# kshedden/muscato

Measured on AMD Instinct MI355X. Metric: reads/sec (100 bp, multi-map) at 1/2/4/8 MI355X; confirm-kernel HBM GB/s vs peak, higher is better.
Workload: dtype u32

## Files before the change

include/muscato_hip.h:

```cpp
#ifndef MUSCATO_HIP_H
#define MUSCATO_HIP_H

#include <stdint.h>

#ifdef __cplusplus
extern "C" {
#endif

#define MUSC_ABI_VERSION 3
#define MUSC_MAX_WINDOWS 16

typedef struct musc_ctx musc_ctx;

typedef struct {
  uint32_t read_idx;
  uint32_t gene_idx;
  uint32_t pos;
  uint32_t nmiss;
} musc_hit;

typedef struct {
  int32_t n_windows;
  int32_t windows[MUSC_MAX_WINDOWS];
  int32_t window_width;
  double pmatch;
  int32_t min_dinuc;
  int32_t max_read_length;
  int32_t max_matches;
  int32_t match_mode;
  int32_t mmtol;
  int32_t apply_mmtol;
  int32_t max_mismatch_p1;
  int32_t skip_block_check;
  int32_t n_shards;
  int32_t reserved[2];
} musc_params;

typedef struct {
  uint64_t n_reads;
  uint64_t n_read_windows;
  uint64_t n_candidates;
  uint64_t n_pairs;
  uint64_t n_accepted;
  uint64_t n_hits;
  uint64_t n_overflow_blocks;
  uint64_t confirm_bytes;
  uint32_t confirm_launches;
  uint32_t n_batches;
  float ms_screen;
  float ms_scan;
  uint32_t match_variant;
  float ms_confirm;
  float ms_select;
  float ms_total;
  float ms_index_build;
  float ms_read_prep;
  uint64_t n_descriptors;
  uint32_t index_kind;
  uint32_t match_launches;
  uint64_t n_overflow_entries;
  uint64_t match_bytes;
  uint64_t match_bytes_strict;
  uint64_t index_bytes;
} musc_stats;

int musc_abi_version(void);

int musc_init(int device_ordinal, musc_ctx** out);
void musc_destroy(musc_ctx* ctx);
const char* musc_last_error(musc_ctx* ctx);
int musc_reload_env(musc_ctx* ctx);

int musc_db_load_ascii(musc_ctx* ctx, const char* seqs, const uint64_t* offsets, uint32_t nseq,
                       int on_device);
int musc_db_load_packed(musc_ctx* ctx, const uint8_t* bases2bit, const uint8_t* nmask,
                        const uint64_t* seq_offsets, uint32_t nseq);
int musc_db_build_index(musc_ctx* ctx, int32_t window_width);
int musc_db_build_index_for(musc_ctx* ctx, const musc_params* params, int32_t max_read_len);

int musc_db_set_partition_bases(musc_ctx* ctx, uint64_t max_bases);
int musc_db_partitions(musc_ctx* ctx, uint32_t* first_target, uint32_t cap, uint32_t* n);

int musc_reads_load_ascii(musc_ctx* ctx, const char* seqs, const uint64_t* offsets,
                          uint64_t nreads, int on_device);
int musc_reads_load_packed(musc_ctx* ctx, const uint8_t* bases2bit, const uint8_t* nmask,
                           const uint64_t* read_offsets, uint64_t nreads);
int musc_reads_load_packed32(musc_ctx* ctx, const uint8_t* bases2bit, const uint8_t* nmask,
                             const uint32_t* lengths, uint32_t fixed_len, uint64_t nreads, int async);

int musc_reads_sort_unique(musc_ctx* ctx, const char* seqs, const uint64_t* offsets, uint64_t nreads,
                           int on_device, uint32_t** order, uint32_t** ustart, uint64_t* nunique);

typedef struct musc_fastq_prep {
  uint64_t n_records, n_short, n_reads, n_unique;
  uint32_t max_len, reserved;
  uint64_t *name_off, *seq_off;
  uint32_t *name_len, *seq_len;
  uint32_t *order, *ustart;
} musc_fastq_prep;
int  musc_reads_prep_fastq(musc_ctx* ctx, const char* text, uint64_t nbytes, int on_device,
                           int32_t min_read_len, int32_t max_read_len, musc_fastq_prep* out);
void musc_fastq_prep_free(musc_fastq_prep* p);

int musc_match_device(musc_ctx* ctx, const musc_params* params, uint64_t* nhits);
int musc_hits_copy(musc_ctx* ctx, musc_hit* dst, uint64_t capacity, int dst_on_device);
int musc_hits_copy_packed(musc_ctx* ctx, uint64_t* dst, uint64_t capacity, int dst_on_device,
                          uint64_t read_base, const int32_t* bits);
int musc_hits_unpack(musc_ctx* ctx, const uint64_t* src, uint64_t n, int on_device, const int32_t* bits,
                     musc_hit* dst);
int musc_hits_copy_compact(musc_ctx* ctx, uint32_t* words, uint64_t words_capacity, uint8_t* counts,
                           uint64_t counts_capacity, int dst_on_device, const int32_t* bits);
int musc_match(musc_ctx* ctx, const musc_params* params, musc_hit** hits, uint64_t* nhits);
void musc_free_hits(musc_hit* hits);

int musc_get_stats(musc_ctx* ctx, musc_stats* out);

int musc_results_set_gene_text(musc_ctx* ctx, const char* text, const uint64_t* offsets, const uint8_t* absent, uint32_t nseq);
int musc_results_set_read_text(musc_ctx* ctx, const char* text, const uint64_t* offsets, uint64_t nreads);
int musc_results_order(musc_ctx* ctx, const musc_hit* hits, uint64_t n, int on_device, uint64_t* nlines, uint64_t* nbytes);
int musc_results_hits(musc_ctx* ctx, musc_hit* dst, uint64_t capacity, int dst_on_device);
int musc_results_text(musc_ctx* ctx, uint64_t line0, uint64_t nlines, char* dst, uint64_t capacity, int dst_on_device,
                      uint64_t* nbytes);
int musc_results_last_ms(musc_ctx* ctx, float* ms_order, float* ms_text);
int musc_results_number_key(uint32_t pos, uint32_t nmiss, uint64_t* key);

#define MUSC_INSTANCE_WORDS 4
#define MUSC_INST_MATCH_T 1u
#define MUSC_INST_MATCH_G 2u
#define MUSC_INST_SCREEN 3u
#define MUSC_INST_SCREEN_T 4u
#define MUSC_INST_CONFIRM 5u
int musc_last_instance(const musc_ctx* ctx, uint32_t* out);
int musc_instances(uint32_t* out, uint32_t capacity, uint32_t* n);

int musc_stream_plan(uint64_t nreads, uint32_t fixed_len, uint32_t batch_reads, uint64_t* ends, uint8_t* is_batch_end,
                     uint64_t capacity, uint64_t* n, uint64_t* planned_batches);

int musc_overflow_probes(musc_ctx* ctx, uint32_t** read_idx, uint32_t** window, uint64_t* n);
void musc_free_u32(uint32_t* p);

int musc_gather(musc_ctx* const* ctxs, int n, const uint64_t* read_base, musc_hit** hits,
                uint64_t* nhits);
int musc_gather_rccl(musc_ctx* const* ctxs, int n, const uint64_t* read_base, musc_hit** hits,
                     uint64_t* nhits);
int musc_rccl_probe(char* msg, uint64_t cap);

#ifdef __cplusplus
}
#endif
#endif
```

muscato_amd/_lib.py:

```python
from __future__ import annotations

import ctypes
import os

HERE = os.path.dirname(os.path.abspath(__file__))
LIB_PATH = os.environ.get("MUSC_LIB_PATH") or os.path.join(HERE, "libmuscato_hip.so")

MUSC_MAX_WINDOWS = 16


class MuscHit(ctypes.Structure):
    _fields_ = [("read_idx", ctypes.c_uint32), ("gene_idx", ctypes.c_uint32),
                ("pos", ctypes.c_uint32), ("nmiss", ctypes.c_uint32)]


class MuscParams(ctypes.Structure):
    _fields_ = [
        ("n_windows", ctypes.c_int32),
        ("windows", ctypes.c_int32 * MUSC_MAX_WINDOWS),
        ("window_width", ctypes.c_int32),
        ("pmatch", ctypes.c_double),
        ("min_dinuc", ctypes.c_int32),
        ("max_read_length", ctypes.c_int32),
        ("max_matches", ctypes.c_int32),
        ("match_mode", ctypes.c_int32),
        ("mmtol", ctypes.c_int32),
        ("apply_mmtol", ctypes.c_int32),
        ("max_mismatch_p1", ctypes.c_int32),
        ("skip_block_check", ctypes.c_int32),
        ("n_shards", ctypes.c_int32),
        ("reserved", ctypes.c_int32 * 2),
    ]


class MuscStats(ctypes.Structure):
    _fields_ = [
        ("n_reads", ctypes.c_uint64), ("n_read_windows", ctypes.c_uint64),
        ("n_candidates", ctypes.c_uint64), ("n_pairs", ctypes.c_uint64), ("n_accepted", ctypes.c_uint64),
        ("n_hits", ctypes.c_uint64), ("n_overflow_blocks", ctypes.c_uint64),
        ("confirm_bytes", ctypes.c_uint64),
        ("confirm_launches", ctypes.c_uint32), ("n_batches", ctypes.c_uint32),
        ("ms_screen", ctypes.c_float), ("ms_scan", ctypes.c_float), ("match_variant", ctypes.c_uint32),
        ("ms_confirm", ctypes.c_float), ("ms_select", ctypes.c_float), ("ms_total", ctypes.c_float),
        ("ms_index_build", ctypes.c_float), ("ms_read_prep", ctypes.c_float),
        ("n_descriptors", ctypes.c_uint64),
        ("index_kind", ctypes.c_uint32), ("match_launches", ctypes.c_uint32),
        ("n_overflow_entries", ctypes.c_uint64), ("match_bytes", ctypes.c_uint64),
        ("match_bytes_strict", ctypes.c_uint64), ("index_bytes", ctypes.c_uint64),
    ]


class MuscFastqPrep(ctypes.Structure):
    _fields_ = [
        ("n_records", ctypes.c_uint64), ("n_short", ctypes.c_uint64), ("n_reads", ctypes.c_uint64), ("n_unique", ctypes.c_uint64),
        ("max_len", ctypes.c_uint32), ("reserved", ctypes.c_uint32),
        ("name_off", ctypes.POINTER(ctypes.c_uint64)), ("seq_off", ctypes.POINTER(ctypes.c_uint64)),
        ("name_len", ctypes.POINTER(ctypes.c_uint32)), ("seq_len", ctypes.POINTER(ctypes.c_uint32)),
        ("order", ctypes.POINTER(ctypes.c_uint32)), ("ustart", ctypes.POINTER(ctypes.c_uint32)),
    ]


SYMBOLS = [
    "musc_abi_version", "musc_init", "musc_destroy", "musc_last_error", "musc_reload_env",
    "musc_db_load_ascii", "musc_db_load_packed", "musc_db_build_index", "musc_db_build_index_for",
    "musc_db_set_partition_bases", "musc_db_partitions",
    "musc_reads_load_ascii", "musc_reads_load_packed", "musc_reads_load_packed32", "musc_reads_sort_unique",
    "musc_reads_prep_fastq", "musc_fastq_prep_free",
    "musc_match_device", "musc_hits_copy", "musc_hits_copy_packed", "musc_hits_copy_compact", "musc_hits_unpack", "musc_match", "musc_free_hits",
    "musc_get_stats", "musc_last_instance", "musc_instances", "musc_stream_plan", "musc_gather", "musc_gather_rccl", "musc_rccl_probe", "musc_overflow_probes", "musc_free_u32",
    "musc_results_set_gene_text", "musc_results_set_read_text", "musc_results_order", "musc_results_hits", "musc_results_text",
    "musc_results_last_ms", "musc_results_number_key",
]

_lib = None


def load() -> ctypes.CDLL:
    global _lib
    if _lib is not None:
        return _lib
    if not os.path.exists(LIB_PATH):
        raise ImportError(
            "muscato_amd: %s is missing -- build it with `python -m muscato_amd.build` "
            "(hipcc, gfx950).  There is no CPU fallback." % LIB_PATH)
    import sys
    torch = sys.modules.get("torch")
    if torch is not None:
        try:
            if torch.cuda.is_available():
                torch.cuda.init()
        except Exception:
            pass
    lib = ctypes.CDLL(LIB_PATH)
    for s in SYMBOLS:
        if not hasattr(lib, s):
            raise ImportError("muscato_amd: %s does not export %s" % (LIB_PATH, s))
    vp, u64, i32 = ctypes.c_void_p, ctypes.c_uint64, ctypes.c_int32
    lib.musc_abi_version.restype = ctypes.c_int
    lib.musc_init.argtypes = [ctypes.c_int, ctypes.POINTER(vp)]
    lib.musc_destroy.argtypes = [vp]
    lib.musc_destroy.restype = None
    lib.musc_last_error.argtypes = [vp]
    lib.musc_last_error.restype = ctypes.c_char_p
    lib.musc_reload_env.argtypes = [vp]
    lib.musc_db_load_ascii.argtypes = [vp, vp, vp, ctypes.c_uint32, ctypes.c_int]
    lib.musc_db_load_packed.argtypes = [vp, vp, vp, vp, ctypes.c_uint32]
    lib.musc_db_build_index.argtypes = [vp, i32]
    lib.musc_db_build_index_for.argtypes = [vp, ctypes.POINTER(MuscParams), i32]
    lib.musc_db_set_partition_bases.argtypes = [vp, u64]
    lib.musc_db_partitions.argtypes = [vp, vp, ctypes.c_uint32, ctypes.POINTER(ctypes.c_uint32)]
    lib.musc_reads_load_ascii.argtypes = [vp, vp, vp, u64, ctypes.c_int]
    lib.musc_reads_load_packed.argtypes = [vp, vp, vp, vp, u64]
    lib.musc_reads_load_packed32.argtypes = [vp, vp, vp, vp, ctypes.c_uint32, u64, ctypes.c_int]
    lib.musc_reads_sort_unique.argtypes = [vp, vp, vp, u64, ctypes.c_int, ctypes.POINTER(vp), ctypes.POINTER(vp),
                                           ctypes.POINTER(u64)]
    lib.musc_reads_prep_fastq.argtypes = [vp, vp, u64, ctypes.c_int, i32, i32, ctypes.POINTER(MuscFastqPrep)]
    lib.musc_reads_prep_fastq.restype = ctypes.c_int
    lib.musc_fastq_prep_free.argtypes = [ctypes.POINTER(MuscFastqPrep)]
    lib.musc_fastq_prep_free.restype = None
    lib.musc_match_device.argtypes = [vp, ctypes.POINTER(MuscParams), ctypes.POINTER(u64)]
    lib.musc_hits_copy.argtypes = [vp, vp, u64, ctypes.c_int]
    lib.musc_hits_copy_packed.argtypes = [vp, vp, u64, ctypes.c_int, u64, ctypes.POINTER(i32)]
    lib.musc_hits_copy_compact.argtypes = [vp, vp, u64, vp, u64, ctypes.c_int, ctypes.POINTER(i32)]
    lib.musc_hits_unpack.argtypes = [vp, vp, u64, ctypes.c_int, ctypes.POINTER(i32), vp]
    lib.musc_match.argtypes = [vp, ctypes.POINTER(MuscParams), ctypes.POINTER(vp), ctypes.POINTER(u64)]
    lib.musc_free_hits.argtypes = [vp]
    lib.musc_free_hits.restype = None
    lib.musc_get_stats.argtypes = [vp, ctypes.POINTER(MuscStats)]
    lib.musc_last_instance.argtypes = [vp, ctypes.POINTER(ctypes.c_uint32)]
    lib.musc_instances.argtypes = [ctypes.POINTER(ctypes.c_uint32), ctypes.c_uint32, ctypes.POINTER(ctypes.c_uint32)]
    lib.musc_stream_plan.argtypes = [u64, ctypes.c_uint32, ctypes.c_uint32, vp, vp, u64, ctypes.POINTER(u64), ctypes.POINTER(u64)]
    lib.musc_overflow_probes.argtypes = [vp, ctypes.POINTER(vp), ctypes.POINTER(vp), ctypes.POINTER(u64)]
    lib.musc_overflow_probes.restype = ctypes.c_int
    lib.musc_free_u32.argtypes = [vp]
    lib.musc_free_u32.restype = None
    lib.musc_gather.argtypes = [ctypes.POINTER(vp), ctypes.c_int, ctypes.POINTER(u64),
                                ctypes.POINTER(vp), ctypes.POINTER(u64)]
    lib.musc_gather_rccl.argtypes = lib.musc_gather.argtypes
    lib.musc_rccl_probe.argtypes = [ctypes.c_char_p, ctypes.c_uint64]
    lib.musc_results_set_gene_text.argtypes = [vp, vp, vp, vp, ctypes.c_uint32]
    lib.musc_results_set_read_text.argtypes = [vp, vp, vp, u64]
    lib.musc_results_order.argtypes = [vp, vp, u64, ctypes.c_int, ctypes.POINTER(u64), ctypes.POINTER(u64)]
    lib.musc_results_hits.argtypes = [vp, vp, u64, ctypes.c_int]
    lib.musc_results_text.argtypes = [vp, u64, u64, vp, u64, ctypes.c_int, ctypes.POINTER(u64)]
    lib.musc_results_last_ms.argtypes = [vp, ctypes.POINTER(ctypes.c_float), ctypes.POINTER(ctypes.c_float)]
    lib.musc_results_number_key.argtypes = [ctypes.c_uint32, ctypes.c_uint32, ctypes.POINTER(u64)]
    for name in ("musc_results_set_gene_text", "musc_results_set_read_text", "musc_results_order", "musc_results_hits",
                 "musc_results_text", "musc_results_last_ms", "musc_results_number_key"):
        getattr(lib, name).restype = ctypes.c_int
    for name in ("musc_init", "musc_reload_env", "musc_db_load_ascii", "musc_db_load_packed", "musc_db_build_index", "musc_db_build_index_for", "musc_db_build_index_for",
                 "musc_db_set_partition_bases", "musc_db_partitions",
                 "musc_reads_load_ascii", "musc_reads_load_packed", "musc_reads_load_packed32", "musc_reads_sort_unique", "musc_match_device",
                 "musc_hits_copy", "musc_hits_copy_packed", "musc_hits_copy_compact", "musc_hits_unpack", "musc_match", "musc_get_stats", "musc_last_instance", "musc_instances",
                 "musc_stream_plan", "musc_gather", "musc_gather_rccl", "musc_rccl_probe"):
        getattr(lib, name).restype = ctypes.c_int
    _lib = lib
    return lib
```

muscato_amd/csrc/muscato_hip.hip:

```cpp

#include <hip/hip_runtime.h>
#include <rccl/rccl.h>
#include <dlfcn.h>

#include <algorithm>
#include <cstdarg>
#include <cstdio>
#include <cstdlib>
#include <cstring>
#include <map>
#include <mutex>
#include <string>
#include <type_traits>
#include <vector>

#include "../../include/muscato_hip.h"

#include "kernels_common.hpp"
#include "kernels_index.hpp"
#include "kernels_screen.hpp"
#include "kernels_confirm.hpp"
#include "kernels_match.hpp"
#include "kernels_match_lane_inst.hpp"
#include "kernels_screen_lane.hpp"
#include "kernels_partition.hpp"
#include "kernels_results.hpp"
MUSC_LANE_INSTANCES_4(extern)
MUSC_LANE_INSTANCES_8(extern)
MUSC_LANE_INSTANCES_12(extern)
MUSC_LANE_INSTANCES_8W(extern)
MUSC_LANE_INSTANCES_12W(extern)
MUSC_LANE_INSTANCES_16W(extern)
MUSC_LANE_INSTANCES_SPEC(extern)
MUSC_DMA_INSTANCES(extern)


namespace {

thread_local std::string g_init_error;

template <class T>
struct DevBuf {
  T* p = nullptr;
  uint64_t cap = 0;
  void release() {
    if (p) (void)hipFree(p);
    p = nullptr;
    cap = 0;
  }
};

struct Roctx {
  int (*push)(const char*) = nullptr;
  int (*pop)() = nullptr;
  Roctx() {
    for (const char* name : {"librocprofiler-sdk-roctx.so.1", "librocprofiler-sdk-roctx.so", "libroctx64.so.4", "libroctx64.so"}) {
      if (void* h = dlopen(name, RTLD_NOW | RTLD_LOCAL)) {
        push = reinterpret_cast<int (*)(const char*)>(dlsym(h, "roctxRangePushA"));
        pop = reinterpret_cast<int (*)()>(dlsym(h, "roctxRangePop"));
        if (push && pop) return;
        push = nullptr;
        pop = nullptr;
      }
    }
  }
};
const Roctx& roctx() {
  static const Roctx r;
  return r;
}
struct Range {
  bool on;
  explicit Range(const char* name) : on(roctx().push != nullptr) {
    if (on) (void)roctx().push(name);
  }
  ~Range() {
    if (on) (void)roctx().pop();
  }
};

struct CaptureGuard {
  hipStream_t st = nullptr;
  bool active = false;
  hipError_t begin(hipStream_t s) {
    const hipError_t e = hipStreamBeginCapture(s, hipStreamCaptureModeThreadLocal);
    if (e == hipSuccess) {
      st = s;
      active = true;
    }
    return e;
  }
  hipError_t end(hipGraph_t* g) {
    active = false;
    return hipStreamEndCapture(st, g);
  }
  ~CaptureGuard() {
    if (!active) return;
    hipGraph_t g = nullptr;
    (void)hipStreamEndCapture(st, &g);
    if (g) (void)hipGraphDestroy(g);
    (void)hipGetLastError();
  }
};

struct TmpBufs {
  void* p[16] = {};
  int n = 0;
  template <class T>
  hipError_t alloc(T** out, size_t bytes) {
    void* q = nullptr;
    *out = nullptr;
    if (n >= 16) return hipErrorOutOfMemory;
    const hipError_t e = hipMalloc(&q, bytes ? bytes : 16);
    if (e == hipSuccess) p[n++] = q;
    *out = (T*)q;
    return e;
  }
  void release() {
    for (int i = 0; i < n; i++) (void)hipFree(p[i]);
    n = 0;
  }
  ~TmpBufs() { release(); }
};

}

struct StreamPlan {
  std::vector<uint64_t> piece_end, batch_end;
};
static void stream_plan(uint64_t nreads, uint64_t batch_reads, StreamPlan* sp) {
  auto up64 = [](uint64_t x) { return (x + 63) & ~63ull; };
  sp->piece_end.clear();
  sp->batch_end.clear();
  const uint64_t full = std::max<uint64_t>(up64(batch_reads), 64);
  const uint64_t last_max = std::max<uint64_t>(up64(batch_reads / 16), 64);
  const uint64_t piece = up64(std::max<uint64_t>(batch_reads / 4, 64));
  for (uint64_t r0 = 0; r0 < nreads;) {
    const uint64_t left = nreads - r0;
    const uint64_t n = left >= 2 * full ? full : left <= last_max ? left : up64((left + 1) / 2);
    for (uint64_t p = r0 + piece; p < r0 + n; p += piece) sp->piece_end.push_back(p);
    r0 += n;
    sp->piece_end.push_back(r0);
    sp->batch_end.push_back(r0);
  }
}
static uint64_t stream_plan_batch(const StreamPlan& sp, uint64_t r0) {
  const auto it = std::upper_bound(sp.batch_end.begin(), sp.batch_end.end(), r0);
  return it == sp.batch_end.end() ? 0 : *it - r0;
}

struct EnvKnobs {
  enum { IDX_AUTO = 0, IDX_CLASSIC, IDX_LINES, IDX_CLASSIC64 };
  int index = IDX_AUTO;
  bool match_dma = false;
  bool screen_wg = false;
  int context = 0;
  bool no_x_context = false;
  bool force_wide = false;
  int index_bits = 0;
  bool ctx_direct = false;
  int debug_grid = 0;
  bool debug_sync = false;
  int graph = -1;
  bool pipeline = false;
  bool no_spec = false;
  long batch_reads = 0;
  long index_budget_mb = 0;
  void read() {
    *this = EnvKnobs();
    auto is = [](const char* v, const char* w) { return v && !strcmp(v, w); };
    const char* e = getenv("MUSC_INDEX");
    index = is(e, "classic") ? IDX_CLASSIC : is(e, "lines") ? IDX_LINES : is(e, "classic64") ? IDX_CLASSIC64 : IDX_AUTO;
    e = getenv("MUSC_MATCH");
    match_dma = is(e, "dma");
    screen_wg = is(getenv("MUSC_SCREEN"), "wg");
    e = getenv("MUSC_CONTEXT");
    context = is(e, "narrow") ? 1 : is(e, "wide") ? 2 : 0;
    no_x_context = getenv("MUSC_NO_X_CONTEXT") != nullptr;
    force_wide = getenv("MUSC_DEBUG_FORCE_WIDE") != nullptr;
    if ((e = getenv("MUSC_DEBUG_INDEX_BITS"))) index_bits = atoi(e);
    ctx_direct = (e = getenv("MUSC_DEBUG_CTX_DIRECT")) && atoi(e) > 0;
    if ((e = getenv("MUSC_DEBUG_GRID"))) debug_grid = atoi(e);
    debug_sync = getenv("MUSC_DEBUG_SYNC") != nullptr;
    if ((e = getenv("MUSC_GRAPH"))) graph = atoi(e);
    if ((e = getenv("MUSC_PIPELINE"))) pipeline = atoi(e) > 0;
    no_spec = getenv("MUSC_NO_SPEC") != nullptr;
    if ((e = getenv("MUSC_BATCH_READS"))) batch_reads = atol(e);
    if ((e = getenv("MUSC_DEBUG_INDEX_BUDGET_MB"))) index_budget_mb = atol(e);
  }
};

struct musc_ctx {
  int device = 0;
  hipStream_t stream = nullptr;
  std::string err;
  EnvKnobs env;

  uint32_t* db2 = nullptr;
  uint32_t* dbm2 = nullptr;
  bool db_has_x = false;
  bool reads_have_x = false;
  DevBuf<uint32_t> rdx;
  uint64_t rdx_epoch = ~0ull;
  int rdx_wide = -1;
  uint64_t xok_epoch = ~0ull;
  double xok_pmatch = -1.0;
  int32_t xok_mmp1 = -1;
  bool xok = false;
  uint32_t* dbx = nullptr;
  uint64_t max_tlen = 0;
  uint64_t xokdb_epoch = ~0ull;
  int32_t xokdb_key[CTX_MAX_W + 3] = {0};
  bool xokdb = false;
  uint64_t* seq_off = nullptr;
  uint32_t nseq = 0;
  uint64_t nbases = 0;
  uint64_t db_words = 0;
  std::vector<uint64_t> h_seq_off;

  uint64_t part_bases = 0;
  std::vector<uint32_t> part_first;
  int part_kind = 0;
  uint64_t part_size = 0;
  uint32_t cur_part = 0;
  DevBuf<musc_hit> pacc;
  DevBuf<uint32_t> pbest;
  DevBuf<uint64_t> pcnt, padj;
  DevBuf<uint32_t> pflags, pflags_tmp;
  DevBuf<uint32_t> block_acc;

  int idx_ww = 0, idx_bits = 0, idx_direct = 0;
  uint32_t idx_g0 = 0, idx_g1 = 0;
  int wide = 0;
  Bucket* idx_T = nullptr;
  uint4* idx_E = nullptr;
  bool idx_lines = false;
  unsigned scrt_resident = 0;
  int scrt_rw = 0;
  uint64_t idx_T_bytes = 0, idx_E_cap = 0;
  uint64_t idx_n = 0;
  uint64_t idx_novf = 0;
  int idx_kind = 0;
  int idx_wide = 0;
  int idx_CL = 0;
  CtxBucket* ctx_T = nullptr;
  CtxEntry* ctx_E = nullptr;
  uint64_t ctx_T_cap = 0, ctx_E_cap = 0;
  PathParams* d_pp = nullptr;
  PathParams h_pp;
  bool h_pp_valid = false;
  MatchParams* d_mp = nullptr;
  MatchParams h_mp;
  bool h_mp_valid = false;
  int spec_geom = 0;
  DevBuf<uint4> spill;

  uint32_t* rd = nullptr;
  uint64_t rd_cap = 0;
  uint32_t* rdm = nullptr;
  uint64_t nreads = 0;
  int rw = 0;
  uint32_t max_len = 0;

  struct Upload {
    uint32_t* stage = nullptr;
    uint64_t stage_words = 0;
    hipStream_t s_up = nullptr;
    std::vector<hipEvent_t> ev;
    StreamPlan plan;
    uint64_t next_piece = 0;
    uint64_t packed_upto = 0;
    uint32_t L = 0;
    bool active = false;
  } up;

  struct BatchSet {
    DevBuf<uint32_t> wb, rvalid, tbase, tcount;
    DevBuf<uint4> cdesc;
  } bs[2];
  int cur = 0;
  hipStream_t stream2 = nullptr;
  hipStream_t s_confirm = nullptr;
  hipEvent_t ev_ready[2] = {nullptr, nullptr}, ev_free[2] = {nullptr, nullptr}, ev_join = nullptr;
  DevBuf<uint32_t> scan_tmp, tcount2, tpre;
  DevBuf<uint4> stage;
  DevBuf<uint32_t> p_nx;
  DevBuf<uint16_t> nmiss_tab;
  DevBuf<uint32_t> block_table;
  bool force_exact_blocks = false;
  uint64_t exact_epoch = 0;
  musc_params exact_params;
  PathParams last_pp;
  uint32_t last_max_matches = 0;
  uint32_t last_inst[MUSC_INSTANCE_WORDS] = {0, 0, 0, 0};
  bool last_exact_blocks = false;
  unsigned long long* counters = nullptr;
  uint64_t* h_pinned = nullptr;

  DevBuf<musc_hit> hits;
  uint64_t nhits = 0;
  DevBuf<uint64_t> packed;
  std::vector<hipEvent_t> dl_ev;
  DevBuf<musc_hit> gathered;
  uint32_t* d_flag = nullptr;

  char* res_gtext = nullptr;
  uint64_t* res_goff = nullptr;
  uint32_t* res_rank = nullptr;
  char* res_ttext = nullptr;
  uint64_t* res_toff = nullptr;
  DevBuf<musc_hit> res_hits;
  DevBuf<uint64_t> res_off;
  DevBuf<unsigned char> res_stage;
  uint64_t res_n = 0, res_bytes = 0;
  bool res_valid = false;
  bool hits_current = false;
  float res_ms_order = 0, res_ms_text = 0;

  uint32_t batch_reads = 16u << 20;
  uint64_t data_epoch = 1;
  uint64_t sized_epoch = 0;
  musc_params sized_params;
  bool sized_exact_blocks = false;
  uint32_t sized_bsz = 0;
  musc_stats stats;
  hipGraphExec_t graph_exec = nullptr;
  bool graph_failed = false;
  uint64_t graph_epoch = 0;
  musc_params graph_params;
  int graph_block_mode = -1;
  uint32_t graph_batches = 0;
  std::vector<hipEvent_t> ev_pool;
  size_t ev_used = 0;
  double nm_pmatch = -1.0;
  int32_t nm_mmp1 = -1;
  uint32_t nm_maxlen = 0xFFFFFFFFu;
};

namespace {

int fail(musc_ctx* c, int code, const char* fmt, ...) {
  char buf[512];
  va_list ap;
  va_start(ap, fmt);
  vsnprintf(buf, sizeof buf, fmt, ap);
  va_end(ap);
  if (c) c->err = buf; else g_init_error = buf;
  return code;
}

#define HIPCHK(c, expr)                                                                 \
  do {                                                                                  \
    hipError_t e_ = (expr);                                                             \
    if (e_ != hipSuccess) {                                                             \
      (void)hipGetLastError();                                                          \
      return fail((c), 10, "%s failed: %s (%s:%d)", #expr, hipGetErrorString(e_), __FILE__, __LINE__); \
    }                                                                                   \
  } while (0)

template <class T>
int ensure(musc_ctx* c, DevBuf<T>& b, uint64_t n, bool keep = false) {
  if (n <= b.cap && b.p) return 0;
  uint64_t ncap = std::max<uint64_t>(n, b.cap + b.cap / 2);
  ncap = std::max<uint64_t>(ncap, 1024);
  T* np = nullptr;
  HIPCHK(c, hipMalloc((void**)&np, ncap * sizeof(T) + 64));
  if (keep && b.p && b.cap) {
    hipError_t e = hipMemcpyAsync(np, b.p, b.cap * sizeof(T), hipMemcpyDeviceToDevice, c->stream);
    if (e == hipSuccess) e = hipStreamSynchronize(c->stream);
    if (e != hipSuccess) {
      (void)hipFree(np);
      return fail(c, 10, "hit buffer grow failed: %s", hipGetErrorString(e));
    }
  }
  b.release();
  b.p = np;
  b.cap = ncap;
  return 0;
}

inline unsigned nblk(uint64_t n, unsigned b) { return (unsigned)((n + b - 1) / b); }

uint64_t scan_tmp_elems(uint64_t n) {
  uint64_t t = 0;
  while (n > SCAN_TILE) {
    n = (n + SCAN_TILE - 1) / SCAN_TILE;
    t += (n + 8 + 3) & ~3ull;
  }
  return t + 8;
}

int scan_u32(musc_ctx* c, const uint32_t* in, uint32_t* out, uint64_t n, bool inclusive, uint32_t* tmp,
             hipStream_t st = nullptr) {
  if (!st) st = c->stream;
  const uint64_t nb = (n + SCAN_TILE - 1) / SCAN_TILE;
  if (nb > 0x7FFFFFFFull) return fail(c, 11, "scan too large");
  if (nb <= 1) {
    if (inclusive) hipLaunchKernelGGL(k_scan_block<true>, dim3(1), dim3(SCAN_BLOCK), 0, st, in, out, (uint32_t*)nullptr, n);
    else hipLaunchKernelGGL(k_scan_block<false>, dim3(1), dim3(SCAN_BLOCK), 0, st, in, out, (uint32_t*)nullptr, n);
    HIPCHK(c, hipGetLastError());
    return 0;
  }
  uint32_t* sums = tmp;
  if (inclusive) hipLaunchKernelGGL(k_scan_block<true>, dim3((unsigned)nb), dim3(SCAN_BLOCK), 0, st, in, out, sums, n);
  else hipLaunchKernelGGL(k_scan_block<false>, dim3((unsigned)nb), dim3(SCAN_BLOCK), 0, st, in, out, sums, n);
  HIPCHK(c, hipGetLastError());
  int rc = scan_u32(c, sums, sums, nb, false, tmp + ((nb + 8 + 3) & ~3ull), st);
  if (rc) return rc;
  hipLaunchKernelGGL(k_scan_add, dim3((unsigned)nb), dim3(SCAN_BLOCK), 0, st, out, sums, n);
  HIPCHK(c, hipGetLastError());
  return 0;
}

int scan_u64(musc_ctx* c, const uint64_t* in, uint64_t* out, uint64_t n, uint64_t* tmp) {
  const uint64_t nb = (n + SCAN_TILE - 1) / SCAN_TILE;
  if (nb > 0x7FFFFFFFull) return fail(c, 11, "scan too large");
  if (nb <= 1) {
    hipLaunchKernelGGL(k_scan64_block, dim3(1), dim3(SCAN_BLOCK), 0, c->stream, in, out, (uint64_t*)nullptr, n);
    HIPCHK(c, hipGetLastError());
    return 0;
  }
  hipLaunchKernelGGL(k_scan64_block, dim3((unsigned)nb), dim3(SCAN_BLOCK), 0, c->stream, in, out, tmp, n);
  HIPCHK(c, hipGetLastError());
  int rc = scan_u64(c, tmp, tmp, nb, tmp + ((nb + 8 + 3) & ~3ull));
  if (rc) return rc;
  hipLaunchKernelGGL(k_scan64_add, dim3((unsigned)nb), dim3(SCAN_BLOCK), 0, c->stream, out, tmp, n);
  HIPCHK(c, hipGetLastError());
  return 0;
}

void free_index(musc_ctx* c) {
  c->idx_ww = 0;
  c->idx_n = 0;
  c->data_epoch++;
}

void drop_ctx_index(musc_ctx* c) {
  if (c->ctx_T) (void)hipFree(c->ctx_T);
  if (c->ctx_E) (void)hipFree(c->ctx_E);
  c->ctx_T = nullptr;
  c->ctx_E = nullptr;
  c->ctx_T_cap = c->ctx_E_cap = 0;
}

void drop_gene_text(musc_ctx* c) {
  if (c->res_gtext) (void)hipFree(c->res_gtext);
  if (c->res_goff) (void)hipFree(c->res_goff);
  if (c->res_rank) (void)hipFree(c->res_rank);
  c->res_gtext = nullptr;
  c->res_goff = nullptr;
  c->res_rank = nullptr;
  c->res_valid = false;
  c->hits_current = false;
}
void drop_read_text(musc_ctx* c) {
  if (c->res_ttext) (void)hipFree(c->res_ttext);
  if (c->res_toff) (void)hipFree(c->res_toff);
  c->res_ttext = nullptr;
  c->res_toff = nullptr;
  c->res_valid = false;
}
void forget_read_text(musc_ctx* c) {
  drop_read_text(c);
  c->hits_current = false;
}

void free_db(musc_ctx* c) {
  free_index(c);
  drop_gene_text(c);
  if (c->db2) (void)hipFree(c->db2);
  if (c->dbm2) (void)hipFree(c->dbm2);
  if (c->dbx) (void)hipFree(c->dbx);
  if (c->seq_off) (void)hipFree(c->seq_off);
  c->db2 = c->dbm2 = c->dbx = nullptr;
  c->db_has_x = false;
  c->seq_off = nullptr;
  c->nseq = 0;
  c->nbases = 0;
  c->h_seq_off.clear();
  c->part_first.clear();
  c->data_epoch++;
}

void drop_reads(musc_ctx* c, bool keep_rd) {
  if (c->up.active) {
    (void)hipStreamSynchronize(c->up.s_up);
    c->up.active = false;
  }
  if (c->rd && !(keep_rd && c->rd_cap)) {
    (void)hipFree(c->rd);
    c->rd = nullptr;
    c->rd_cap = 0;
  }
  if (c->rdm) (void)hipFree(c->rdm);
  c->rdm = nullptr;
  forget_read_text(c);
  c->reads_have_x = false;
  c->nreads = 0;
  c->rw = 0;
  c->data_epoch++;
}
void free_reads(musc_ctx* c) { drop_reads(c, false); }

struct EvPair {
  hipEvent_t a, b;
};

hipEvent_t pool_event(musc_ctx* c) {
  if (c->ev_used == c->ev_pool.size()) {
    hipEvent_t e = nullptr;
    if (hipEventCreate(&e) != hipSuccess) return nullptr;
    c->ev_pool.push_back(e);
  }
  return c->ev_pool[c->ev_used++];
}

struct Timer {
  musc_ctx* c;
  bool off = false;
  std::vector<EvPair> ev[5];
  explicit Timer(musc_ctx* ctx) : c(ctx) { c->ev_used = 0; }
  int begin(int fam, hipStream_t s = nullptr) {
    if (off) return 0;
    EvPair p;
    p.a = pool_event(c);
    p.b = pool_event(c);
    if (!p.a || !p.b) return 1;
    (void)hipEventRecord(p.a, s ? s : c->stream);
    ev[fam].push_back(p);
    return 0;
  }
  void end(int fam, hipStream_t s = nullptr) {
    if (!off && !ev[fam].empty()) (void)hipEventRecord(ev[fam].back().b, s ? s : c->stream);
  }
  float total(int fam) {
    float t = 0;
    for (auto& p : ev[fam]) {
      float ms = 0;
      if (hipEventElapsedTime(&ms, p.a, p.b) == hipSuccess) t += ms;
    }
    return t;
  }
};

int check_params(musc_ctx* c, const musc_params* P) {
  if (!P) return fail(c, 2, "params is NULL");
  if (P->n_windows < 1 || P->n_windows > MUSC_MAX_WINDOWS)
    return fail(c, 2, "n_windows=%d outside 1..%d", P->n_windows, MUSC_MAX_WINDOWS);
  if (P->window_width < 1 || P->window_width > 4096) return fail(c, 2, "bad window_width=%d", P->window_width);
  for (int k = 0; k < P->n_windows; k++)
    if (P->windows[k] < 0 || P->windows[k] > 60000) return fail(c, 2, "bad window start %d", P->windows[k]);
  if (!(P->pmatch >= 0.0 && P->pmatch <= 1.0)) return fail(c, 2, "PMatch=%g outside [0,1]", P->pmatch);
  if (P->match_mode != 0 && P->match_mode != 1) return fail(c, 2, "match_mode must be 0 (best) or 1 (first)");
  if (P->mmtol < 0) return fail(c, 2, "MMTol < 0");
  if (P->max_mismatch_p1 < 0) return fail(c, 2, "max_mismatch_p1 < 0");
  return 0;
}

}

extern "C" {

int musc_abi_version(void) { return MUSC_ABI_VERSION; }

const char* musc_last_error(musc_ctx* ctx) { return ctx ? ctx->err.c_str() : g_init_error.c_str(); }

int musc_init(int device_ordinal, musc_ctx** out) {
  if (!out) return fail(nullptr, 2, "musc_init: out is NULL");
  *out = nullptr;
  int ndev = 0;
  hipError_t e = hipGetDeviceCount(&ndev);
  if (e != hipSuccess || ndev == 0)
    return fail(nullptr, 3, "musc_init: no HIP device (%s); this library has no CPU fallback",
                e == hipSuccess ? "device count 0" : hipGetErrorString(e));
  if (device_ordinal < 0 || device_ordinal >= ndev)
    return fail(nullptr, 2, "musc_init: device %d outside 0..%d", device_ordinal, ndev - 1);
  hipDeviceProp_t prop;
  if ((e = hipGetDeviceProperties(&prop, device_ordinal)) != hipSuccess)
    return fail(nullptr, 3, "musc_init: hipGetDeviceProperties: %s", hipGetErrorString(e));
  if (strncmp(prop.gcnArchName, "gfx950", 6) != 0)
    return fail(nullptr, 3, "musc_init: device %d is %s; this library is built for gfx950 only",
                device_ordinal, prop.gcnArchName);
  if ((e = hipSetDevice(device_ordinal)) != hipSuccess)
    return fail(nullptr, 3, "musc_init: hipSetDevice: %s", hipGetErrorString(e));
  musc_ctx* c = new musc_ctx();
  c->device = device_ordinal;
  memset(&c->stats, 0, sizeof c->stats);
  if ((e = hipStreamCreateWithFlags(&c->stream, hipStreamNonBlocking)) != hipSuccess ||
      (e = hipStreamCreateWithFlags(&c->stream2, hipStreamNonBlocking)) != hipSuccess ||
      (e = hipEventCreateWithFlags(&c->ev_ready[0], hipEventDisableTiming)) != hipSuccess ||
      (e = hipEventCreateWithFlags(&c->ev_ready[1], hipEventDisableTiming)) != hipSuccess ||
      (e = hipEventCreateWithFlags(&c->ev_free[0], hipEventDisableTiming)) != hipSuccess ||
      (e = hipEventCreateWithFlags(&c->ev_free[1], hipEventDisableTiming)) != hipSuccess ||
      (e = hipEventCreateWithFlags(&c->ev_join, hipEventDisableTiming)) != hipSuccess ||
      (e = hipMalloc((void**)&c->counters, CNT_WORDS * sizeof(unsigned long long))) != hipSuccess ||
      (e = hipMalloc((void**)&c->d_flag, 4)) != hipSuccess ||
      (e = hipMalloc((void**)&c->d_mp, sizeof(MatchParams))) != hipSuccess ||
      (e = hipMalloc((void**)&c->d_pp, sizeof(PathParams))) != hipSuccess ||
      (e = hipHostMalloc((void**)&c->h_pinned, CNT_WORDS * sizeof(uint64_t))) != hipSuccess) {
    fail(nullptr, 3, "musc_init: %s", hipGetErrorString(e));
    musc_destroy(c);
    return 3;
  }
  c->env.read();
  if (c->env.batch_reads >= 1 && c->env.batch_reads <= (16l << 20)) c->batch_reads = (uint32_t)c->env.batch_reads;
  *out = c;
  return 0;
}

int musc_reload_env(musc_ctx* c) {
  if (!c) return 1;
  c->env.read();
  c->sized_epoch = 0;
  return 0;
}

void musc_destroy(musc_ctx* c) {
  if (!c) return;
  (void)hipSetDevice(c->device);
  if (c->stream) (void)hipStreamSynchronize(c->stream);
  if (c->stream2) (void)hipStreamSynchronize(c->stream2);
  free_db(c);
  free_reads(c);
  if (c->idx_T) (void)hipFree(c->idx_T);
  if (c->idx_E) (void)hipFree(c->idx_E);
  if (c->ctx_T) (void)hipFree(c->ctx_T);
  if (c->ctx_E) (void)hipFree(c->ctx_E);
  if (c->d_mp) (void)hipFree(c->d_mp);
  if (c->d_pp) (void)hipFree(c->d_pp);
  c->spill.release();
  for (int i = 0; i < 2; i++) {
    c->bs[i].wb.release(); c->bs[i].tbase.release(); c->bs[i].rvalid.release(); c->bs[i].tcount.release();
    c->bs[i].cdesc.release();
  }
  c->scan_tmp.release(); c->tcount2.release(); c->tpre.release(); c->stage.release(); c->rdx.release();
  c->p_nx.release();
  c->nmiss_tab.release();
  c->block_table.release();
  c->pacc.release(); c->pbest.release(); c->pcnt.release(); c->padj.release(); c->pflags.release(); c->pflags_tmp.release();
  c->block_acc.release();
  c->hits.release();
  c->packed.release();
  c->gathered.release();
  c->res_hits.release(); c->res_off.release(); c->res_stage.release();
  if (c->d_flag) (void)hipFree(c->d_flag);
  if (c->counters) (void)hipFree(c->counters);
  if (c->h_pinned) (void)hipHostFree(c->h_pinned);
  for (hipEvent_t ev : {c->ev_ready[0], c->ev_ready[1], c->ev_free[0], c->ev_free[1], c->ev_join})
    if (ev) (void)hipEventDestroy(ev);
  for (hipEvent_t ev : c->ev_pool) (void)hipEventDestroy(ev);
  if (c->graph_exec) (void)hipGraphExecDestroy(c->graph_exec);
  for (hipEvent_t ev : c->up.ev) (void)hipEventDestroy(ev);
  for (hipEvent_t ev : c->dl_ev) (void)hipEventDestroy(ev);
  if (c->up.stage) (void)hipFree(c->up.stage);
  if (c->up.s_up) (void)hipStreamDestroy(c->up.s_up);
  if (c->stream2) (void)hipStreamDestroy(c->stream2);
  if (c->stream) (void)hipStreamDestroy(c->stream);
  delete c;
}


static int db_xblocks(musc_ctx* c) {
  const uint64_t nblk64 = (c->db_words + 64 + 3) / 4;
  const uint64_t nw = nblk64 / 32 + 4;
  if (c->dbx) (void)hipFree(c->dbx);
  c->dbx = nullptr;
  HIPCHK(c, hipMalloc((void**)&c->dbx, nw * 4));
  HIPCHK(c, hipMemsetAsync(c->dbx, 0, nw * 4, c->stream));
  hipLaunchKernelGGL(k_db_xblocks, dim3(nblk(nblk64, 256)), dim3(256), 0, c->stream, c->dbm2, c->db_words, c->dbx);
  HIPCHK(c, hipGetLastError());
  HIPCHK(c, hipStreamSynchronize(c->stream));
  return 0;
}

static int db_finish(musc_ctx* c) {
  uint32_t hasx = 0;
  HIPCHK(c, hipMemcpyAsync(&hasx, c->d_flag, 4, hipMemcpyDeviceToHost, c->stream));
  unsigned long long tl = 0;
  HIPCHK(c, hipMemsetAsync(c->counters + CNT_SCRATCH, 0, 8, c->stream));
  hipLaunchKernelGGL(k_max_len, dim3(std::min(nblk(c->nseq, 256), MAX_GRID)), dim3(256), 0, c->stream, c->seq_off, (uint64_t)c->nseq, c->counters + CNT_SCRATCH);
  HIPCHK(c, hipGetLastError());
  HIPCHK(c, hipMemcpyAsync(&tl, c->counters + CNT_SCRATCH, 8, hipMemcpyDeviceToHost, c->stream));
  HIPCHK(c, hipStreamSynchronize(c->stream));
  c->max_tlen = tl;
  c->db_has_x = hasx != 0;
  if (!hasx) {
    (void)hipFree(c->dbm2);
    c->dbm2 = nullptr;
    return 0;
  }
  return db_xblocks(c);
}

static int db_alloc(musc_ctx* c, const uint64_t* offsets, uint32_t nseq, int on_device) {
  HIPCHK(c, hipSetDevice(c->device));
  free_db(c);
  if (nseq == 0) return fail(c, 2, "database has no sequences");
  uint64_t first = 0, last = 0;
  if (on_device) {
    HIPCHK(c, hipMemcpy(&first, offsets, 8, hipMemcpyDeviceToHost));
    HIPCHK(c, hipMemcpy(&last, offsets + nseq, 8, hipMemcpyDeviceToHost));
  } else {
    first = offsets[0];
    last = offsets[nseq];
  }
  if (first != 0) return fail(c, 2, "offsets[0] must be 0");
  if (last >= (1ull << 36)) return fail(c, 2, "database larger than 2^36 bases");
  c->nseq = nseq;
  c->nbases = last;
  c->db_words = (last + 15) / 16;
  c->h_seq_off.resize((size_t)nseq + 1);
  if (on_device) HIPCHK(c, hipMemcpy(c->h_seq_off.data(), offsets, ((uint64_t)nseq + 1) * 8, hipMemcpyDeviceToHost));
  else memcpy(c->h_seq_off.data(), offsets, ((uint64_t)nseq + 1) * 8);
  const uint64_t alloc_words = c->db_words + 64;
  HIPCHK(c, hipMalloc((void**)&c->db2, alloc_words * 4));
  HIPCHK(c, hipMalloc((void**)&c->dbm2, alloc_words * 4));
  HIPCHK(c, hipMemsetAsync(c->db2, 0, alloc_words * 4, c->stream));
  HIPCHK(c, hipMemsetAsync(c->dbm2, 0, alloc_words * 4, c->stream));
  HIPCHK(c, hipMalloc((void**)&c->seq_off, ((uint64_t)nseq + 1) * 8));
  HIPCHK(c, hipMemcpyAsync(c->seq_off, offsets, ((uint64_t)nseq + 1) * 8,
                           on_device ? hipMemcpyDeviceToDevice : hipMemcpyHostToDevice, c->stream));
  HIPCHK(c, hipMemsetAsync(c->d_flag, 0, 4, c->stream));
  return 0;
}

int musc_db_load_ascii(musc_ctx* c, const char* seqs, const uint64_t* offsets, uint32_t nseq, int on_device) {
  if (!c) return 1;
  if (!seqs || !offsets) return fail(c, 2, "musc_db_load_ascii: NULL input");
  int rc = db_alloc(c, offsets, nseq, on_device);
  if (rc) return rc;
  const unsigned char* src = (const unsigned char*)seqs;
  TmpBufs B;
  unsigned char* tmp = nullptr;
  if (!on_device && c->nbases) {
    HIPCHK(c, B.alloc(&tmp, c->nbases));
    HIPCHK(c, hipMemcpyAsync(tmp, seqs, c->nbases, hipMemcpyHostToDevice, c->stream));
    src = tmp;
  }
  if (c->db_words) {
    hipLaunchKernelGGL(k_pack_db_ascii, dim3(nblk(c->db_words, 256)), dim3(256), 0, c->stream, src, c->nbases,
                       c->db2, c->dbm2, c->db_words, c->d_flag);
    HIPCHK(c, hipGetLastError());
  }
  return db_finish(c);
}

int musc_db_load_packed(musc_ctx* c, const uint8_t* bases2bit, const uint8_t* nmask, const uint64_t* seq_offsets,
                        uint32_t nseq) {
  if (!c) return 1;
  if (!bases2bit || !seq_offsets) return fail(c, 2, "musc_db_load_packed: NULL input");
  int rc = db_alloc(c, seq_offsets, nseq, 0);
  if (rc) return rc;
  TmpBufs B;
  uint32_t* t2 = nullptr;
  uint16_t* tm = nullptr;
  const uint64_t w = c->db_words;
  if (w) {
    HIPCHK(c, B.alloc(&t2, w * 4));
    HIPCHK(c, hipMemsetAsync(t2, 0, w * 4, c->stream));
    HIPCHK(c, hipMemcpyAsync(t2, bases2bit, (c->nbases + 3) / 4, hipMemcpyHostToDevice, c->stream));
    if (nmask) {
      HIPCHK(c, B.alloc(&tm, w * 2));
      HIPCHK(c, hipMemsetAsync(tm, 0, w * 2, c->stream));
      HIPCHK(c, hipMemcpyAsync(tm, nmask, (c->nbases + 7) / 8, hipMemcpyHostToDevice, c->stream));
    }
    hipLaunchKernelGGL(k_pack_db_packed, dim3(nblk(w, 256)), dim3(256), 0, c->stream, t2, tm, c->db2, c->dbm2, w,
                       c->d_flag);
    HIPCHK(c, hipGetLastError());
  }
  return db_finish(c);
}

extern "C++" {
struct IdxRange {
  uint32_t g0, g1;
  uint64_t b0, b1, size;
};
static IdxRange whole_db(const musc_ctx* c) { return IdxRange{0, c->nseq, 0, c->nbases, c->nbases}; }

static uint64_t index_room(musc_ctx* c, uint64_t reserve) {
  size_t mfree = 0, mtotal = 0;
  if (hipMemGetInfo(&mfree, &mtotal) != hipSuccess) {
    (void)hipGetLastError();
    return 0;
  }
  const uint64_t have = (uint64_t)mfree + c->idx_T_bytes + c->idx_E_cap * sizeof(uint4) +
                        (c->ctx_T ? c->ctx_T_cap * sizeof(CtxBucket) : 0) + (c->ctx_E ? c->ctx_E_cap * sizeof(CtxEntry) : 0);
  uint64_t room = have > reserve ? have - reserve : 0;
  if (c->env.index_budget_mb > 0) room = std::min<uint64_t>(room, (uint64_t)c->env.index_budget_mb << 20);
  return room;
}

static uint64_t lines_need(uint64_t nb, uint64_t bases) {
  return (nb + 1) * (sizeof(LineBucket) + 8) + (bases > 7 * nb ? (bases - 7 * nb) * 16 : 0) + nb * 64;
}
static uint64_t classic64_need(uint64_t nb, uint64_t bases) { return (nb + 1) * (sizeof(Bucket) + 16) + bases * sizeof(uint4); }
static const uint64_t LINES_RESERVE = 12ull << 30, CLASSIC_RESERVE = 4ull << 30, CTX_RESERVE = 4ull << 30;

static bool want_line_buckets(musc_ctx* c, int32_t ww, int bits, int direct, uint64_t bases) {
  if (c->env.index == EnvKnobs::IDX_LINES) return true;
  if (c->env.index == EnvKnobs::IDX_CLASSIC64) return false;
  if (!direct) return false;
  (void)ww;
  const uint64_t nb = 1ull << bits;
  if (bases < 4 * nb) return false;
  return lines_need(nb, bases) <= index_room(c, LINES_RESERVE);
}

static void classic_table(const musc_ctx* c, int32_t ww, uint64_t bases, int* bits, int* direct) {
  *direct = 0;
  const uint64_t floor_bases = std::max<uint64_t>(bases, 1ull << 19);
  if (2 * ww <= 30 && (1ull << (2 * ww)) <= 32 * floor_bases) {
    *bits = 2 * ww;
    *direct = 1;
  } else {
    *bits = 10;
    while (*bits < 31 && (1ull << *bits) < bases) (*bits)++;
  }
  if (c->env.index_bits >= 8 && c->env.index_bits <= 31) { *bits = c->env.index_bits; *direct = 0; }
}

static void ctx_table(const musc_ctx* c, int32_t ww, uint64_t bases, int* bits, int* direct) {
  *direct = 0;
  const uint64_t floor_bases = std::max<uint64_t>(bases, 1ull << 9);
  if (2 * ww <= 30 && ((1ull << (2 * ww)) <= 2 * floor_bases || c->env.ctx_direct)) {
    *bits = 2 * ww;
    *direct = 1;
  } else {
    *bits = 10;
    while (*bits < 30 && (1ull << *bits) < bases) (*bits)++;
  }
  if (c->env.index_bits >= 8 && c->env.index_bits <= 30) { *bits = c->env.index_bits; *direct = 0; }
}
static uint64_t ctx_need(int bits, int wide, uint64_t bases) {
  const uint64_t esz = wide ? sizeof(CtxEntryW) : sizeof(CtxEntry);
  return ((1ull << bits) + 1) * (sizeof(CtxBucket) + 12) + bases / (wide ? 2 : 3) * esz;
}

template <class BT>
static int build_index_buckets(musc_ctx* c, int32_t ww, int bits, int direct, const IdxRange& R) {
  const uint64_t nb = 1ull << bits;
  c->ev_used = 0;
  hipEvent_t e0 = pool_event(c), e1 = pool_event(c), e2 = pool_event(c), e3 = pool_event(c);
  if (!e0 || !e1 || !e2 || !e3) return fail(c, 10, "hipEventCreate failed");
  if (c->idx_T_bytes < (nb + 1) * sizeof(BT)) {
    if (c->idx_T) (void)hipFree(c->idx_T);
    c->idx_T = nullptr;
    c->idx_T_bytes = 0;
    HIPCHK(c, hipMalloc((void**)&c->idx_T, (nb + 1) * sizeof(BT)));
    c->idx_T_bytes = (nb + 1) * sizeof(BT);
  }
  BT* const T = reinterpret_cast<BT*>(c->idx_T);
  TmpBufs B;
  uint64_t *tmp = nullptr, *stmp = nullptr;
  HIPCHK(c, B.alloc(&tmp, (nb + 1 + 16) * 8));
  HIPCHK(c, B.alloc(&stmp, scan_tmp_elems(nb + 1) * 8));
  HIPCHK(c, hipEventRecord(e0, c->stream));
  HIPCHK(c, hipMemsetAsync(T, 0, (nb + 1) * sizeof(BT), c->stream));
  const unsigned blocks = (unsigned)std::min<uint64_t>((R.b1 - R.b0 + 255) / 256, 1u << 22);
  if (R.b1 > R.b0) {
    hipLaunchKernelGGL((k_index<false, BT>), dim3(blocks), dim3(256), 0, c->stream, c->db2, c->dbm2, c->seq_off, c->nseq,
                       R.b0, R.b1, ww, bits, direct, c->wide, T, (uint4*)nullptr);
    HIPCHK(c, hipGetLastError());
  }
  hipLaunchKernelGGL((k_index_ovf_count<BT>), dim3(nblk(nb + 1, 256)), dim3(256), 0, c->stream, T, nb, tmp);
  HIPCHK(c, hipGetLastError());
  int rc = scan_u64(c, tmp, tmp, nb + 1, stmp);
  if (rc) return rc;
  uint64_t novf = 0;
  HIPCHK(c, hipMemcpyAsync(&novf, tmp + nb, 8, hipMemcpyDeviceToHost, c->stream));
  hipLaunchKernelGGL((k_index_ovf_set<BT>), dim3(nblk(nb, 256)), dim3(256), 0, c->stream, T, nb, tmp);
  HIPCHK(c, hipGetLastError());
  HIPCHK(c, hipEventRecord(e2, c->stream));
  HIPCHK(c, hipStreamSynchronize(c->stream));
  B.release();
  if (std::is_same<BT, LineBucket>::value) {
    if (novf >= 0xFFFFFFF0ull) return fail(c, 5, "internal: %llu overflow lines do not fit 32-bit numbers", (unsigned long long)novf);
    novf *= 8;
  }
  c->idx_novf = novf;
  if (c->idx_E_cap < novf + 16) {
    if (c->idx_E) (void)hipFree(c->idx_E);
    c->idx_E = nullptr;
    c->idx_E_cap = 0;
    HIPCHK(c, hipMalloc((void**)&c->idx_E, ((uint64_t)novf + 16) * sizeof(uint4)));
    c->idx_E_cap = novf + 16;
  }
  HIPCHK(c, hipEventRecord(e3, c->stream));
  if (R.b1 > R.b0) {
    hipLaunchKernelGGL((k_index<true, BT>), dim3(blocks), dim3(256), 0, c->stream, c->db2, c->dbm2, c->seq_off, c->nseq,
                       R.b0, R.b1, ww, bits, direct, c->wide, T, c->idx_E);
    HIPCHK(c, hipGetLastError());
  }
  HIPCHK(c, hipEventRecord(e1, c->stream));
  HIPCHK(c, hipStreamSynchronize(c->stream));
  float ms = 0, ms2 = 0;
  (void)hipEventElapsedTime(&ms, e0, e2);
  (void)hipEventElapsedTime(&ms2, e3, e1);
  c->stats.ms_index_build = ms + ms2;
  return 0;
}
}

static int build_index_classic(musc_ctx* c, int32_t ww, const IdxRange& R, int lines_kind) {
  c->wide = c->nbases >= 0xFFFFFFF0ull || c->env.force_wide;
  if (c->wide && c->nseq >= (1u << 24))
    return fail(c, 5, "a database of 2^32 bases or more may hold at most 2^24 targets (has %u)", c->nseq);
  int bits, direct;
  classic_table(c, ww, R.size, &bits, &direct);
  if (c->idx_ww == ww && c->idx_kind == 0 && c->idx_T && c->idx_bits == bits && c->idx_direct == direct &&
      c->idx_g0 == R.g0 && c->idx_g1 == R.g1 && (lines_kind < 0 || c->idx_lines == (lines_kind == 1)) &&
      !(c->env.index == EnvKnobs::IDX_LINES && !c->idx_lines) && !(c->env.index == EnvKnobs::IDX_CLASSIC64 && c->idx_lines))
    return 0;
  const bool lines = lines_kind >= 0 ? lines_kind == 1 : want_line_buckets(c, ww, bits, direct, R.size) && bits <= 30;
  free_index(c);
  drop_ctx_index(c);
  c->idx_kind = 0;
  c->idx_lines = lines;
  const int rc = lines ? build_index_buckets<LineBucket>(c, ww, bits, direct, R) : build_index_buckets<Bucket>(c, ww, bits, direct, R);
  if (rc) return rc;
  c->idx_ww = ww;
  c->idx_bits = bits;
  c->idx_direct = direct;
  c->idx_g0 = R.g0;
  c->idx_g1 = R.g1;
  return 0;
}

int musc_db_build_index(musc_ctx* c, int32_t ww) {
  if (!c) return 1;
  if (!c->db2) return fail(c, 4, "no database loaded");
  if (ww < 1 || ww > 4096) return fail(c, 2, "bad window width %d", ww);
  HIPCHK(c, hipSetDevice(c->device));
  return build_index_classic(c, ww, whole_db(c), -1);
}

static int build_index_ctx(musc_ctx* c, int32_t ww, int32_t CL, int wide, const IdxRange& R) {
  int bits, direct;
  ctx_table(c, ww, R.size, &bits, &direct);
  if (c->idx_kind == 1 && c->idx_ww == ww && c->idx_CL == CL && c->idx_wide == wide && c->idx_bits == bits &&
      c->idx_direct == direct && c->idx_g0 == R.g0 && c->idx_g1 == R.g1 && c->ctx_T)
    return 0;
  free_index(c);
  c->wide = 0;
  const uint64_t nb = 1ull << bits;
  if (ctx_need(bits, wide, R.size) > index_room(c, CTX_RESERVE)) return 100;
  if (c->idx_T) (void)hipFree(c->idx_T);
  if (c->idx_E) (void)hipFree(c->idx_E);
  c->idx_T = nullptr;
  c->idx_E = nullptr;
  c->idx_T_bytes = c->idx_E_cap = 0;
  c->ev_used = 0;
  hipEvent_t e0 = pool_event(c), e1 = pool_event(c), e2 = pool_event(c), e3 = pool_event(c);
  if (!e0 || !e1 || !e2 || !e3) return fail(c, 10, "hipEventCreate failed");
  if (c->ctx_T_cap < nb + 1) {
    if (c->ctx_T) (void)hipFree(c->ctx_T);
    c->ctx_T = nullptr;
    c->ctx_T_cap = 0;
    if (hipMalloc((void**)&c->ctx_T, (nb + 1) * sizeof(CtxBucket)) != hipSuccess) {
      (void)hipGetLastError();
      c->ctx_T = nullptr;
      return 100;
    }
    c->ctx_T_cap = nb + 1;
  }
  TmpBufs B;
  uint64_t *tmp = nullptr, *stmp = nullptr;
  uint32_t* cursor = nullptr;
  if (B.alloc(&tmp, (nb + 1 + 16) * 8) != hipSuccess || B.alloc(&stmp, scan_tmp_elems(nb + 1) * 8) != hipSuccess ||
      B.alloc(&cursor, (nb + 1) * 4) != hipSuccess) {
    (void)hipGetLastError();
    return 100;
  }
  HIPCHK(c, hipEventRecord(e0, c->stream));
  HIPCHK(c, hipMemsetAsync(c->ctx_T, 0, (nb + 1) * sizeof(CtxBucket), c->stream));
  HIPCHK(c, hipMemsetAsync(cursor, 0, (nb + 1) * 4, c->stream));
  const unsigned blocks = (unsigned)std::min<uint64_t>((R.b1 - R.b0 + 255) / 256, 1u << 22);
  const uint32_t* const xm2 = c->db_has_x ? c->dbm2 : nullptr;
  const uint32_t* const xbl = c->db_has_x ? c->dbx : nullptr;
  if (R.b1 > R.b0) {
    hipLaunchKernelGGL((k_index_ctx<false, false>), dim3(blocks), dim3(256), 0, c->stream, c->db2, xm2, xbl, c->seq_off, c->nseq, c->nbases,
                       R.b0, R.b1, ww, bits, direct, CL, c->ctx_T, (void*)nullptr, cursor);
    HIPCHK(c, hipGetLastError());
  }
  hipLaunchKernelGGL(k_ctx_ovf_count, dim3(nblk(nb + 1, 256)), dim3(256), 0, c->stream, c->ctx_T, nb,
                     (uint32_t)(wide ? CTXW_INLINE : CTX_INLINE), tmp);
  HIPCHK(c, hipGetLastError());
  int rc = scan_u64(c, tmp, tmp, nb + 1, stmp);
  if (rc) return rc;
  uint64_t novf = 0;
  HIPCHK(c, hipMemcpyAsync(&novf, tmp + nb, 8, hipMemcpyDeviceToHost, c->stream));
  hipLaunchKernelGGL(k_ctx_ovf_set, dim3(nblk(nb, 256)), dim3(256), 0, c->stream, c->ctx_T, nb, tmp);
  HIPCHK(c, hipGetLastError());
  HIPCHK(c, hipEventRecord(e2, c->stream));
  HIPCHK(c, hipStreamSynchronize(c->stream));
  if (novf >= 0xFFFFFFF0ull) return fail(c, 5, "internal: %llu overflow entries do not fit 32-bit offsets", (unsigned long long)novf);
  c->idx_novf = novf;
  const uint64_t ecap = (ctx_entries_bytes(novf + 16, wide) + sizeof(CtxEntry) - 1) / sizeof(CtxEntry);
  if (c->ctx_E_cap < ecap) {
    if (c->ctx_E) (void)hipFree(c->ctx_E);
    c->ctx_E = nullptr;
    c->ctx_E_cap = 0;
    if (hipMalloc((void**)&c->ctx_E, ecap * sizeof(CtxEntry)) != hipSuccess) {
      (void)hipGetLastError();
      c->ctx_E = nullptr;
      return 100;
    }
    c->ctx_E_cap = ecap;
  }
  HIPCHK(c, hipEventRecord(e3, c->stream));
  if (R.b1 > R.b0) {
    if (wide)
      hipLaunchKernelGGL((k_index_ctx<true, true>), dim3(blocks), dim3(256), 0, c->stream, c->db2, xm2, xbl, c->seq_off, c->nseq, c->nbases,
                         R.b0, R.b1, ww, bits, direct, CL, c->ctx_T, (void*)c->ctx_E, cursor);
    else
      hipLaunchKernelGGL((k_index_ctx<true, false>), dim3(blocks), dim3(256), 0, c->stream, c->db2, xm2, xbl, c->seq_off, c->nseq, c->nbases,
                         R.b0, R.b1, ww, bits, direct, CL, c->ctx_T, (void*)c->ctx_E, cursor);
    HIPCHK(c, hipGetLastError());
  }
  HIPCHK(c, hipEventRecord(e1, c->stream));
  HIPCHK(c, hipStreamSynchronize(c->stream));
  float ms = 0, ms2 = 0;
  (void)hipEventElapsedTime(&ms, e0, e2);
  (void)hipEventElapsedTime(&ms2, e3, e1);
  c->stats.ms_index_build = ms + ms2;
  c->idx_kind = 1;
  c->idx_wide = wide;
  c->idx_ww = ww;
  c->idx_CL = CL;
  c->idx_bits = bits;
  c->idx_direct = direct;
  c->idx_g0 = R.g0;
  c->idx_g1 = R.g1;
  return 0;
}

enum MatchKind { MK_LANE = 2, MK_DMA = 3 };
static int match_kind(const musc_ctx* c, int W) {
  if (c->env.match_dma && W == 2 && c->rw == 8 && c->idx_kind == 1 && !c->idx_wide && !c->db_has_x && !c->reads_have_x) return MK_DMA;
  return MK_LANE;
}

static bool reads_xpos(musc_ctx* c, int wide) {
  if (c->rdx_epoch == c->data_epoch && c->rdx_wide == wide) return true;
  if (ensure(c, c->rdx, c->nreads)) return false;
  if (wide)
    hipLaunchKernelGGL(k_read_xpos<true>, dim3(nblk(c->nreads, 256)), dim3(256), 0, c->stream, c->rd, c->rdm, c->nreads, c->rw, c->rdx.p);
  else
    hipLaunchKernelGGL(k_read_xpos<false>, dim3(nblk(c->nreads, 256)), dim3(256), 0, c->stream, c->rd, c->rdm, c->nreads, c->rw, c->rdx.p);
  if (hipGetLastError() != hipSuccess) return false;
  c->rdx_epoch = c->data_epoch;
  c->rdx_wide = wide;
  c->xok_epoch = ~0ull;
  c->xokdb_epoch = ~0ull;
  return true;
}

static bool reads_x_fit(musc_ctx* c, const musc_params* P, uint32_t max_len, int wide) {
  if (!c->rdm || !c->rd || !c->nreads) return false;
  if (c->env.no_x_context) return false;
  if (!reads_xpos(c, wide)) return false;
  max_len = std::max(max_len, c->max_len);
  if (c->xok_epoch == c->data_epoch && c->xok_pmatch == P->pmatch && c->xok_mmp1 == P->max_mismatch_p1) return c->xok;
  std::vector<uint16_t> tab((size_t)max_len + 2);
  for (uint32_t L = 0; L < tab.size(); L++) {
    volatile double a = 1.0 - P->pmatch;
    volatile double b = a * (double)L;
    long long v = (long long)b;
    if (P->max_mismatch_p1 > 0) v = P->max_mismatch_p1 - 1;
    if (v < 0) v = 0;
    if (v > 0xFFFE) v = 0xFFFE;
    tab[L] = (uint16_t)v;
  }
  TmpBufs B;
  uint16_t* d_tab = nullptr;
  uint32_t bad = 1;
  if (B.alloc(&d_tab, tab.size() * 2) != hipSuccess) return false;
  if (hipMemcpyAsync(d_tab, tab.data(), tab.size() * 2, hipMemcpyHostToDevice, c->stream) != hipSuccess) return false;
  if (hipMemsetAsync(c->d_flag, 0, 4, c->stream) != hipSuccess) return false;
  hipLaunchKernelGGL(k_xpos_check, dim3(nblk(c->nreads, 256)), dim3(256), 0, c->stream, c->rd, c->rdx.p, c->nreads, c->rw, d_tab,
                     max_len, wide ? XPos<true>::MAX : XPos<false>::MAX, c->d_flag);
  if (hipMemcpyAsync(&bad, c->d_flag, 4, hipMemcpyDeviceToHost, c->stream) != hipSuccess) return false;
  if (hipStreamSynchronize(c->stream) != hipSuccess) return false;
  c->xok = bad == 0;
  c->xok_epoch = c->data_epoch;
  c->xok_pmatch = P->pmatch;
  c->xok_mmp1 = P->max_mismatch_p1;
  return c->xok;
}

static bool reads_x_fit_db(musc_ctx* c, const musc_params* P, int wide) {
  if (!c->rdm || !c->rd || !c->nreads) return false;
  if (!reads_xpos(c, wide)) return false;
  int32_t key[CTX_MAX_W + 3] = {P->n_windows, P->window_width, wide};
  XWins wn;
  memset(&wn, 0, sizeof wn);
  wn.n = P->n_windows;
  wn.ww = P->window_width;
  for (int k = 0; k < P->n_windows && k < CTX_MAX_W; k++) key[3 + k] = wn.q1[k] = P->windows[k];
  if (c->xokdb_epoch == c->data_epoch && memcmp(key, c->xokdb_key, sizeof key) == 0) return c->xokdb;
  uint32_t bad = 1;
  if (hipMemsetAsync(c->d_flag, 0, 4, c->stream) != hipSuccess) return false;
  if (wide) hipLaunchKernelGGL(k_xpos_check_db<true>, dim3(nblk(c->nreads, 256)), dim3(256), 0, c->stream, c->rdx.p, c->nreads, wn, c->d_flag);
  else hipLaunchKernelGGL(k_xpos_check_db<false>, dim3(nblk(c->nreads, 256)), dim3(256), 0, c->stream, c->rdx.p, c->nreads, wn, c->d_flag);
  if (hipMemcpyAsync(&bad, c->d_flag, 4, hipMemcpyDeviceToHost, c->stream) != hipSuccess) return false;
  if (hipStreamSynchronize(c->stream) != hipSuccess) return false;
  c->xokdb = bad == 0;
  c->xokdb_epoch = c->data_epoch;
  memcpy(c->xokdb_key, key, sizeof key);
  return c->xokdb;
}

static bool ctx_eligible(musc_ctx* c, const musc_params* P, uint32_t max_len, int* CL, int* wide) {
  if (c->env.index != EnvKnobs::IDX_AUTO) return false;
  if (c->db_has_x && (c->max_tlen >= 0x80000000ull || c->nseq > (1u << 24) || c->env.no_x_context)) return false;
  if (c->nbases >= 0xFFFFFFF0ull || c->env.force_wide) return false;
  if (P->n_windows > CTX_MAX_W) return false;
  int q1min = P->windows[0], q1max = P->windows[0];
  for (int k = 1; k < P->n_windows; k++) {
    q1min = std::min(q1min, P->windows[k]);
    q1max = std::max(q1max, P->windows[k]);
  }
  const int64_t span = (int64_t)q1max - q1min + (int64_t)max_len;
  const int wenv = c->env.context;
  *CL = q1max;
  *wide = 0;
  if (span > CTX_BASES || q1max > CTX_BASES || wenv == 2) {
    if (wenv == 1) return false;
    if (span > CTXW_BASES || q1max > CTXW_BASES) return false;
    *wide = 1;
  }
  if (c->reads_have_x && !(c->db_has_x ? reads_x_fit_db(c, P, *wide) : reads_x_fit(c, P, max_len, *wide))) return false;
  return true;
}

enum { PK_CTX = 1, PK_LINES = 2, PK_CLASSIC64 = 3 };
static const uint32_t MAX_PARTITIONS = 4096;

static int index_kind_for(musc_ctx* c, int32_t ww, bool ctx_ok, int wide, uint64_t bases, bool fit, uint64_t extra) {
  int bits, direct;
  if (ctx_ok) {
    ctx_table(c, ww, bases, &bits, &direct);
    if (ctx_need(bits, wide, bases) <= index_room(c, CTX_RESERVE + extra)) return PK_CTX;
  }
  classic_table(c, ww, bases, &bits, &direct);
  const uint64_t nb = 1ull << bits;
  const bool lines = bits <= 30 && (c->env.index == EnvKnobs::IDX_LINES ||
                                    (c->env.index != EnvKnobs::IDX_CLASSIC64 && direct && bases >= 4 * nb &&
                                     lines_need(nb, bases) <= index_room(c, LINES_RESERVE + extra)));
  if (lines) return !fit || lines_need(nb, bases) <= index_room(c, LINES_RESERVE + extra) ? PK_LINES : 0;
  return !fit || classic64_need(nb, bases) <= index_room(c, CLASSIC_RESERVE + extra) ? PK_CLASSIC64 : 0;
}

static uint64_t merge_reserve(const musc_ctx* c) {
  const uint64_t tuples = std::max<uint64_t>(c->hits.cap, c->nreads);
  return 20 * (c->nreads + 1) + (4ull << BLOCK_TABLE_BITS) + 20 * tuples;
}

static bool cut_targets(const musc_ctx* c, uint64_t limit, std::vector<uint32_t>* first, uint64_t* largest) {
  const std::vector<uint64_t>& off = c->h_seq_off;
  limit = std::min(limit, c->nbases);
  first->assign(1, 0u);
  *largest = 0;
  uint32_t g = 0;
  while (g < c->nseq) {
    uint32_t g1 = (uint32_t)(std::upper_bound(off.begin() + g + 1, off.begin() + c->nseq + 1, off[g] + limit) - off.begin()) - 1;
    if (g1 <= g) g1 = g + 1;
    *largest = std::max<uint64_t>(*largest, off[g1] - off[g]);
    first->push_back(g1);
    if (first->size() > MAX_PARTITIONS + 1) return false;
    g = g1;
  }
  return true;
}

static int plan_partitions(musc_ctx* c, const musc_params* P, uint32_t max_len) {
  const int32_t ww = P->window_width;
  const std::vector<uint32_t> one = {0u, c->nseq};
  if (!c->part_bases && c->idx_ww == ww && c->idx_g0 == 0 && c->idx_g1 == c->nseq && c->nseq) {
    c->part_first = one;
    return 0;
  }
  int CL = 0, wide = 0;
  const bool ctx_ok = ctx_eligible(c, P, max_len, &CL, &wide);
  std::vector<uint32_t> first;
  uint64_t largest = 0;
  int kind = 0;
  if (c->part_bases) {
    if (!cut_targets(c, c->part_bases, &first, &largest))
      return fail(c, 5, "DbPartitionBases %llu cuts the database into more than %u partitions",
                  (unsigned long long)c->part_bases, MAX_PARTITIONS);
    const uint64_t extra = first.size() > 2 ? merge_reserve(c) : 0;
    kind = index_kind_for(c, ww, ctx_ok, wide, largest, true, extra);
    if (!kind) kind = index_kind_for(c, ww, false, wide, largest, false, 0);
  } else if (index_kind_for(c, ww, ctx_ok, wide, c->nbases, true, 0)) {
    first = one;
  } else {
    uint32_t lo = 2, hi = MAX_PARTITIONS;
    bool found = false;
    while (lo <= hi) {
      const uint32_t n = lo + (hi - lo) / 2;
      std::vector<uint32_t> f;
      uint64_t lg = 0;
      const bool ok = cut_targets(c, (c->nbases + n - 1) / n, &f, &lg);
      const int k = ok ? index_kind_for(c, ww, ctx_ok, wide, lg, true, merge_reserve(c)) : 0;
      if (k) {
        first.swap(f);
        largest = lg;
        kind = k;
        found = true;
        hi = n - 1;
      } else {
        lo = n + 1;
      }
    }
    if (!found)
      return fail(c, 5, "the index of this database does not fit the device even in %u partitions", MAX_PARTITIONS);
  }
  c->part_first = first;
  c->part_kind = first.size() > 2 ? kind : 0;
  c->part_size = first.size() > 2 ? largest : c->nbases;
  return 0;
}

static int ensure_index(musc_ctx* c, const musc_params* P, uint32_t max_len) {
  int CL = 0, wide = 0;
  if (c->part_first.size() > 2) {
    const uint32_t p = c->cur_part;
    const uint32_t g0 = c->part_first[p], g1 = c->part_first[p + 1];
    const IdxRange R{g0, g1, c->h_seq_off[g0], c->h_seq_off[g1], c->part_size};
    if (c->part_kind == PK_CTX) {
      if (!ctx_eligible(c, P, max_len, &CL, &wide)) return fail(c, 12, "internal: a partition lost context-bucket eligibility");
      const int rc = build_index_ctx(c, P->window_width, CL, wide, R);
      if (rc == 100)
        return fail(c, 5, "the context index of partition %u (%llu bases) does not fit the device", p,
                    (unsigned long long)(R.b1 - R.b0));
      return rc;
    }
    return build_index_classic(c, P->window_width, R, c->part_kind == PK_LINES ? 1 : 0);
  }
  if (ctx_eligible(c, P, max_len, &CL, &wide)) {
    const int rc = build_index_ctx(c, P->window_width, CL, wide, whole_db(c));
    if (rc != 100) return rc;
  }
  return musc_db_build_index(c, P->window_width);
}

int musc_db_build_index_for(musc_ctx* c, const musc_params* P, int32_t max_read_len) {
  if (!c) return 1;
  int rc = check_params(c, P);
  if (rc) return rc;
  if (!c->db2) return fail(c, 4, "no database loaded");
  HIPCHK(c, hipSetDevice(c->device));
  const uint32_t ml = max_read_len > 0 ? (uint32_t)max_read_len
                                       : (P->max_read_length > 0 ? (uint32_t)P->max_read_length : c->max_len);
  if ((rc = plan_partitions(c, P, ml))) return rc;
  c->cur_part = 0;
  return ensure_index(c, P, ml);
}

int musc_db_set_partition_bases(musc_ctx* c, uint64_t max_bases) {
  if (!c) return 1;
  c->part_bases = max_bases;
  return 0;
}

int musc_db_partitions(musc_ctx* c, uint32_t* first_target, uint32_t cap, uint32_t* n) {
  if (!c) return 1;
  if (!n) return fail(c, 2, "musc_db_partitions: n is NULL");
  *n = c->part_first.empty() ? 0u : (uint32_t)c->part_first.size() - 1;
  if (!first_target || !*n) return 0;
  if (cap < *n + 1) return fail(c, 2, "musc_db_partitions: room for %u boundaries < %u", cap, *n + 1);
  memcpy(first_target, c->part_first.data(), (*n + 1) * sizeof(uint32_t));
  return 0;
}


static int upload_prepare(musc_ctx* c, uint64_t r0, uint64_t n, hipStream_t st) {
  musc_ctx::Upload& u = c->up;
  if (!u.active) return 0;
  const uint64_t want = std::min<uint64_t>(r0 + n, c->nreads);
  while (u.packed_upto < want && u.next_piece < u.plan.piece_end.size()) {
    const uint64_t i = u.next_piece;
    const uint64_t first = u.packed_upto, cnt = u.plan.piece_end[i] - first;
    HIPCHK(c, hipStreamWaitEvent(st, u.ev[i], 0));
    hipLaunchKernelGGL(k_pack_reads_fixed, dim3(nblk(cnt * (uint64_t)c->rw, 256)), dim3(256), 0, st, u.stage, first, cnt, u.L, c->rw, c->rd);
    HIPCHK(c, hipGetLastError());
    u.packed_upto = first + cnt;
    u.next_piece = i + 1;
  }
  if (u.packed_upto >= c->nreads) u.active = false;
  return 0;
}

static int reads_load(musc_ctx* c, const unsigned char* ascii, const uint8_t* bases2bit, const uint8_t* nmask,
                      const uint64_t* offsets, uint64_t nreads, int on_device, bool packed) {
  HIPCHK(c, hipSetDevice(c->device));
  free_reads(c);
  if (nreads >= 0xFFFFFFF0ull) return fail(c, 2, "too many reads for 32-bit read_idx");
  c->nreads = nreads;
  if (nreads == 0) {
    c->rw = 4;
    return 0;
  }
  TmpBufs B;
  uint64_t* d_off = nullptr;
  const uint64_t* offp = offsets;
  if (!on_device) {
    HIPCHK(c, B.alloc(&d_off, (nreads + 1) * 8));
    HIPCHK(c, hipMemcpyAsync(d_off, offsets, (nreads + 1) * 8, hipMemcpyHostToDevice, c->stream));
    offp = d_off;
  }
  HIPCHK(c, hipMemsetAsync(c->counters + CNT_SCRATCH, 0, 8, c->stream));
  hipLaunchKernelGGL(k_max_len, dim3(std::min(nblk(nreads, 256), MAX_GRID)), dim3(256), 0, c->stream, offp, nreads, c->counters + CNT_SCRATCH);
  HIPCHK(c, hipGetLastError());
  HIPCHK(c, hipMemcpyAsync(c->h_pinned, c->counters + CNT_SCRATCH, 8, hipMemcpyDeviceToHost, c->stream));
  uint64_t first = 0, total = 0;
  HIPCHK(c, hipMemcpyAsync(&first, offp, 8, hipMemcpyDeviceToHost, c->stream));
  HIPCHK(c, hipMemcpyAsync(&total, offp + nreads, 8, hipMemcpyDeviceToHost, c->stream));
  HIPCHK(c, hipStreamSynchronize(c->stream));
  const uint64_t maxlen = c->h_pinned[0];
  if (first != 0) return fail(c, 2, "read offsets[0] must be 0");
  if (maxlen > 65535) return fail(c, 2, "read of %llu bases exceeds the 65535-base record limit", (unsigned long long)maxlen);
  c->max_len = (uint32_t)maxlen;
  int rw = (int)((2 * maxlen + 31) / 32) + 1;
  rw = (rw + 3) & ~3;
  if (rw < 4) rw = 4;
  c->rw = rw;
  const uint64_t words = nreads * (uint64_t)rw;
  if (words >= (1ull << 32)) return fail(c, 2, "too many read words for one dispatch (reads x record words >= 2^32)");
  HIPCHK(c, hipMalloc((void**)&c->rd, words * 4 + 256));
  HIPCHK(c, hipMemsetAsync(c->rd + words, 0, 256, c->stream));
  const bool may_have_x = !packed || nmask != nullptr;
  if (may_have_x) {
    HIPCHK(c, hipMalloc((void**)&c->rdm, words * 4 + 256));
    HIPCHK(c, hipMemsetAsync(c->rdm + words, 0, 256, c->stream));
  }
  uint32_t* d_hasx = c->d_flag;
  HIPCHK(c, hipMemsetAsync(d_hasx, 0, 4, c->stream));
  unsigned char *t1 = nullptr, *t2 = nullptr;
  if (!packed) {
    const unsigned char* src = ascii;
    if (!on_device && total) {
      HIPCHK(c, B.alloc(&t1, total));
      HIPCHK(c, hipMemcpyAsync(t1, ascii, total, hipMemcpyHostToDevice, c->stream));
      src = t1;
    }
    hipLaunchKernelGGL(k_pack_reads<false>, dim3(nblk(words, 256)), dim3(256), 0, c->stream, src,
                       (const uint32_t*)nullptr, (const uint32_t*)nullptr, offp, nreads, rw, c->rd, c->rdm, d_hasx);
  } else {
    const uint64_t b2 = ((total + 3) / 4 + 7) & ~3ull, bm = ((total + 7) / 8 + 7) & ~3ull;
    HIPCHK(c, B.alloc(&t1, b2 + 16));
    HIPCHK(c, hipMemsetAsync(t1, 0, b2 + 16, c->stream));
    HIPCHK(c, hipMemcpyAsync(t1, bases2bit, (total + 3) / 4, hipMemcpyHostToDevice, c->stream));
    if (nmask) {
      HIPCHK(c, B.alloc(&t2, bm + 16));
      HIPCHK(c, hipMemsetAsync(t2, 0, bm + 16, c->stream));
      HIPCHK(c, hipMemcpyAsync(t2, nmask, (total + 7) / 8, hipMemcpyHostToDevice, c->stream));
    }
    hipLaunchKernelGGL(k_pack_reads<true>, dim3(nblk(words, 256)), dim3(256), 0, c->stream,
                       (const unsigned char*)nullptr, (const uint32_t*)t1, (const uint32_t*)t2, offp, nreads, rw,
                       c->rd, c->rdm, d_hasx);
  }
  HIPCHK(c, hipGetLastError());
  uint32_t hasx = 0;
  HIPCHK(c, hipMemcpyAsync(&hasx, d_hasx, 4, hipMemcpyDeviceToHost, c->stream));
  HIPCHK(c, hipStreamSynchronize(c->stream));
  c->reads_have_x = hasx != 0;
  if (!hasx && c->rdm) {
    (void)hipFree(c->rdm);
    c->rdm = nullptr;
  }
  return 0;
}

static int reads_load_fixed(musc_ctx* c, const uint8_t* bases2bit, uint32_t L, uint64_t nreads, int async) {
  HIPCHK(c, hipSetDevice(c->device));
  drop_reads(c, true);
  int rw = (int)((2ull * L + 31) / 32) + 1;
  rw = (rw + 3) & ~3;
  if (rw < 4) rw = 4;
  const uint64_t words = nreads * (uint64_t)rw;
  const char* refuse = nreads >= 0xFFFFFFF0ull ? "too many reads for 32-bit read_idx"
                       : L > 65535             ? "read length exceeds the 65535-base record limit"
                       : words >= (1ull << 32) ? "too many read words for one dispatch (reads x record words >= 2^32)"
                                               : nullptr;
  if (refuse) {
    free_reads(c);
    return fail(c, 2, "%s", refuse);
  }
  c->nreads = nreads;
  if (nreads == 0) {
    c->rw = 4;
    return 0;
  }
  c->max_len = L;
  c->rw = rw;
  c->reads_have_x = false;
  musc_ctx::Upload& u = c->up;
  const uint64_t total_bytes = (nreads * (uint64_t)L + 3) / 4;
  const uint64_t need_words = (total_bytes + 3) / 4 + 4;
  if (u.stage_words < need_words) {
    if (u.stage) (void)hipFree(u.stage);
    u.stage = nullptr;
    u.stage_words = 0;
    HIPCHK(c, hipMalloc((void**)&u.stage, need_words * 4));
    u.stage_words = need_words;
  }
  if (!u.s_up) HIPCHK(c, hipStreamCreateWithFlags(&u.s_up, hipStreamNonBlocking));
  stream_plan(nreads, c->batch_reads, &u.plan);
  const std::vector<uint64_t>& ends = u.plan.piece_end;
  u.L = L;
  u.packed_upto = 0;
  u.next_piece = 0;
  while (u.ev.size() < ends.size()) {
    hipEvent_t e = nullptr;
    HIPCHK(c, hipEventCreateWithFlags(&e, hipEventDisableTiming));
    u.ev.push_back(e);
  }
  HIPCHK(c, hipMemsetAsync(u.stage + (need_words - 4), 0, 16, u.s_up));
  for (size_t i = 0; i < ends.size(); i++) {
    const uint64_t b0 = (i ? ends[i - 1] : 0) * (uint64_t)L / 4;
    const uint64_t b1 = std::min<uint64_t>((ends[i] * (uint64_t)L + 3) / 4, total_bytes);
    HIPCHK(c, hipMemcpyAsync(reinterpret_cast<uint8_t*>(u.stage) + b0, bases2bit + b0, b1 - b0, hipMemcpyHostToDevice, u.s_up));
    HIPCHK(c, hipEventRecord(u.ev[i], u.s_up));
  }
  u.active = true;
  if (c->rd_cap < words * 4 + 256) {
    if (c->rd) (void)hipFree(c->rd);
    c->rd = nullptr;
    c->rd_cap = 0;
    HIPCHK(c, hipMalloc((void**)&c->rd, words * 4 + 256));
    c->rd_cap = words * 4 + 256;
  }
  HIPCHK(c, hipMemsetAsync(c->rd + words, 0, 256, c->stream));
  if (!async) {
    int rc = upload_prepare(c, 0, nreads, c->stream);
    if (rc) return rc;
    HIPCHK(c, hipStreamSynchronize(c->stream));
  }
  return 0;
}

int musc_reads_load_packed32(musc_ctx* c, const uint8_t* bases2bit, const uint8_t* nmask, const uint32_t* lengths,
                             uint32_t fixed_len, uint64_t nreads, int async) {
  if (!c) return 1;
  if (!bases2bit && nreads) return fail(c, 2, "musc_reads_load_packed32: NULL input");
  if (!lengths && !nmask) return reads_load_fixed(c, bases2bit, fixed_len, nreads, async);
  HIPCHK(c, hipSetDevice(c->device));
  TmpBufs B;
  uint64_t *d_off = nullptr, *stmp = nullptr;
  uint32_t* d_len = nullptr;
  HIPCHK(c, B.alloc(&d_off, (nreads + 2) * 8));
  if (lengths) {
    HIPCHK(c, B.alloc(&d_len, (nreads + 1) * 4));
    HIPCHK(c, B.alloc(&stmp, scan_tmp_elems(nreads + 1) * 8));
    HIPCHK(c, hipMemcpyAsync(d_len, lengths, nreads * 4, hipMemcpyHostToDevice, c->stream));
    hipLaunchKernelGGL(k_widen_u32, dim3(nblk(nreads + 1, 256)), dim3(256), 0, c->stream, d_len, nreads, d_off);
    HIPCHK(c, hipGetLastError());
    int rc = scan_u64(c, d_off, d_off, nreads + 1, stmp);
    if (rc) return rc;
  } else {
    hipLaunchKernelGGL(k_iota_mul, dim3(nblk(nreads + 1, 256)), dim3(256), 0, c->stream, d_off, nreads, (uint64_t)fixed_len);
    HIPCHK(c, hipGetLastError());
  }
  return reads_load(c, nullptr, bases2bit, nmask, d_off, nreads, 1, true);
}

int musc_reads_load_ascii(musc_ctx* c, const char* seqs, const uint64_t* offsets, uint64_t nreads, int on_device) {
  if (!c) return 1;
  if ((!seqs || !offsets) && nreads) return fail(c, 2, "musc_reads_load_ascii: NULL input");
  return reads_load(c, (const unsigned char*)seqs, nullptr, nullptr, offsets, nreads, on_device, false);
}

int musc_reads_load_packed(musc_ctx* c, const uint8_t* bases2bit, const uint8_t* nmask, const uint64_t* read_offsets,
                           uint64_t nreads) {
  if (!c) return 1;
  if ((!bases2bit || !read_offsets) && nreads) return fail(c, 2, "musc_reads_load_packed: NULL input");
  return reads_load(c, nullptr, bases2bit, nmask, read_offsets, nreads, 0, true);
}


static int match_partitioned(musc_ctx* c, const musc_params* P, uint64_t* nhits);

}

#include "muscato_pass.hpp"

extern "C" {

static int match_partitions_run(musc_ctx* c, const musc_params* P, uint64_t* nhits) {
  const uint32_t np = (uint32_t)c->part_first.size() - 1;
  const uint64_t nr = c->nreads;
  const bool check_blocks = !P->skip_block_check;
  const uint32_t BT = 1u << BLOCK_TABLE_BITS;
  int rc = 0;
  if ((rc = ensure(c, c->pbest, nr + 1))) return rc;
  HIPCHK(c, hipMemsetAsync(c->pbest.p, 0xFF, (nr + 1) * 4, c->stream));
  if (check_blocks) {
    if ((rc = ensure(c, c->block_acc, BT))) return rc;
    HIPCHK(c, hipMemsetAsync(c->block_acc.p, 0, (uint64_t)BT * 4, c->stream));
  }
  musc_stats sum;
  memset(&sum, 0, sizeof sum);
  std::vector<uint64_t> seg(np + 1, 0);
  for (uint32_t p = 0; p < np && !rc; p++) {
    c->cur_part = p;
    uint64_t nh = 0;
    if ((rc = ensure_index(c, P, c->max_len))) break;
    const float build_ms = c->stats.ms_index_build;
    if ((rc = match_index_pass(c, P, &nh))) break;
    const musc_stats& s = c->stats;
    sum.n_read_windows += s.n_read_windows;
    sum.n_candidates += s.n_candidates;
    sum.n_pairs += s.n_pairs;
    sum.n_accepted += s.n_accepted;
    sum.confirm_bytes += s.confirm_bytes;
    sum.confirm_launches += s.confirm_launches;
    sum.n_batches += s.n_batches;
    sum.ms_screen += s.ms_screen;
    sum.ms_scan += s.ms_scan;
    sum.ms_confirm += s.ms_confirm;
    sum.ms_select += s.ms_select;
    sum.ms_total += s.ms_total;
    sum.ms_index_build += build_ms;
    sum.n_descriptors += s.n_descriptors;
    sum.match_launches += s.match_launches;
    sum.n_overflow_entries += s.n_overflow_entries;
    sum.match_bytes += s.match_bytes;
    sum.match_bytes_strict += s.match_bytes_strict;
    sum.index_kind = s.index_kind;
    sum.match_variant = s.match_variant;
    sum.index_bytes = s.index_bytes;
    if (nh) {
      if ((rc = ensure(c, c->pacc, seg[p] + nh, true))) break;
      HIPCHK(c, hipMemcpyAsync(c->pacc.p + seg[p], c->hits.p, nh * sizeof(musc_hit), hipMemcpyDeviceToDevice, c->stream));
      hipLaunchKernelGGL(k_part_best, dim3(std::min(nblk(nh, 256), 4u * MAX_GRID)), dim3(256), 0, c->stream,
                         reinterpret_cast<const uint4*>(c->pacc.p + seg[p]), nh, c->pbest.p);
      HIPCHK(c, hipGetLastError());
    }
    if (check_blocks) {
      hipLaunchKernelGGL(k_add_u32, dim3(nblk(BT, 256)), dim3(256), 0, c->stream, c->block_acc.p, c->block_table.p, (uint64_t)BT);
      HIPCHK(c, hipGetLastError());
    }
    seg[p + 1] = seg[p] + nh;
  }
  if (rc) return rc;

  Range rg("partition merge");
  hipEvent_t ev0 = pool_event(c), ev1 = pool_event(c);
  if (!ev0 || !ev1) return fail(c, 10, "hipEventCreate failed");
  HIPCHK(c, hipEventRecord(ev0, c->stream));
  const uint64_t total_in = seg[np];
  const uint32_t mmtol = P->mmtol > 0xFFFF ? 0xFFFFu : (uint32_t)P->mmtol;
  uint64_t max_seg = 0;
  for (uint32_t p = 0; p < np; p++) max_seg = std::max(max_seg, seg[p + 1] - seg[p]);
  if (max_seg >= 0xFFFFFFFFull) return fail(c, 6, "one partition returned %llu tuples (>= 2^32)", (unsigned long long)max_seg);
  if ((rc = ensure(c, c->pcnt, nr + 1)) || (rc = ensure(c, c->padj, nr + 1)) ||
      (rc = ensure(c, c->pflags, max_seg + 1)) || (rc = ensure(c, c->pflags_tmp, scan_tmp_elems(max_seg + 1))))
    return rc;
  if (scan_tmp_elems(nr + 1) * 2 > c->pflags_tmp.cap && (rc = ensure(c, c->pflags_tmp, scan_tmp_elems(nr + 1) * 2)))
    return rc;
  HIPCHK(c, hipMemsetAsync(c->pcnt.p, 0, (nr + 1) * 8, c->stream));
  if (total_in) {
    hipLaunchKernelGGL(k_part_count, dim3(std::min(nblk(total_in, 256), 4u * MAX_GRID)), dim3(256), 0, c->stream,
                       reinterpret_cast<const uint4*>(c->pacc.p), total_in, c->pbest.p, mmtol, P->apply_mmtol,
                       reinterpret_cast<unsigned long long*>(c->pcnt.p));
    HIPCHK(c, hipGetLastError());
  }
  if ((rc = scan_u64(c, c->pcnt.p, c->pcnt.p, nr + 1, reinterpret_cast<uint64_t*>(c->pflags_tmp.p)))) return rc;
  HIPCHK(c, hipMemcpyAsync(c->h_pinned, c->pcnt.p + nr, 8, hipMemcpyDeviceToHost, c->stream));
  HIPCHK(c, hipStreamSynchronize(c->stream));
  const uint64_t total = c->h_pinned[0];
  if ((rc = ensure(c, c->hits, total ? total : 1))) return rc;
  HIPCHK(c, hipMemsetAsync(c->d_flag, 0, 4, c->stream));
  for (uint32_t p = 0; p < np; p++) {
    const uint64_t n = seg[p + 1] - seg[p];
    if (!n) continue;
    const uint4* const h = reinterpret_cast<const uint4*>(c->pacc.p + seg[p]);
    const dim3 grid(std::min(nblk(n + 1, 256), 4u * MAX_GRID));
    hipLaunchKernelGGL(k_part_flags, grid, dim3(256), 0, c->stream, h, n, c->pbest.p, mmtol, P->apply_mmtol, c->pflags.p);
    HIPCHK(c, hipGetLastError());
    if ((rc = scan_u32(c, c->pflags.p, c->pflags.p, n + 1, false, c->pflags_tmp.p, c->stream))) return rc;
    hipLaunchKernelGGL(k_part_head, grid, dim3(256), 0, c->stream, h, n, c->pflags.p, c->pcnt.p, c->padj.p);
    HIPCHK(c, hipGetLastError());
    hipLaunchKernelGGL(k_part_scatter, grid, dim3(256), 0, c->stream, h, n, c->pflags.p, c->padj.p, c->pcnt.p,
                       reinterpret_cast<uint4*>(c->hits.p), total, c->d_flag);
    HIPCHK(c, hipGetLastError());
  }
  if (check_blocks) {
    HIPCHK(c, hipMemcpyAsync(c->block_table.p, c->block_acc.p, (uint64_t)BT * 4, hipMemcpyDeviceToDevice, c->stream));
    HIPCHK(c, hipMemsetAsync(c->counters + CNT_OVF_BLOCKS, 0, 8, c->stream));
    hipLaunchKernelGGL(k_block_overflow, dim3(1024), dim3(256), 0, c->stream, c->block_table.p, c->last_max_matches, c->counters);
    HIPCHK(c, hipGetLastError());
  }
  HIPCHK(c, hipEventRecord(ev1, c->stream));
  c->h_pinned[1] = 0;
  HIPCHK(c, hipMemcpyAsync(c->h_pinned, c->counters + CNT_OVF_BLOCKS, 8, hipMemcpyDeviceToHost, c->stream));
  HIPCHK(c, hipMemcpyAsync(c->h_pinned + 1, c->d_flag, 4, hipMemcpyDeviceToHost, c->stream));
  HIPCHK(c, hipStreamSynchronize(c->stream));
  if (c->h_pinned[1]) return fail(c, 12, "internal: the partition merge overran its %llu tuples", (unsigned long long)total);
  float merge_ms = 0;
  (void)hipEventElapsedTime(&merge_ms, ev0, ev1);
  sum.ms_select += merge_ms;
  sum.ms_total += merge_ms;
  sum.n_reads = nr;
  sum.n_hits = c->nhits = total;
  sum.n_overflow_blocks = check_blocks ? c->h_pinned[0] : ~0ull;
  c->stats = sum;
  c->last_exact_blocks = check_blocks;
  if (nhits) *nhits = total;
  return 0;
}

static int match_partitioned(musc_ctx* c, const musc_params* P, uint64_t* nhits) {
  const bool keep_force = c->force_exact_blocks;
  c->force_exact_blocks = true;
  const int rc = match_partitions_run(c, P, nhits);
  c->force_exact_blocks = keep_force;
  (void)hipStreamSynchronize(c->stream);
  c->pacc.release();
  c->pbest.release();
  c->pcnt.release();
  c->padj.release();
  c->pflags.release();
  c->pflags_tmp.release();
  c->block_acc.release();
  return rc;
}

int musc_hits_copy(musc_ctx* c, musc_hit* dst, uint64_t capacity, int dst_on_device) {
  if (!c) return 1;
  if (capacity < c->nhits) return fail(c, 2, "musc_hits_copy: capacity %llu < %llu hits",
                                       (unsigned long long)capacity, (unsigned long long)c->nhits);
  if (c->nhits == 0) return 0;
  if (!dst) return fail(c, 2, "musc_hits_copy: dst is NULL");
  HIPCHK(c, hipSetDevice(c->device));
  HIPCHK(c, hipMemcpyAsync(dst, c->hits.p, c->nhits * sizeof(musc_hit),
                           dst_on_device ? hipMemcpyDeviceToDevice : hipMemcpyDeviceToHost, c->stream));
  HIPCHK(c, hipStreamSynchronize(c->stream));
  return 0;
}


static ResData res_data(const musc_ctx* c) {
  ResData D;
  D.rd = c->rd;
  D.rdm = c->reads_have_x ? c->rdm : nullptr;
  D.db2 = c->db2;
  D.dbm2 = c->db_has_x ? c->dbm2 : nullptr;
  D.seq_off = c->seq_off;
  D.gtext = c->res_gtext;
  D.goff = c->res_goff;
  D.ttext = c->res_ttext;
  D.toff = c->res_toff;
  D.nreads = c->nreads;
  D.nseq = c->nseq;
  D.rw = c->rw;
  return D;
}

static int upload_text(musc_ctx* c, const char* what, const char* text, const uint64_t* offsets, uint64_t n, char** d_text, uint64_t** d_off) {
  for (uint64_t i = 0; i < n; i++)
    if (offsets[i + 1] < offsets[i]) return fail(c, 2, "%s: offsets decrease at item %llu", what, (unsigned long long)i);
  const uint64_t bytes = offsets[n];
  HIPCHK(c, hipMalloc((void**)d_text, bytes + 16));
  HIPCHK(c, hipMalloc((void**)d_off, (n + 1) * 8));
  if (bytes) HIPCHK(c, hipMemcpyAsync(*d_text, text, bytes, hipMemcpyHostToDevice, c->stream));
  HIPCHK(c, hipMemcpyAsync(*d_off, offsets, (n + 1) * 8, hipMemcpyHostToDevice, c->stream));
  HIPCHK(c, hipStreamSynchronize(c->stream));
  return 0;
}

int musc_results_set_gene_text(musc_ctx* c, const char* text, const uint64_t* offsets, const uint8_t* absent, uint32_t nseq) {
  if (!c) return 1;
  if (!offsets || (!text && offsets[nseq] != 0)) return fail(c, 2, "musc_results_set_gene_text: NULL input");
  if (!c->db2 || nseq != c->nseq)
    return fail(c, 2, "musc_results_set_gene_text: text of %u genes for a database of %u targets", nseq, c->nseq);
  HIPCHK(c, hipSetDevice(c->device));
  const bool list_ok = c->hits_current;
  drop_gene_text(c);
  c->hits_current = list_ok;
  int rc = upload_text(c, "musc_results_set_gene_text", text, offsets, nseq, &c->res_gtext, &c->res_goff);
  if (rc) {
    drop_gene_text(c);
    return rc;
  }
  std::vector<uint32_t> order;
  order.reserve(nseq);
  for (uint32_t g = 0; g < nseq; g++)
    if (!absent || !absent[g]) order.push_back(g);
  auto cmp = [&](uint32_t a, uint32_t b) {
    const uint64_t la = offsets[a + 1] - offsets[a], lb = offsets[b + 1] - offsets[b];
    const int d = memcmp(text + offsets[a], text + offsets[b], (size_t)std::min(la, lb));
    return d ? d : la < lb ? -1 : la > lb ? 1 : 0;
  };
  std::sort(order.begin(), order.end(), [&](uint32_t a, uint32_t b) { return cmp(a, b) < 0; });
  std::vector<uint32_t> rank(nseq, RES_ABSENT);
  uint32_t rk = 0;
  for (size_t i = 0; i < order.size(); i++) {
    if (i && cmp(order[i - 1], order[i]) != 0) rk++;
    rank[order[i]] = rk;
  }
  hipError_t e = hipMalloc((void**)&c->res_rank, (uint64_t)nseq * 4 + 16);
  if (e == hipSuccess) e = hipMemcpy(c->res_rank, rank.data(), (uint64_t)nseq * 4, hipMemcpyHostToDevice);
  if (e != hipSuccess) {
    drop_gene_text(c);
    return fail(c, 10, "musc_results_set_gene_text: %s", hipGetErrorString(e));
  }
  return 0;
}

int musc_results_set_read_text(musc_ctx* c, const char* text, const uint64_t* offsets, uint64_t nreads) {
  if (!c) return 1;
  if (!offsets || (!text && offsets[nreads] != 0)) return fail(c, 2, "musc_results_set_read_text: NULL input");
  if (nreads != c->nreads)
    return fail(c, 2, "musc_results_set_read_text: text of %llu reads, %llu are loaded", (unsigned long long)nreads, (unsigned long long)c->nreads);
  HIPCHK(c, hipSetDevice(c->device));
  drop_read_text(c);
  const int rc = upload_text(c, "musc_results_set_read_text", text, offsets, nreads, &c->res_ttext, &c->res_toff);
  if (rc) drop_read_text(c);
  return rc;
}

int musc_results_number_key(uint32_t pos, uint32_t nmiss, uint64_t* key) {
  if (!key || nmiss > 99999u) return 2;
  *key = res_number_key(pos, nmiss);
  return 0;
}

static int results_order_impl(musc_ctx* c, const musc_hit* hits, uint64_t n, int on_device) {
  const dim3 B256(256);
  auto grid = [](uint64_t k) { return dim3(std::max(1u, std::min(nblk(k, 256), MAX_GRID))); };
  const uint4* d_in = reinterpret_cast<const uint4*>(hits);
  TmpBufs B;
  if (!hits) {
    if (!c->hits_current)
      return fail(c, 2, "musc_results_order: the resident tuple list is not that of a pass over the reads and the database in hand");
    d_in = reinterpret_cast<const uint4*>(c->hits.p);
    n = c->nhits;
  } else if (on_device && ((uintptr_t)hits & 15u)) {
    return fail(c, 2, "musc_results_order: a device list must be 16-byte aligned");
  } else if (!on_device && n) {
    for (uint64_t i = 0; i < n; i++) {
      const musc_hit& h = hits[i];
      if (h.read_idx >= c->nreads || h.gene_idx >= c->nseq || h.nmiss > RES_MAX_NMISS ||
          h.pos > c->h_seq_off[(size_t)h.gene_idx + 1] - c->h_seq_off[h.gene_idx])
        return fail(c, 2, "musc_results_order: tuple %llu (read %u, gene %u, pos %u, nmiss %u) is outside the loaded reads and targets",
                    (unsigned long long)i, h.read_idx, h.gene_idx, h.pos, h.nmiss);
    }
    uint4* up = nullptr;
    HIPCHK(c, B.alloc(&up, n * 16));
    HIPCHK(c, hipMemcpyAsync(up, hits, n * 16, hipMemcpyHostToDevice, c->stream));
    d_in = up;
  }
  if (n >= 0xFFFFFFF0ull) return fail(c, 2, "musc_results_order: too many tuples for 32-bit line numbers");
  int rc;
  if ((rc = ensure(c, c->res_off, n + 1))) return rc;
  if (n == 0) {
    HIPCHK(c, hipMemsetAsync(c->res_off.p, 0, 8, c->stream));
    HIPCHK(c, hipStreamSynchronize(c->stream));
    return 0;
  }

  uint32_t *keep = nullptr, *excl = nullptr, *stmp = nullptr;
  uint4* a = nullptr;
  HIPCHK(c, B.alloc(&keep, n * 4));
  HIPCHK(c, B.alloc(&excl, n * 4));
  HIPCHK(c, B.alloc(&stmp, scan_tmp_elems(n) * 4));
  HIPCHK(c, hipMemsetAsync(c->d_flag, 0, 4, c->stream));
  hipLaunchKernelGGL(k_results_flag, grid(n), B256, 0, c->stream, d_in, n, c->nreads, c->nseq, c->seq_off, c->res_rank, keep, c->d_flag);
  HIPCHK(c, hipGetLastError());
  if ((rc = scan_u32(c, keep, excl, n, false, stmp))) return rc;
  uint32_t* const h32 = reinterpret_cast<uint32_t*>(c->h_pinned);
  HIPCHK(c, hipMemcpyAsync(h32, c->d_flag, 4, hipMemcpyDeviceToHost, c->stream));
  HIPCHK(c, hipMemcpyAsync(h32 + 1, excl + (n - 1), 4, hipMemcpyDeviceToHost, c->stream));
  HIPCHK(c, hipMemcpyAsync(h32 + 2, keep + (n - 1), 4, hipMemcpyDeviceToHost, c->stream));
  HIPCHK(c, hipStreamSynchronize(c->stream));
  if (h32[0] & 1u)
    return fail(c, 2, "musc_results_order: a tuple names a read, a target or a position outside the loaded reads and targets");
  const bool read_major = !(h32[0] & 2u);
  const uint64_t m = (uint64_t)h32[1] + h32[2];
  if ((rc = ensure(c, c->res_hits, std::max<uint64_t>(m, 1)))) return rc;
  uint4* const out = reinterpret_cast<uint4*>(c->res_hits.p);
  if (m == 0) {
    HIPCHK(c, hipMemsetAsync(c->res_off.p, 0, 8, c->stream));
    HIPCHK(c, hipStreamSynchronize(c->stream));
    return 0;
  }
  HIPCHK(c, B.alloc(&a, m * 16));
  hipLaunchKernelGGL(k_results_compact, grid(n), B256, 0, c->stream, d_in, keep, excl, n, a);
  HIPCHK(c, hipGetLastError());

  uint64_t *k0 = nullptr, *k1 = nullptr;
  uint32_t *p0 = nullptr, *p1 = nullptr;
  void* tmp = nullptr;
  size_t tmp_bytes = 0;
  auto sort_bufs = [&](TmpBufs& T, uint64_t k) -> int {
    HIPCHK(c, T.alloc(&k0, k * 8));
    HIPCHK(c, T.alloc(&k1, k * 8));
    HIPCHK(c, T.alloc(&p0, k * 4));
    HIPCHK(c, T.alloc(&p1, k * 4));
    tmp_bytes = 0;
    for (unsigned end : {32u, 33u, 60u, 63u}) {
      size_t tb = 0;
      HIPCHK(c, rocprim::radix_sort_pairs(nullptr, tb, k0, k1, p0, p1, (size_t)k, 0u, end, c->stream));
      tmp_bytes = std::max(tmp_bytes, tb);
    }
    HIPCHK(c, T.alloc(&tmp, tmp_bytes));
    return 0;
  };
  auto sort_pass = [&](const uint32_t* idx, uint64_t k, uint32_t what, unsigned end_bit) -> int {
    hipLaunchKernelGGL(k_results_keys, grid(k), B256, 0, c->stream, a, idx, p0, k, what, c->res_rank, c->rd, c->rw, c->db2,
                       c->db_has_x ? c->dbm2 : (const uint32_t*)nullptr, c->seq_off, k0);
    HIPCHK(c, hipGetLastError());
    HIPCHK(c, rocprim::radix_sort_pairs(tmp, tmp_bytes, k0, k1, p0, p1, (size_t)k, 0u, end_bit, c->stream));
    std::swap(p0, p1);
    return 0;
  };

  if (!read_major) {
    TmpBufs T;
    uint4* a2 = nullptr;
    if ((rc = sort_bufs(T, m))) return rc;
    HIPCHK(c, B.alloc(&a2, m * 16));
    hipLaunchKernelGGL(k_results_iota, grid(m), B256, 0, c->stream, p0, m);
    HIPCHK(c, hipGetLastError());
    if ((rc = sort_pass(nullptr, m, RES_KEY_READ, 32u))) return rc;
    hipLaunchKernelGGL(k_results_gather, grid(m), B256, 0, c->stream, a, p0, m, a2);
    HIPCHK(c, hipGetLastError());
    HIPCHK(c, hipStreamSynchronize(c->stream));
    a = a2;
  }

  uint32_t *multi = nullptr, *incl = nullptr, *idx = nullptr;
  HIPCHK(c, B.alloc(&multi, m * 4));
  HIPCHK(c, B.alloc(&incl, m * 4));
  HIPCHK(c, hipMemsetAsync(c->counters + CNT_SCRATCH, 0, 8, c->stream));
  hipLaunchKernelGGL(k_results_segments, grid(m), B256, 0, c->stream, a, m, c->rd, c->rw, multi, c->counters + CNT_SCRATCH);
  HIPCHK(c, hipGetLastError());
  if ((rc = scan_u32(c, multi, incl, m, true, stmp))) return rc;
  HIPCHK(c, hipMemcpyAsync(h32, incl + (m - 1), 4, hipMemcpyDeviceToHost, c->stream));
  HIPCHK(c, hipMemcpyAsync(c->h_pinned + 1, c->counters + CNT_SCRATCH, 8, hipMemcpyDeviceToHost, c->stream));
  HIPCHK(c, hipStreamSynchronize(c->stream));
  const uint64_t k = h32[0], maxlen = c->h_pinned[1];
  if (k == 0) {
    HIPCHK(c, hipMemcpyAsync(out, a, m * 16, hipMemcpyDeviceToDevice, c->stream));
  } else {
    TmpBufs T;
    if ((rc = sort_bufs(T, k))) return rc;
    HIPCHK(c, T.alloc(&idx, k * 4));
    hipLaunchKernelGGL(k_results_idx, grid(m), B256, 0, c->stream, multi, incl, m, idx);
    hipLaunchKernelGGL(k_results_iota, grid(k), B256, 0, c->stream, p0, k);
    HIPCHK(c, hipGetLastError());
    const uint32_t nw = (uint32_t)((maxlen + RES_BASES_PER_WORD - 1) / RES_BASES_PER_WORD);
    if ((rc = sort_pass(idx, k, RES_KEY_RANK, 32u))) return rc;
    if ((rc = sort_pass(idx, k, RES_KEY_NUMBER, 60u))) return rc;
    for (uint32_t w = nw; w-- > 0;)
      if ((rc = sort_pass(idx, k, RES_KEY_SPAN + w, 63u))) return rc;
    if ((rc = sort_pass(idx, k, RES_KEY_READ, 32u))) return rc;
    hipLaunchKernelGGL(k_results_place, grid(m), B256, 0, c->stream, a, multi, incl, idx, p0, m, out);
    HIPCHK(c, hipGetLastError());
    HIPCHK(c, hipStreamSynchronize(c->stream));
  }

  uint64_t* stmp64 = nullptr;
  HIPCHK(c, B.alloc(&stmp64, scan_tmp_elems(m + 1) * 8));
  hipLaunchKernelGGL(k_results_len, grid(m + 1), B256, 0, c->stream, out, m, res_data(c), c->res_off.p);
  HIPCHK(c, hipGetLastError());
  if ((rc = scan_u64(c, c->res_off.p, c->res_off.p, m + 1, stmp64))) return rc;
  HIPCHK(c, hipMemcpyAsync(c->h_pinned, c->res_off.p + m, 8, hipMemcpyDeviceToHost, c->stream));
  HIPCHK(c, hipStreamSynchronize(c->stream));
  c->res_n = m;
  c->res_bytes = c->h_pinned[0];
  return 0;
}

int musc_results_order(musc_ctx* c, const musc_hit* hits, uint64_t n, int on_device, uint64_t* nlines, uint64_t* nbytes) {
  if (!c) return 1;
  if (nlines) *nlines = 0;
  if (nbytes) *nbytes = 0;
  c->res_valid = false;
  c->res_n = c->res_bytes = 0;
  if (!c->db2 || !c->res_gtext || !c->res_rank) return fail(c, 2, "musc_results_order: no gene text (musc_results_set_gene_text)");
  if (c->up.active) return fail(c, 2, "musc_results_order: a streamed read load has not been matched yet");
  HIPCHK(c, hipSetDevice(c->device));
  c->ev_used = 0;
  hipEvent_t e0 = pool_event(c), e1 = pool_event(c);
  if (!e0 || !e1) return fail(c, 10, "hipEventCreate failed");
  HIPCHK(c, hipEventRecord(e0, c->stream));
  const int rc = results_order_impl(c, hits, n, on_device);
  if (rc) {
    (void)hipStreamSynchronize(c->stream);
    return rc;
  }
  HIPCHK(c, hipEventRecord(e1, c->stream));
  HIPCHK(c, hipStreamSynchronize(c->stream));
  c->res_ms_order = 0;
  (void)hipEventElapsedTime(&c->res_ms_order, e0, e1);
  c->res_ms_text = 0;
  c->res_valid = true;
  if (nlines) *nlines = c->res_n;
  if (nbytes) *nbytes = c->res_bytes;
  return 0;
}

int musc_results_hits(musc_ctx* c, musc_hit* dst, uint64_t capacity, int dst_on_device) {
  if (!c) return 1;
  if (!c->res_valid) return fail(c, 2, "musc_results_hits: no ordered list (musc_results_order)");
  if (capacity < c->res_n) return fail(c, 2, "musc_results_hits: capacity %llu < %llu tuples", (unsigned long long)capacity, (unsigned long long)c->res_n);
  if (c->res_n == 0) return 0;
  if (!dst) return fail(c, 2, "musc_results_hits: dst is NULL");
  HIPCHK(c, hipSetDevice(c->device));
  HIPCHK(c, hipMemcpyAsync(dst, c->res_hits.p, c->res_n * sizeof(musc_hit), dst_on_device ? hipMemcpyDeviceToDevice : hipMemcpyDeviceToHost, c->stream));
  HIPCHK(c, hipStreamSynchronize(c->stream));
  return 0;
}

static const uint64_t RES_STAGE_BYTES = 64ull << 20;
static const uint64_t RES_STAGE_LINES = 1ull << 20;

static void launch_render(musc_ctx* c, uint64_t l0, uint64_t l1, unsigned char* out) {
  const uint64_t nl = l1 - l0;
  const unsigned blocks = (unsigned)std::min<uint64_t>((nl + 3) / 4, 4 * MAX_GRID);
  hipLaunchKernelGGL(k_results_render, dim3(blocks), dim3(256), 0, c->stream, reinterpret_cast<const uint4*>(c->res_hits.p), c->res_off.p, l0, l1,
                     res_data(c), out, c->d_flag);
}

static int results_text_impl(musc_ctx* c, uint64_t l0, uint64_t l1, char* dst, uint64_t capacity, int dst_on_device, uint64_t* nbytes) {
  HIPCHK(c, hipMemcpyAsync(c->h_pinned, c->res_off.p + l0, 8, hipMemcpyDeviceToHost, c->stream));
  HIPCHK(c, hipMemcpyAsync(c->h_pinned + 1, c->res_off.p + l1, 8, hipMemcpyDeviceToHost, c->stream));
  HIPCHK(c, hipStreamSynchronize(c->stream));
  const uint64_t o0 = c->h_pinned[0], bytes = c->h_pinned[1] - o0;
  *nbytes = bytes;
  if (!dst) return 0;
  if (capacity < bytes)
    return fail(c, 2, "musc_results_text: capacity %llu < %llu bytes", (unsigned long long)capacity, (unsigned long long)bytes);
  HIPCHK(c, hipMemsetAsync(c->d_flag, 0, 4, c->stream));
  if (dst_on_device) {
    launch_render(c, l0, l1, reinterpret_cast<unsigned char*>(dst));
    HIPCHK(c, hipGetLastError());
    return 0;
  }
  std::vector<uint64_t> off;
  for (uint64_t b0 = l0; b0 < l1;) {
    const uint64_t b1 = std::min(l1, b0 + RES_STAGE_LINES);
    off.resize(b1 - b0 + 1);
    HIPCHK(c, hipMemcpyAsync(off.data(), c->res_off.p + b0, (b1 - b0 + 1) * 8, hipMemcpyDeviceToHost, c->stream));
    HIPCHK(c, hipStreamSynchronize(c->stream));
    for (uint64_t p0 = b0; p0 < b1;) {
      const uint64_t start = off[p0 - b0];
      uint64_t p1 = std::upper_bound(off.begin() + (p0 - b0), off.end(), start + RES_STAGE_BYTES) - off.begin() - 1 + b0;
      p1 = std::min(std::max(p1, p0 + 1), b1);
      const uint64_t pb = off[p1 - b0] - start;
      int rc = ensure(c, c->res_stage, std::max(pb, RES_STAGE_BYTES));
      if (rc) return rc;
      launch_render(c, p0, p1, c->res_stage.p);
      HIPCHK(c, hipGetLastError());
      HIPCHK(c, hipMemcpyAsync(dst + (start - o0), c->res_stage.p, pb, hipMemcpyDeviceToHost, c->stream));
      HIPCHK(c, hipStreamSynchronize(c->stream));
      p0 = p1;
    }
    b0 = b1;
  }
  return 0;
}

int musc_results_text(musc_ctx* c, uint64_t line0, uint64_t nlines, char* dst, uint64_t capacity, int dst_on_device, uint64_t* nbytes) {
  if (!c) return 1;
  if (!nbytes) return fail(c, 2, "musc_results_text: nbytes is NULL");
  *nbytes = 0;
  if (!c->res_valid) return fail(c, 2, "musc_results_text: no ordered list (musc_results_order)");
  if (line0 >= c->res_n || nlines == 0) return 0;
  const uint64_t l1 = nlines > c->res_n - line0 ? c->res_n : line0 + nlines;
  HIPCHK(c, hipSetDevice(c->device));
  c->ev_used = 0;
  hipEvent_t e0 = pool_event(c), e1 = pool_event(c);
  if (!e0 || !e1) return fail(c, 10, "hipEventCreate failed");
  HIPCHK(c, hipEventRecord(e0, c->stream));
  const int rc = results_text_impl(c, line0, l1, dst, capacity, dst_on_device, nbytes);
  const hipError_t er = hipEventRecord(e1, c->stream);
  uint32_t* const h_bad = reinterpret_cast<uint32_t*>(c->h_pinned + 2);
  *h_bad = 0;
  const hipError_t ef = rc == 0 && dst ? hipMemcpyAsync(h_bad, c->d_flag, 4, hipMemcpyDeviceToHost, c->stream) : hipSuccess;
  const hipError_t es = hipStreamSynchronize(c->stream);
  if (rc) return rc;
  HIPCHK(c, er);
  HIPCHK(c, ef);
  HIPCHK(c, es);
  if (*h_bad) {
    *nbytes = 0;
    return fail(c, 11, "musc_results_text: a line of the ordered list no longer fits the reads, the database or the texts in hand");
  }
  float ms = 0;
  if (dst && hipEventElapsedTime(&ms, e0, e1) == hipSuccess) c->res_ms_text += ms;
  return 0;
}

int musc_results_last_ms(musc_ctx* c, float* ms_order, float* ms_text) {
  if (!c) return 1;
  if (ms_order) *ms_order = c->res_ms_order;
  if (ms_text) *ms_text = c->res_ms_text;
  return 0;
}

extern "C++" {
template <class Pack>
static int download_chunks(musc_ctx* c, uint64_t n, size_t elem, const void* src, void* dst, Pack pack) {
  if (!c->up.s_up) HIPCHK(c, hipStreamCreateWithFlags(&c->up.s_up, hipStreamNonBlocking));
  const uint64_t smallest = std::min<uint64_t>(c->batch_reads, 1u << 18);
  uint64_t sz = std::max<uint64_t>(n / 32, smallest);
  size_t k = 0;
  for (uint64_t t0 = 0; t0 < n; k++, sz *= 4) {
    const uint64_t t1 = n - t0 <= sz + sz / 2 ? n : t0 + sz;
    if (k == c->dl_ev.size()) {
      hipEvent_t e = nullptr;
      HIPCHK(c, hipEventCreateWithFlags(&e, hipEventDisableTiming));
      c->dl_ev.push_back(e);
    }
    pack(t0, t1);
    HIPCHK(c, hipGetLastError());
    HIPCHK(c, hipEventRecord(c->dl_ev[k], c->stream));
    HIPCHK(c, hipStreamWaitEvent(c->up.s_up, c->dl_ev[k], 0));
    HIPCHK(c, hipMemcpyAsync((char*)dst + t0 * elem, (const char*)src + t0 * elem, (t1 - t0) * elem, hipMemcpyDeviceToHost, c->up.s_up));
    t0 = t1;
  }
  return 0;
}
}

static int download_end(musc_ctx* c, uint32_t* h_bad, void* tail_dst, const void* tail_src, uint64_t tail_bytes) {
  hipError_t e = hipMemcpyAsync(h_bad, c->d_flag, 4, hipMemcpyDeviceToHost, c->stream);
  if (e == hipSuccess && tail_bytes) {
    hipStream_t st = c->up.s_up ? c->up.s_up : c->stream;
    if (st != c->stream && (e = hipEventRecord(c->ev_join, c->stream)) == hipSuccess) e = hipStreamWaitEvent(st, c->ev_join, 0);
    if (e == hipSuccess) e = hipMemcpyAsync(tail_dst, tail_src, tail_bytes, hipMemcpyDeviceToHost, st);
  }
  const hipError_t e1 = hipStreamSynchronize(c->stream);
  const hipError_t e2 = c->up.s_up ? hipStreamSynchronize(c->up.s_up) : hipSuccess;
  if (e == hipSuccess) e = e1 != hipSuccess ? e1 : e2;
  if (e != hipSuccess) {
    (void)hipGetLastError();
    return fail(c, 10, "copying the tuples to the host failed: %s", hipGetErrorString(e));
  }
  return 0;
}

static int check_pack_bits(musc_ctx* c, const int32_t* bits, PackBits* b) {
  if (!bits) return fail(c, 2, "bits is NULL");
  int sum = 0;
  for (int i = 0; i < 4; i++) {
    if (bits[i] < 1 || bits[i] > 32) return fail(c, 2, "field width %d outside 1..32", bits[i]);
    sum += bits[i];
  }
  if (sum > 64) return fail(c, 2, "field widths add up to %d > 64 bits", sum);
  *b = PackBits{bits[0], bits[1], bits[2], bits[3]};
  return 0;
}

int musc_hits_copy_packed(musc_ctx* c, uint64_t* dst, uint64_t capacity, int dst_on_device, uint64_t read_base,
                          const int32_t* bits) {
  if (!c) return 1;
  PackBits b;
  int rc = check_pack_bits(c, bits, &b);
  if (rc) return rc;
  if (capacity < c->nhits) return fail(c, 2, "musc_hits_copy_packed: capacity %llu < %llu hits",
                                       (unsigned long long)capacity, (unsigned long long)c->nhits);
  if (c->nhits == 0) return 0;
  if (!dst) return fail(c, 2, "musc_hits_copy_packed: dst is NULL");
  HIPCHK(c, hipSetDevice(c->device));
  uint64_t* out = dst;
  if (!dst_on_device) {
    if ((rc = ensure(c, c->packed, c->nhits))) return rc;
    out = c->packed.p;
  }
  HIPCHK(c, hipMemsetAsync(c->d_flag, 0, 4, c->stream));
  const uint4* const hits = reinterpret_cast<const uint4*>(c->hits.p);
  auto pack = [&](uint64_t t0, uint64_t t1) {
    hipLaunchKernelGGL(k_pack_hits, dim3(std::min(nblk(t1 - t0, 256), MAX_GRID)), dim3(256), 0, c->stream, hits + t0, t1 - t0,
                       read_base, b, out + t0, c->d_flag);
  };
  uint32_t* const h_bad = reinterpret_cast<uint32_t*>(c->h_pinned);
  if (dst_on_device) {
    pack(0, c->nhits);
    HIPCHK(c, hipGetLastError());
    HIPCHK(c, hipMemcpyAsync(h_bad, c->d_flag, 4, hipMemcpyDeviceToHost, c->stream));
    HIPCHK(c, hipStreamSynchronize(c->stream));
  } else {
    rc = download_chunks(c, c->nhits, 8, out, dst, pack);
    const int rc_end = download_end(c, h_bad, nullptr, nullptr, 0);
    if (rc || rc_end) return rc ? rc : rc_end;
  }
  const uint32_t bad = *h_bad;
  if (bad) return fail(c, 8, "musc_hits_copy_packed: a tuple field does not fit its width (%d/%d/%d/%d bits)",
                       b.read, b.gene, b.pos, b.nmiss);
  return 0;
}

int musc_hits_copy_compact(musc_ctx* c, uint32_t* words, uint64_t words_cap, uint8_t* counts, uint64_t counts_cap,
                           int dst_on_device, const int32_t* bits) {
  if (!c) return 1;
  if (!bits) return fail(c, 2, "bits is NULL");
  int sum = 0;
  for (int i = 0; i < 3; i++) {
    if (bits[i] < 1 || bits[i] > 30) return fail(c, 2, "field width %d outside 1..30", bits[i]);
    sum += bits[i];
  }
  if (sum > 32) return fail(c, 2, "field widths add up to %d > 32 bits", sum);
  if (words_cap < c->nhits) return fail(c, 2, "musc_hits_copy_compact: room for %llu tuples < %llu",
                                        (unsigned long long)words_cap, (unsigned long long)c->nhits);
  if (counts_cap < c->nreads) return fail(c, 2, "musc_hits_copy_compact: room for %llu reads < %llu",
                                          (unsigned long long)counts_cap, (unsigned long long)c->nreads);
  if ((c->nhits && !words) || (c->nreads && !counts)) return fail(c, 2, "musc_hits_copy_compact: NULL destination");
  HIPCHK(c, hipSetDevice(c->device));
  const PackBits b{0, bits[0], bits[1], bits[2]};
  uint32_t* dw = words;
  uint8_t* dc = counts;
  if (!dst_on_device) {
    int rc = ensure(c, c->packed, (c->nhits * 4 + c->nreads + 15) / 8 + 2);
    if (rc) return rc;
    dw = reinterpret_cast<uint32_t*>(c->packed.p);
    dc = reinterpret_cast<uint8_t*>(dw + c->nhits);
  }
  HIPCHK(c, hipMemsetAsync(c->d_flag, 0, 4, c->stream));
  if (c->nreads) HIPCHK(c, hipMemsetAsync(dc, 0, c->nreads, c->stream));
  const uint4* const hits = reinterpret_cast<const uint4*>(c->hits.p);
  uint32_t* const h_bad = reinterpret_cast<uint32_t*>(c->h_pinned);
  if (dst_on_device) {
    if (c->nhits) {
      hipLaunchKernelGGL(k_pack_compact, dim3(std::min(nblk(c->nhits, 256), MAX_GRID)), dim3(256), 0, c->stream, hits, c->nhits,
                         b, dw, dc, c->d_flag);
      HIPCHK(c, hipGetLastError());
    }
    HIPCHK(c, hipMemcpyAsync(h_bad, c->d_flag, 4, hipMemcpyDeviceToHost, c->stream));
    HIPCHK(c, hipStreamSynchronize(c->stream));
  } else {
    int rc = download_chunks(c, c->nhits, 4, dw, words, [&](uint64_t t0, uint64_t t1) {
      hipLaunchKernelGGL(k_pack_compact_range, dim3(std::min(nblk(t1 - t0, 256), MAX_GRID)), dim3(256), 0, c->stream, hits,
                         c->nhits, t0, t1, b, dw, dc, c->d_flag);
    });
    const int rc_end = download_end(c, h_bad, counts, dc, c->nreads);
    if (rc || rc_end) return rc ? rc : rc_end;
  }
  const uint32_t bad = *h_bad;
  if (bad & 4u) return fail(c, 12, "internal: the hit list is not read-major");
  if (bad) return fail(c, 8, "musc_hits_copy_compact: %s", (bad & 1u) ? "a tuple field does not fit its width"
                                                                      : "a read has more than 255 tuples");
  return 0;
}

int musc_hits_unpack(musc_ctx* c, const uint64_t* src, uint64_t n, int on_device, const int32_t* bits, musc_hit* dst) {
  if (!c) return 1;
  PackBits b;
  int rc = check_pack_bits(c, bits, &b);
  if (rc) return rc;
  if (n == 0) return 0;
  if (!src || !dst) return fail(c, 2, "musc_hits_unpack: NULL pointer");
  if (!on_device) {
    for (uint64_t i = 0; i < n; i++) {
      uint64_t v = src[i];
      dst[i].nmiss = (uint32_t)(v & ((1ull << b.nmiss) - 1ull));
      v >>= b.nmiss;
      dst[i].pos = (uint32_t)(v & ((1ull << b.pos) - 1ull));
      v >>= b.pos;
      dst[i].gene_idx = (uint32_t)(v & ((1ull << b.gene) - 1ull));
      v >>= b.gene;
      dst[i].read_idx = (uint32_t)v;
    }
    return 0;
  }
  HIPCHK(c, hipSetDevice(c->device));
  hipLaunchKernelGGL(k_unpack_hits, dim3(std::min(nblk(n, 256), MAX_GRID)), dim3(256), 0, c->stream, src, n, b,
                     reinterpret_cast<uint4*>(dst));
  HIPCHK(c, hipGetLastError());
  HIPCHK(c, hipStreamSynchronize(c->stream));
  return 0;
}

int musc_match(musc_ctx* c, const musc_params* P, musc_hit** hits, uint64_t* nhits) {
  if (!c) return 1;
  if (!hits || !nhits) return fail(c, 2, "musc_match: NULL output pointer");
  *hits = nullptr;
  *nhits = 0;
  uint64_t n = 0;
  int rc = musc_match_device(c, P, &n);
  if (rc) return rc;
  musc_hit* h = (musc_hit*)malloc(sizeof(musc_hit) * (n ? n : 1));
  if (!h) return fail(c, 7, "out of host memory for %llu hits", (unsigned long long)n);
  rc = musc_hits_copy(c, h, n, 0);
  if (rc) {
    free(h);
    return rc;
  }
  *hits = h;
  *nhits = n;
  return 0;
}

void musc_free_hits(musc_hit* hits) { free(hits); }

int musc_overflow_probes(musc_ctx* c, uint32_t** read_idx, uint32_t** window, uint64_t* n) {
  if (!c) return 1;
  if (!read_idx || !window || !n) return fail(c, 2, "musc_overflow_probes: NULL output pointer");
  *read_idx = *window = nullptr;
  *n = 0;
  if (c->stats.n_overflow_blocks == 0 || c->stats.n_overflow_blocks == ~0ull) return 0;
  if (!c->last_exact_blocks || !c->block_table.p) return fail(c, 4, "no exact block counters from the last pass");
  HIPCHK(c, hipSetDevice(c->device));
  uint64_t cap = 1u << 20;
  for (;;) {
    TmpBufs B;
    uint2* d_out = nullptr;
    HIPCHK(c, B.alloc(&d_out, cap * sizeof(uint2)));
    HIPCHK(c, hipMemsetAsync(c->counters + CNT_BATCH, 0, 8, c->stream));
    const dim3 grid(std::min(nblk(c->nreads, 256), MAX_GRID)), block(256);
    switch (c->rw) {
      case 4: hipLaunchKernelGGL((k_hot_probes<4>), grid, block, 0, c->stream, c->rd, c->rdm, c->nreads, c->rw, c->d_pp, c->block_table.p, c->last_max_matches, d_out, cap, c->counters + CNT_BATCH); break;
      case 8: hipLaunchKernelGGL((k_hot_probes<8>), grid, block, 0, c->stream, c->rd, c->rdm, c->nreads, c->rw, c->d_pp, c->block_table.p, c->last_max_matches, d_out, cap, c->counters + CNT_BATCH); break;
      case 12: hipLaunchKernelGGL((k_hot_probes<12>), grid, block, 0, c->stream, c->rd, c->rdm, c->nreads, c->rw, c->d_pp, c->block_table.p, c->last_max_matches, d_out, cap, c->counters + CNT_BATCH); break;
      case 16: hipLaunchKernelGGL((k_hot_probes<16>), grid, block, 0, c->stream, c->rd, c->rdm, c->nreads, c->rw, c->d_pp, c->block_table.p, c->last_max_matches, d_out, cap, c->counters + CNT_BATCH); break;
      default: hipLaunchKernelGGL((k_hot_probes<0>), grid, block, 0, c->stream, c->rd, c->rdm, c->nreads, c->rw, c->d_pp, c->block_table.p, c->last_max_matches, d_out, cap, c->counters + CNT_BATCH); break;
    }
    hipError_t e = hipGetLastError();
    if (e == hipSuccess) e = hipMemcpyAsync(c->h_pinned, c->counters + CNT_BATCH, 8, hipMemcpyDeviceToHost, c->stream);
    if (e == hipSuccess) e = hipStreamSynchronize(c->stream);
    if (e != hipSuccess) return fail(c, 10, "musc_overflow_probes: %s", hipGetErrorString(e));
    const uint64_t found = c->h_pinned[0];
    if (found > cap) {
      cap = found + 16;
      continue;
    }
    std::vector<uint2> h(found ? found : 1);
    if (found) e = hipMemcpy(h.data(), d_out, found * sizeof(uint2), hipMemcpyDeviceToHost);
    if (e != hipSuccess) return fail(c, 10, "musc_overflow_probes: %s", hipGetErrorString(e));
    uint32_t* r = (uint32_t*)malloc(sizeof(uint32_t) * (found ? found : 1));
    uint32_t* w = (uint32_t*)malloc(sizeof(uint32_t) * (found ? found : 1));
    if (!r || !w) {
      free(r);
      free(w);
      return fail(c, 7, "musc_overflow_probes: out of host memory");
    }
    for (uint64_t j = 0; j < found; j++) {
      r[j] = h[j].x;
      w[j] = h[j].y;
    }
    *read_idx = r;
    *window = w;
    *n = found;
    return 0;
  }
}

void musc_free_u32(uint32_t* p) { free(p); }

int musc_get_stats(musc_ctx* c, musc_stats* out) {
  if (!c || !out) return 1;
  *out = c->stats;
  return 0;
}

int musc_last_instance(const musc_ctx* c, uint32_t* out) {
  if (!c || !out) return 1;
  for (int i = 0; i < MUSC_INSTANCE_WORDS; i++) out[i] = c->last_inst[i];
  return 0;
}

int musc_instances(uint32_t* out, uint32_t capacity, uint32_t* n) {
  if (!n) return 1;
  std::vector<uint32_t> ids;
  auto add = [&](uint32_t id) {
    if (id && std::find(ids.begin(), ids.end(), id) == ids.end()) ids.push_back(id);
  };
  static const int strides[] = {4, 8, 12, 16, 20};
  for (int rw : strides) {
    for (int kind : {MK_LANE, MK_DMA})
      for (int sg = 0; sg <= MUSC_SPEC_GEOMS; sg++)
        for (int wide = 0; wide < 2; wide++)
          for (int W = 1; W <= CTX_MAX_W; W++)
            for (int xm = 0; xm < 3; xm++) add(match_instance(kind, sg, rw, wide != 0, W, xm).id);
    add(screen_t_instance(rw).id);
    for (int mask = 0; mask < 2; mask++)
      for (int W = 2; W <= 3; W++) {
        for (int lines = 0; lines < 2; lines++) add(screen_instance(rw, mask != 0, W, lines != 0).id);
        add(confirm_instance(rw, mask != 0, W).id);
      }
  }
  *n = (uint32_t)ids.size();
  if (out)
    for (uint32_t i = 0; i < capacity && i < ids.size(); i++) out[i] = ids[i];
  return 0;
}

int musc_stream_plan(uint64_t nreads, uint32_t fixed_len, uint32_t batch_reads, uint64_t* ends, uint8_t* is_batch_end,
                     uint64_t capacity, uint64_t* n, uint64_t* planned_batches) {
  if (!n || fixed_len > 65535 || nreads >= 0xFFFFFFF0ull) return 1;
  if (batch_reads < 1 || batch_reads > (16u << 20)) batch_reads = 16u << 20;
  StreamPlan sp;
  stream_plan(nreads, batch_reads, &sp);
  *n = sp.piece_end.size();
  if (planned_batches) *planned_batches = std::max<uint64_t>(sp.batch_end.size(), 1);
  size_t b = 0;
  for (size_t i = 0; i < sp.piece_end.size() && i < capacity; i++) {
    if (ends) ends[i] = sp.piece_end[i];
    while (b < sp.batch_end.size() && sp.batch_end[b] < sp.piece_end[i]) b++;
    if (is_batch_end) is_batch_end[i] = b < sp.batch_end.size() && sp.batch_end[b] == sp.piece_end[i];
  }
  return 0;
}

int musc_gather(musc_ctx* const* ctxs, int n, const uint64_t* read_base, musc_hit** hits, uint64_t* nhits) {
  if (!ctxs || n < 1 || !hits || !nhits) return 1;
  uint64_t total = 0;
  for (int i = 0; i < n; i++) {
    if (!ctxs[i]) return 1;
    total += ctxs[i]->nhits;
  }
  musc_hit* h = (musc_hit*)malloc(sizeof(musc_hit) * (total ? total : 1));
  if (!h) return fail(ctxs[0], 7, "musc_gather: out of host memory");
  uint64_t o = 0;
  for (int i = 0; i < n; i++) {
    musc_ctx* c = ctxs[i];
    int rc = musc_hits_copy(c, h + o, c->nhits, 0);
    if (rc) {
      free(h);
      return rc;
    }
    const uint64_t base = read_base ? read_base[i] : 0;
    for (uint64_t j = 0; j < c->nhits; j++) h[o + j].read_idx += (uint32_t)base;
    o += c->nhits;
  }
  *hits = h;
  *nhits = total;
  return 0;
}

namespace {
struct RcclApi {
  void* lib = nullptr;
  decltype(&ncclCommInitAll) CommInitAll = nullptr;
  decltype(&ncclCommDestroy) CommDestroy = nullptr;
  decltype(&ncclGroupStart) GroupStart = nullptr;
  decltype(&ncclGroupEnd) GroupEnd = nullptr;
  decltype(&ncclSend) Send = nullptr;
  decltype(&ncclRecv) Recv = nullptr;
  decltype(&ncclGetErrorString) GetErrorString = nullptr;
  std::string err;
  std::map<std::vector<int>, std::vector<ncclComm_t>> comms;
};
std::mutex g_rccl_mu;

RcclApi* rccl_api() {
  static RcclApi api;
  if (api.lib || !api.err.empty()) return &api;
  std::string first_err;
  std::vector<std::string> names;
  if (const char* e = getenv("MUSC_RCCL_LIB")) names.push_back(e);
  else names = {"/opt/rocm/lib/librccl.so.1", "librccl.so.1", "librccl.so"};
  for (const std::string& name : names) {
    (void)dlerror();
    api.lib = dlopen(name.c_str(), RTLD_NOW | RTLD_LOCAL);
    if (api.lib) break;
    const char* e = dlerror();
    if (first_err.empty()) first_err = e ? e : "not found";
  }
  if (!api.lib) {
    api.err = std::string("cannot load librccl: ") + first_err;
    return &api;
  }
#define MUSC_RCCL_SYM(FIELD, NAME)                                   \
  api.FIELD = reinterpret_cast<decltype(api.FIELD)>(dlsym(api.lib, NAME)); \
  if (!api.FIELD && api.err.empty()) api.err = std::string("librccl lacks ") + NAME;
  MUSC_RCCL_SYM(CommInitAll, "ncclCommInitAll")
  MUSC_RCCL_SYM(CommDestroy, "ncclCommDestroy")
  MUSC_RCCL_SYM(GroupStart, "ncclGroupStart")
  MUSC_RCCL_SYM(GroupEnd, "ncclGroupEnd")
  MUSC_RCCL_SYM(Send, "ncclSend")
  MUSC_RCCL_SYM(Recv, "ncclRecv")
  MUSC_RCCL_SYM(GetErrorString, "ncclGetErrorString")
#undef MUSC_RCCL_SYM
  return &api;
}
}

int musc_rccl_probe(char* msg, uint64_t cap) {
  std::lock_guard<std::mutex> lock(g_rccl_mu);
  RcclApi* api = rccl_api();
  if (msg && cap) {
    strncpy(msg, api->err.c_str(), cap - 1);
    msg[cap - 1] = 0;
  }
  return api->err.empty() ? 0 : 20;
}

__global__ void k_rebase_reads(uint4* __restrict__ h, uint64_t n, uint32_t base) {
  for (uint64_t i = (uint64_t)blockIdx.x * blockDim.x + threadIdx.x; i < n; i += (uint64_t)gridDim.x * blockDim.x) h[i].x += base;
}

int musc_gather_rccl(musc_ctx* const* ctxs, int n, const uint64_t* read_base, musc_hit** hits, uint64_t* nhits) {
  if (!ctxs || n < 1 || !hits || !nhits) return 1;
  *hits = nullptr;
  *nhits = 0;
  uint64_t total = 0;
  std::vector<uint64_t> off(n + 1, 0);
  std::vector<int> devs(n);
  for (int i = 0; i < n; i++) {
    if (!ctxs[i]) return 1;
    devs[i] = ctxs[i]->device;
    off[i] = total;
    total += ctxs[i]->nhits;
  }
  off[n] = total;
  musc_ctx* c0 = ctxs[0];
  for (int i = 0; i < n; i++)
    for (int j = i + 1; j < n; j++)
      if (devs[i] == devs[j]) return fail(c0, 2, "musc_gather_rccl: contexts %d and %d share device %d", i, j, devs[i]);
  std::lock_guard<std::mutex> lock(g_rccl_mu);
  std::vector<ncclComm_t>* comms = nullptr;
  RcclApi* api = nullptr;
  if (n > 1) {
    api = rccl_api();
    if (!api->err.empty()) return fail(c0, 20, "musc_gather_rccl: %s", api->err.c_str());
    auto it = api->comms.find(devs);
    if (it == api->comms.end()) {
      std::vector<ncclComm_t> cs(n);
      const ncclResult_t r = api->CommInitAll(cs.data(), n, devs.data());
      if (r != ncclSuccess) return fail(c0, 20, "musc_gather_rccl: ncclCommInitAll: %s", api->GetErrorString(r));
      it = api->comms.emplace(devs, cs).first;
    }
    comms = &it->second;
  }
  HIPCHK(c0, hipSetDevice(c0->device));
  int rc = ensure(c0, c0->gathered, total ? total : 1);
  if (rc) return rc;
  if (c0->nhits)
    HIPCHK(c0, hipMemcpyAsync(c0->gathered.p, c0->hits.p, c0->nhits * sizeof(musc_hit), hipMemcpyDeviceToDevice, c0->stream));
  if (n > 1) {
    ncclResult_t r = api->GroupStart();
    for (int i = 1; i < n && r == ncclSuccess; i++) {
      if (!ctxs[i]->nhits) continue;
      const size_t bytes = ctxs[i]->nhits * sizeof(musc_hit);
      (void)hipSetDevice(ctxs[i]->device);
      r = api->Send(ctxs[i]->hits.p, bytes, ncclUint8, 0, (*comms)[i], ctxs[i]->stream);
      if (r != ncclSuccess) break;
      (void)hipSetDevice(c0->device);
      r = api->Recv(c0->gathered.p + off[i], bytes, ncclUint8, i, (*comms)[0], c0->stream);
    }
    const ncclResult_t r2 = api->GroupEnd();
    if (r == ncclSuccess) r = r2;
    if (r != ncclSuccess) return fail(c0, 20, "musc_gather_rccl: %s", api->GetErrorString(r));
  }
  HIPCHK(c0, hipSetDevice(c0->device));
  for (int i = 0; i < n; i++) {
    const uint64_t base = read_base ? read_base[i] : 0;
    if (!base || !ctxs[i]->nhits) continue;
    hipLaunchKernelGGL(k_rebase_reads, dim3(std::min(nblk(ctxs[i]->nhits, 256), MAX_GRID)), dim3(256), 0, c0->stream,
                       reinterpret_cast<uint4*>(c0->gathered.p + off[i]), ctxs[i]->nhits, (uint32_t)base);
    HIPCHK(c0, hipGetLastError());
  }
  for (int i = 1; i < n; i++) {
    HIPCHK(ctxs[i], hipSetDevice(ctxs[i]->device));
    HIPCHK(ctxs[i], hipStreamSynchronize(ctxs[i]->stream));
  }
  HIPCHK(c0, hipSetDevice(c0->device));
  musc_hit* h = (musc_hit*)malloc(sizeof(musc_hit) * (total ? total : 1));
  if (!h) return fail(c0, 7, "musc_gather_rccl: out of host memory");
  hipError_t e = hipSuccess;
  if (total) e = hipMemcpyAsync(h, c0->gathered.p, total * sizeof(musc_hit), hipMemcpyDeviceToHost, c0->stream);
  if (e == hipSuccess) e = hipStreamSynchronize(c0->stream);
  if (e != hipSuccess) {
    free(h);
    return fail(c0, 10, "musc_gather_rccl: %s", hipGetErrorString(e));
  }
  *hits = h;
  *nhits = total;
  return 0;
}

}

#include "kernels_fastq.hpp"
#include "muscato_prep.hpp"
```

muscato_amd/csrc/muscato_pass.hpp:

```cpp
#pragma once

namespace {

bool screen_lane(const musc_ctx* c, bool mask) {
  return c->idx_lines && !mask && !c->rdm && (c->rw == 4 || c->rw == 8 || c->rw == 12 || c->rw == 16) && !c->env.screen_wg;
}

template <class F>
auto by_rw(int rw, F&& f) {
  switch (rw) {
    case 4: return f(std::integral_constant<int, 4>{});
    case 8: return f(std::integral_constant<int, 8>{});
    case 12: return f(std::integral_constant<int, 12>{});
    case 16: return f(std::integral_constant<int, 16>{});
    default: return f(std::integral_constant<int, 0>{});
  }
}

typedef decltype(&k_screen_t<8>) screen_t_fn;
typedef decltype(&k_screen<0, false, false, false>) screen_fn;
typedef decltype(&k_confirm<0, false, false>) confirm_fn;
template <class Fn>
struct Inst {
  Fn fn;
  uint32_t id;
};
constexpr uint32_t inst_id(uint32_t family, int rw, int a = 0, int b = 0, int c = 0, int d = 0) {
  return family | (uint32_t)rw << 8 | (uint32_t)a << 16 | (uint32_t)b << 20 | (uint32_t)c << 24 | (uint32_t)d << 28;
}
#define INST_SCREEN_T(RW) Inst<screen_t_fn>{k_screen_t<RW>, inst_id(MUSC_INST_SCREEN_T, RW)}
#define INST_SCREEN(RW, M, ONE, LN) Inst<screen_fn>{k_screen<RW, M, ONE, LN>, inst_id(MUSC_INST_SCREEN, RW, M, ONE, LN)}
#define INST_CONFIRM(RW, M, W2) Inst<confirm_fn>{k_confirm<RW, M, W2>, inst_id(MUSC_INST_CONFIRM, RW, M, W2)}

Inst<screen_t_fn> screen_t_instance(int rw) {
  return by_rw(rw, [](auto r) -> Inst<screen_t_fn> {
    if constexpr (decltype(r)::value != 0) return INST_SCREEN_T(decltype(r)::value);
    else return Inst<screen_t_fn>{nullptr, 0};
  });
}

Inst<screen_fn> screen_instance(int rw, bool mask, int W, bool lines) {
  const int m = mask, one = W <= 2, ln = lines;
  return by_rw(rw, [&](auto r) -> Inst<screen_fn> {
    constexpr int RW = decltype(r)::value;
    static const Inst<screen_fn> k[2][2][2] = {
        {{INST_SCREEN(RW, false, false, false), INST_SCREEN(RW, false, false, true)}, {INST_SCREEN(RW, false, true, false), INST_SCREEN(RW, false, true, true)}},
        {{INST_SCREEN(RW, true, false, false), INST_SCREEN(RW, true, false, true)}, {INST_SCREEN(RW, true, true, false), INST_SCREEN(RW, true, true, true)}}};
    return k[m][one][ln];
  });
}

Inst<confirm_fn> confirm_instance(int rw, bool mask, int W) {
  const int m = mask, w2 = W <= 2;
  return by_rw(rw, [&](auto r) -> Inst<confirm_fn> {
    constexpr int RW = decltype(r)::value;
    static const Inst<confirm_fn> k[2][2] = {{INST_CONFIRM(RW, false, false), INST_CONFIRM(RW, false, true)}, {INST_CONFIRM(RW, true, false), INST_CONFIRM(RW, true, true)}};
    return k[m][w2];
  });
}

unsigned screen_grid(musc_ctx* c, uint32_t n, bool mask) {
  unsigned g = std::min(nblk(n, TILE), MAX_GRID);
  if (screen_lane(c, mask)) {
    if (!c->scrt_resident || c->scrt_rw != c->rw) {
      int per_cu = 0, ncu = 0;
      const void* fn = reinterpret_cast<const void*>(screen_t_instance(c->rw).fn);
      if (hipOccupancyMaxActiveBlocksPerMultiprocessor(&per_cu, fn, 64, 0) != hipSuccess || per_cu < 1) { (void)hipGetLastError(); per_cu = 8; }
      if (hipDeviceGetAttribute(&ncu, hipDeviceAttributeMultiprocessorCount, c->device) != hipSuccess || ncu < 1) ncu = 256;
      c->scrt_resident = (unsigned)per_cu * (unsigned)ncu;
      c->scrt_rw = c->rw;
    }
    g = std::min(g, std::min(c->scrt_resident, MAX_GRID));
  }
  return g;
}

enum PassOutcome {
  PASS_DONE = 0,
  PASS_RERUN_CAREFUL,
  PASS_RERUN_EXACT,
  PASS_RERUN_NO_GRAPH,
};

struct PassPlan {
  const musc_params* P = nullptr;
  PathParams pp;
  uint64_t max_matches = 0, planned_batches = 0;
  int block_mode = 0;
  uint32_t block_thr = 0;
  bool sized = false;
  match_kernel_t kern = nullptr;
  unsigned resident = 0;
  bool mask = false;
};

struct BatchCursor {
  const StreamPlan* plan = nullptr;
  uint32_t bsz = 0;
  uint32_t reads_at(uint64_t r0, uint64_t nreads) const {
    return (uint32_t)(plan ? stream_plan_batch(*plan, r0) : std::min<uint64_t>(bsz, nreads - r0));
  }
  void halve(uint32_t n) {
    bsz = n / 2;
    plan = nullptr;
  }
};
constexpr uint64_t BATCH_OFFSET_CAP = 1ull << 31;

constexpr uint64_t FIRST_PASS_TUPLES_PER_READ = 2, FIRST_PASS_DESC_PER_READ = 4, FIRST_PASS_DESC_MIN = 1024;

struct PassClock {
  Timer tm;
  hipEvent_t ev0, ev1;
  explicit PassClock(musc_ctx* c) : tm(c), ev0(pool_event(c)), ev1(pool_event(c)) {}
};

void launch_screen(musc_ctx* c, const PassPlan& pl, uint64_t r0, uint32_t n) {
  const dim3 sgrid(screen_grid(c, n, pl.mask));
  auto& b = c->bs[c->cur];
  if (screen_lane(c, pl.mask)) {
    const auto k = screen_t_instance(c->rw);
    c->last_inst[1] = k.id;
    hipLaunchKernelGGL(k.fn, sgrid, dim3(64), 0, c->stream, c->rd, r0, n, c->d_pp, c->nmiss_tab.p,
                       reinterpret_cast<const LineBucket*>(c->idx_T), c->idx_E, b.cdesc.p, b.cdesc.cap, b.rvalid.p, b.wb.p,
                       b.tbase.p, b.tcount.p, c->counters + CNT_BATCH, c->counters + CNT_FLAGS);
  } else {
    const auto k = screen_instance(c->rw, c->rdm != nullptr, pl.pp.W, c->idx_lines);
    c->last_inst[1] = k.id;
    hipLaunchKernelGGL(k.fn, sgrid, dim3(TILE), 0, c->stream, c->rd, c->rdm, r0, n, c->rw, c->d_pp,
                       c->nmiss_tab.p, c->idx_T, c->idx_E, b.cdesc.p, b.cdesc.cap, b.rvalid.p, b.wb.p, b.tbase.p, b.tcount.p,
                       c->counters + CNT_BATCH, c->counters + CNT_FLAGS);
  }
}

void launch_confirm(musc_ctx* c, const PassPlan& pl, uint64_t r0, uint32_t n) {
  const dim3 grid(std::min(nblk(n, TILE), MAX_GRID));
  static_assert((1u << 24) / TILE / MAX_GRID <= CONF_TILES, "a k_confirm workgroup keeps its tile list in LDS");
  const size_t lds = pl.block_mode ? (size_t)TILE * pl.pp.W * 4 : 0;
  auto& b = c->bs[c->cur];
  const auto k = confirm_instance(c->rw, pl.mask, pl.pp.W);
  c->last_inst[2] = k.id;
  hipLaunchKernelGGL(k.fn, grid, dim3(TILE), lds, c->s_confirm, c->rd, c->rdm, c->db2, c->dbm2,
                     c->dbx, r0, n, c->rw, c->d_pp, c->nmiss_tab.p, b.cdesc.p, b.rvalid.p, c->p_nx.p, b.tbase.p, b.tcount.p,
                     b.wb.p, pl.block_mode, pl.block_thr, c->block_table.p, c->seq_off, c->stage.p, c->tcount2.p,
                     c->counters);
}

}

static size_t match_dyn_lds(int kind, int W, int block_mode) {
  if (kind == MK_DMA) return block_mode == 1 ? (size_t)(4u << MATCHG_SKETCH_BITS) : 0u;
  const size_t wcnt = (size_t)TILE * W * 4 * (kind == MK_LANE ? 2 : 1);
  return block_mode ? wcnt + (block_mode == 1 ? (4u << MATCH_SKETCH_BITS) : 0u) : 0u;
}

typedef Inst<match_kernel_t> MatchInst;
#define INST_T(RW, W, XM, WD, SG) MatchInst{k_match_t<RW, W, XM, WD, SG>, inst_id(MUSC_INST_MATCH_T, RW, W, XM, WD, SG)}
#define INST_G(RW, SG) MatchInst{k_match_g<RW, SG>, inst_id(MUSC_INST_MATCH_G, RW, 0, 0, 0, SG)}
template <int RW, bool WD>
static MatchInst lane_instance(int W, int xm) {
  static const MatchInst k[4][3] = {
      {INST_T(RW, 1, 0, WD, 0), INST_T(RW, 1, 1, WD, 0), INST_T(RW, 1, 2, WD, 0)},
      {INST_T(RW, 2, 0, WD, 0), INST_T(RW, 2, 1, WD, 0), INST_T(RW, 2, 2, WD, 0)},
      {INST_T(RW, 3, 0, WD, 0), INST_T(RW, 3, 1, WD, 0), INST_T(RW, 3, 2, WD, 0)},
      {INST_T(RW, 4, 0, WD, 0), INST_T(RW, 4, 1, WD, 0), INST_T(RW, 4, 2, WD, 0)}};
  return k[(W >= 1 && W <= 3 ? W : 4) - 1][xm];
}

static MatchInst match_instance(int kind, int spec_geom, int rw, bool wide, int W, int xm) {
  if (kind == MK_DMA) return spec_geom == 1 ? INST_G(8, 1) : INST_G(8, 0);
  if (spec_geom == 1) return INST_T(8, 2, 0, false, 1);
  return by_rw(rw, [&](auto r) -> MatchInst {
    constexpr int RW = decltype(r)::value;
    if constexpr (RW == 0) return MatchInst{nullptr, 0};
    else if (wide) return lane_instance<RW, true>(W, xm);
    else if constexpr (RW <= 12) return lane_instance<RW, false>(W, xm);
    else return MatchInst{nullptr, 0};
  });
}

static unsigned match_resident(musc_ctx* c, match_kernel_t kern, int W, int block_mode) {
  int per_cu = 0, ncu = 0;
  const size_t lds = match_dyn_lds(match_kind(c, W), W, block_mode);
  const void* fn = reinterpret_cast<const void*>(kern);
  hipError_t e = hipOccupancyMaxActiveBlocksPerMultiprocessor(&per_cu, fn, TILE, lds);
  if (e != hipSuccess || per_cu < 1) { (void)hipGetLastError(); per_cu = 2; }
  hipFuncAttributes fa;
  if (hipFuncGetAttributes(&fa, fn) == hipSuccess) {
    const size_t total = ((size_t)fa.sharedSizeBytes + lds + 2047) / 2048 * 2048;
    const int fit = total ? (int)((160u << 10) / total) : per_cu;
    if (fit >= 1 && fit < per_cu) per_cu = fit;
  } else {
    (void)hipGetLastError();
  }
  if (hipDeviceGetAttribute(&ncu, hipDeviceAttributeMultiprocessorCount, c->device) != hipSuccess || ncu < 1) ncu = 256;
  unsigned resident = (unsigned)per_cu * (unsigned)ncu;
  if (c->env.debug_grid >= 1 && (unsigned)c->env.debug_grid < resident) resident = (unsigned)c->env.debug_grid;
  return resident;
}

static void launch_match(musc_ctx* c, const PassPlan& pl, uint64_t r0, uint32_t n, unsigned ngrid) {
  const size_t lds = match_dyn_lds(match_kind(c, pl.pp.W), pl.pp.W, pl.block_mode);
  const uint32_t* const rdx = c->reads_have_x ? (const uint32_t*)c->rdx.p : (const uint32_t*)nullptr;
  hipLaunchKernelGGL(pl.kern, dim3(ngrid), dim3(TILE), lds, c->stream, c->rd, r0, n, c->d_mp, c->nmiss_tab.p, c->ctx_T,
                     c->ctx_E, c->stage.p, c->stage.cap, c->spill.p, c->spill.cap, c->bs[0].tbase.p, c->tcount2.p,
                     pl.block_mode, pl.block_thr, c->block_table.p, c->counters, rdx);
}

template <int SG>
static bool spec_geom_equals(const MatchParams& mp) {
  typedef SpecGeom<SG> G;
  if (mp.W != G::nwin || mp.ww != G::ww || mp.CL != G::CL || mp.min_dinuc != G::min_dinuc || mp.direct != 1 || mp.bits != 2 * G::ww) return false;
  for (int k = 0; k < G::nwin; k++)
    if (mp.win[k] != G::win[k] || mp.need[k] != (1u << k) - 1u) return false;
  return true;
}
static int spec_geom_matches(const musc_ctx* c, const MatchParams& mp) {
  if (c->env.no_spec) return 0;
  if (c->rw != 8 || c->idx_wide || c->db_has_x || c->reads_have_x) return 0;
  return spec_geom_equals<1>(mp) ? 1 : 0;
}

static int match_setup(musc_ctx* c, PassPlan* pl) {
  const PathParams& pp = pl->pp;
  if (c->rw != 4 && c->rw != 8 && c->rw != 12 && !(c->rw == 16 && c->idx_wide))
    return fail(c, 12, "internal: record stride %d on the context path", c->rw);
  static thread_local MatchParams mp;
  memset(&mp, 0, sizeof mp);
  mp.W = pp.W; mp.ww = pp.ww; mp.min_dinuc = pp.min_dinuc; mp.bits = pp.bits; mp.direct = pp.direct;
  mp.mmtol = pp.mmtol; mp.apply_mmtol = pp.apply_mmtol; mp.max_len = pp.max_len; mp.CL = c->idx_CL;
  mp.q1zero_mask = pp.q1zero_mask;
  mp.seq_off = c->db_has_x ? c->seq_off : nullptr;
  mp.dbm2 = c->db_has_x ? c->dbm2 : nullptr;
  for (int k = 0; k < pp.W && k < CTX_MAX_W; k++) mp.win[k] = pp.win[k];
  match_tables(mp);
  c->spec_geom = spec_geom_matches(c, mp);
  c->stats.match_variant = (match_kind(c, pp.W) == MK_DMA ? 4u : 2u) + (c->spec_geom ? 1u : 0u);
  if (!c->h_mp_valid || memcmp(&mp, &c->h_mp, sizeof mp) != 0) {
    c->h_mp = mp;
    HIPCHK(c, hipMemcpyAsync(c->d_mp, &c->h_mp, sizeof mp, hipMemcpyHostToDevice, c->stream));
    HIPCHK(c, hipStreamSynchronize(c->stream));
    c->h_mp_valid = true;
  }
  const int xm = c->db_has_x ? 2 : c->reads_have_x ? 1 : 0;
  const MatchInst inst = match_instance(match_kind(c, pp.W), c->spec_geom, c->rw, c->idx_wide != 0, pp.W, xm);
  pl->kern = inst.fn;
  c->last_inst[0] = inst.id;
  if (!pl->kern) return fail(c, 12, "internal: no fused kernel instance for record stride %d, %d windows", c->rw, pp.W);
  pl->resident = match_resident(c, pl->kern, pp.W, pl->block_mode);
  return 0;
}

static int pass_setup(musc_ctx* c, const musc_params* P, PassPlan* pl, BatchCursor* cur) {
  int rc = 0;
  const float keep_index_ms = c->stats.ms_index_build;
  memset(&c->stats, 0, sizeof c->stats);
  c->stats.ms_index_build = keep_index_ms;
  c->stats.n_reads = c->nreads;
  c->nhits = 0;

  pl->P = P;
  PathParams& pp = pl->pp;
  memset(&pp, 0, sizeof pp);
  pp.W = P->n_windows;
  pp.ww = P->window_width;
  pp.min_dinuc = P->min_dinuc;
  pp.bits = c->idx_bits;
  pp.direct = c->idx_direct;
  pp.mmtol = P->mmtol > 0xFFFF ? 0xFFFF : P->mmtol;
  pp.apply_mmtol = P->apply_mmtol;
  pp.wide = c->wide;
  pp.max_len = (int32_t)c->max_len;
  for (int k = 0; k < pp.W; k++) {
    pp.win[k] = P->windows[k];
    if (P->windows[k] == 0) pp.q1zero_mask |= 1u << k;
  }

  if (c->nm_pmatch != P->pmatch || c->nm_mmp1 != P->max_mismatch_p1 || c->nm_maxlen != c->max_len || !c->nmiss_tab.p) {
    std::vector<uint16_t> tab((size_t)c->max_len + 2);
    for (uint32_t L = 0; L < tab.size(); L++) {
      volatile double a = 1.0 - P->pmatch;
      volatile double b = a * (double)L;
      long long v = (long long)b;
      if (P->max_mismatch_p1 > 0) v = P->max_mismatch_p1 - 1;
      tab[L] = (uint16_t)std::min<long long>(std::max<long long>(v, 0), 0xFFFE);
    }
    if ((rc = ensure(c, c->nmiss_tab, tab.size()))) return rc;
    HIPCHK(c, hipMemcpyAsync(c->nmiss_tab.p, tab.data(), tab.size() * 2, hipMemcpyHostToDevice, c->stream));
    HIPCHK(c, hipStreamSynchronize(c->stream));
    c->nm_pmatch = P->pmatch;
    c->nm_mmp1 = P->max_mismatch_p1;
    c->nm_maxlen = c->max_len;
  }

  HIPCHK(c, hipMemsetAsync(c->counters, 0, CNT_PASS_WORDS * sizeof(unsigned long long), c->stream));
  pl->planned_batches = c->up.active ? std::max<uint64_t>(c->up.plan.batch_end.size(), 1)
                                     : (c->nreads + c->batch_reads - 1) / c->batch_reads + 1;
  pl->max_matches = P->max_matches > 0 ? (uint64_t)P->max_matches : 0x7FFFFFFFull;
  if (P->n_shards > 1) pl->max_matches /= (uint64_t)P->n_shards;
  auto thr_for = [&](uint64_t grid) { return (uint32_t)std::min<uint64_t>(pl->max_matches / (pl->planned_batches * grid), 0x7FFFFFFFull); };
  const uint32_t thr_host = thr_for(MAX_GRID);
  const bool known_exact = c->exact_epoch == c->data_epoch && memcmp(&c->exact_params, P, sizeof *P) == 0;
  pl->block_mode = P->skip_block_check ? 0 : (c->force_exact_blocks || known_exact || thr_host < 2 ? 2 : 1);
  if (pl->block_mode == 2) {
    if ((rc = ensure(c, c->block_table, 1ull << BLOCK_TABLE_BITS))) return rc;
    HIPCHK(c, hipMemsetAsync(c->block_table.p, 0, (1ull << BLOCK_TABLE_BITS) * 4, c->stream));
  }
  if (!c->h_pp_valid || memcmp(&pp, &c->h_pp, sizeof pp) != 0) {
    c->h_pp = pp;
    HIPCHK(c, hipMemcpyAsync(c->d_pp, &c->h_pp, sizeof pp, hipMemcpyHostToDevice, c->stream));
    HIPCHK(c, hipStreamSynchronize(c->stream));
    c->h_pp_valid = true;
  }
  c->stats.index_kind = c->idx_kind == 1 ? (c->idx_wide ? 2u : 1u) : (c->idx_lines ? 3u : 0u);
  c->last_inst[0] = c->last_inst[1] = c->last_inst[2] = 0;
  c->last_inst[3] = (uint32_t)pl->block_mode | (c->force_exact_blocks ? 0x100u : 0u);
  c->stats.index_bytes = c->idx_kind == 1
                             ? ((1ull << c->idx_bits) + 1) * sizeof(CtxBucket) + ctx_entries_bytes(c->idx_novf + 16, c->idx_wide)
                             : ((1ull << c->idx_bits) + 1) * (c->idx_lines ? sizeof(LineBucket) : sizeof(Bucket)) + (c->idx_novf + 16) * sizeof(uint4);
  if (c->idx_kind == 1) {
    if ((rc = match_setup(c, pl))) return rc;
    const uint32_t thr_resident = thr_for(pl->resident);
    if (pl->block_mode == 1 && thr_resident < 2) {
      pl->block_mode = 2;
      c->last_inst[3] = 2u | (c->force_exact_blocks ? 0x100u : 0u);
      if (!c->block_table.p && (rc = ensure(c, c->block_table, 1ull << BLOCK_TABLE_BITS))) return rc;
    }
    pl->block_thr = thr_resident;
  } else {
    pl->block_thr = thr_host;
  }
  pl->mask = c->reads_have_x || c->db_has_x;

  pl->sized = c->sized_epoch == c->data_epoch && c->sized_exact_blocks == (pl->block_mode == 2) &&
              memcmp(&c->sized_params, P, sizeof *P) == 0 && !c->env.debug_sync;
  cur->bsz = pl->sized ? c->sized_bsz : c->batch_reads;
  cur->plan = c->up.active && !pl->sized ? &c->up.plan : nullptr;
  return 0;
}

static int pass_peek(musc_ctx* c) {
  HIPCHK(c, hipMemcpyAsync(c->h_pinned, c->counters, CNT_WORDS * 8, hipMemcpyDeviceToHost, c->stream));
  HIPCHK(c, hipStreamSynchronize(c->stream));
  return 0;
}

static int ensure_tiles(musc_ctx* c, musc_ctx::BatchSet& b, uint32_t ntiles) {
  int rc;
  if ((rc = ensure(c, b.tbase, (uint64_t)ntiles + 1)) || (rc = ensure(c, c->scan_tmp, scan_tmp_elems((uint64_t)ntiles + 1))) ||
      (rc = ensure(c, c->tcount2, (uint64_t)ntiles + 1)) || (rc = ensure(c, c->tpre, (uint64_t)ntiles + 1)))
    return rc;
  return 0;
}

static int launch_compact(musc_ctx* c, Timer& tm, decltype(&k_compact) compact, dim3 grid, uint32_t ntiles, const uint32_t* tbase,
                          hipStream_t st) {
  tm.begin(4, st);
  tm.begin(1, st);
  const int rc = scan_u32(c, c->tcount2.p, c->tpre.p, (uint64_t)ntiles + 1, false, c->scan_tmp.p, st);
  if (rc) return rc;
  tm.end(1, st);
  hipLaunchKernelGGL(compact, grid, dim3(256), 0, st, ntiles, tbase, c->tcount2.p, c->tpre.p, c->stage.p,
                     reinterpret_cast<uint4*>(c->hits.p), c->hits.cap, c->counters);
  HIPCHK(c, hipGetLastError());
  hipLaunchKernelGGL(k_advance, dim3(1), dim3(64), 0, st, c->tpre.p, ntiles, c->counters);
  HIPCHK(c, hipGetLastError());
  tm.end(4, st);
  return 0;
}

static int pass_close(musc_ctx* c, const PassPlan& pl, hipEvent_t ev1) {
  if (pl.block_mode == 2) {
    hipLaunchKernelGGL(k_block_overflow, dim3(1024), dim3(256), 0, c->stream, c->block_table.p, (uint32_t)pl.max_matches,
                       c->counters);
    HIPCHK(c, hipGetLastError());
  }
  if (ev1) HIPCHK(c, hipEventRecord(ev1, c->stream));
  HIPCHK(c, hipMemcpyAsync(c->h_pinned, c->counters, CNT_WORDS * 8, hipMemcpyDeviceToHost, c->stream));
  return 0;
}

static int pass_verdict(musc_ctx* c, const PassPlan& pl, const BatchCursor& cur, const uint64_t* tot, PassClock& clk,
                        PassOutcome* what) {
  const bool fused = c->idx_kind == 1;
  c->last_pp = pl.pp;
  c->last_max_matches = (uint32_t)pl.max_matches;
  c->last_exact_blocks = pl.block_mode == 2;
  HIPCHK(c, hipStreamSynchronize(c->stream));
  const uint64_t* h = c->h_pinned;
  if (h[CNT_FLAGS] & FLAG_SPEC_REFUSED)
    return fail(c, 12, "internal: the kernel instance specialised for geometry %d refused this run's parameters", c->spec_geom);
  if (h[CNT_FLAGS]) {
    if (!pl.sized) return fail(c, 12, "internal: a capacity guard fired although every batch was sized (flags %llu)",
                               (unsigned long long)h[CNT_FLAGS]);
    *what = PASS_RERUN_CAREFUL;
    return 0;
  }
  if (pl.sized) tot = h + CNT_BATCH;
  c->stats.n_accepted = h[CNT_ACCEPTED];
  c->stats.n_hits = c->nhits = h[CNT_HITS];
  c->stats.n_overflow_blocks = pl.block_mode ? h[CNT_OVF_BLOCKS] : ~0ull;
  if (pl.block_mode == 1 && (h[CNT_HOT] || c->stats.n_batches > pl.planned_batches)) {
    *what = PASS_RERUN_EXACT;
    return 0;
  }
  c->stats.ms_screen = clk.tm.total(0);
  c->stats.ms_scan = clk.tm.total(1);
  c->stats.ms_confirm = clk.tm.total(3);
  c->stats.ms_select = clk.tm.total(4);
  (void)hipEventElapsedTime(&c->stats.ms_total, clk.ev0, clk.ev1);
  const uint64_t rec_b = (2 * (uint64_t)c->max_len + 7) / 8;
  c->stats.n_candidates = tot[fused ? MB_CAND : SB_CAND];
  c->stats.n_read_windows = tot[fused ? MB_WINDOWS : SB_WINDOWS];
  if (fused) {
    c->stats.n_pairs = tot[MB_CMP];
    c->stats.n_overflow_entries = tot[MB_OVF];
    const uint64_t ent_b = c->idx_wide ? sizeof(CtxEntryW) : sizeof(CtxEntry);
    c->stats.match_bytes = c->nreads * rec_b + tot[MB_WINDOWS] * sizeof(CtxBucket) + tot[MB_OVF] * ent_b + 16 * c->stats.n_hits;
    c->stats.match_bytes_strict = c->nreads * rec_b + tot[MB_WINDOWS] * 8 + tot[MB_CAND] * ent_b + 16 * c->stats.n_hits;
  } else {
    c->stats.n_descriptors = tot[SB_PAIRS];
    c->stats.n_pairs = tot[SB_PAIRS] + tot[SB_TWO];
    c->stats.confirm_bytes = c->stats.n_descriptors * (12 + rec_b + rec_b + 1) + 16 * c->stats.n_hits;
    if (!pl.sized && c->env.pipeline) {
      int rc;
      if ((rc = ensure(c, c->bs[1].wb, c->bs[0].wb.cap)) || (rc = ensure(c, c->bs[1].rvalid, c->bs[0].rvalid.cap)) ||
          (rc = ensure(c, c->bs[1].tbase, c->bs[0].tbase.cap)) || (rc = ensure(c, c->bs[1].tcount, c->bs[0].tcount.cap)) ||
          (rc = ensure(c, c->bs[1].cdesc, c->bs[0].cdesc.cap)))
        return rc;
    }
  }
  c->sized_epoch = cur.plan ? 0 : c->data_epoch;
  c->sized_params = *pl.P;
  c->sized_exact_blocks = pl.block_mode == 2;
  c->sized_bsz = cur.bsz;
  return 0;
}

static int pass_fused(musc_ctx* c, const PassPlan& pl, BatchCursor cur, PassOutcome* what) {
  int rc = 0;
  const bool sized = pl.sized;
  const bool use_graph = sized && c->env.graph > 0 && !c->graph_failed;
  if (!sized && c->graph_exec) {
    (void)hipGraphExecDestroy(c->graph_exec);
    c->graph_exec = nullptr;
  }
  for (int attempt = 0;; attempt++) {
    if (attempt > 40) return fail(c, 12, "internal: the context pass did not converge on buffer sizes");
    PassClock clk(c);
    if (!clk.ev0 || !clk.ev1) return fail(c, 10, "hipEventCreate failed");
    const bool replay = use_graph && c->graph_exec && c->graph_epoch == c->data_epoch && c->graph_block_mode == pl.block_mode &&
                        memcmp(&c->graph_params, pl.P, sizeof *pl.P) == 0;
    const bool capture = use_graph && !replay;
    if (capture && c->graph_exec) {
      (void)hipGraphExecDestroy(c->graph_exec);
      c->graph_exec = nullptr;
    }
    clk.tm.off = capture || replay;
    CaptureGuard cap;
    if (capture) {
      if (cap.begin(c->stream) != hipSuccess) {
        (void)hipGetLastError();
        *what = PASS_RERUN_NO_GRAPH;
        return 0;
      }
    } else if (!replay) {
      HIPCHK(c, hipEventRecord(clk.ev0, c->stream));
    }
    uint64_t tot[CNT_BATCH_WORDS] = {0}, r0 = 0;
    c->stats.n_batches = c->stats.match_launches = 0;
    bool again = false;
    if (!replay) {
      HIPCHK(c, hipMemsetAsync(c->counters, 0, CNT_WORDS * sizeof(unsigned long long), c->stream));
      if (pl.block_mode == 2) HIPCHK(c, hipMemsetAsync(c->block_table.p, 0, (1ull << BLOCK_TABLE_BITS) * 4, c->stream));
    }
    while (!replay && r0 < c->nreads) {
      const uint32_t n = cur.reads_at(r0, c->nreads);
      const uint32_t ntiles = nblk(n, WT);
      const uint64_t sgrid = std::min<uint64_t>(nblk(n, TILE), pl.resident);
      const uint64_t swaves = sgrid * (TILE / 64);
      if (!sized) {
        if ((rc = ensure_tiles(c, c->bs[0], ntiles)) ||
            (rc = ensure(c, c->stage, std::max<uint64_t>(FIRST_PASS_TUPLES_PER_READ * n, swaves * 64))) ||
            (rc = ensure(c, c->spill, swaves * 32)))
          return rc;
        HIPCHK(c, hipMemsetAsync(c->counters + CNT_BATCH, 0, CNT_BATCH_WORDS * sizeof(unsigned long long), c->stream));
      }
      if ((rc = upload_prepare(c, r0, n, c->stream))) return rc;
      clk.tm.begin(0);
      {
        Range rg("k_match");
        launch_match(c, pl, r0, n, (unsigned)sgrid);
      }
      HIPCHK(c, hipGetLastError());
      clk.tm.end(0);
      c->stats.match_launches++;
      c->stats.n_batches++;
      if (!sized) {
        if ((rc = pass_peek(c))) return rc;
        const uint64_t* h = c->h_pinned;
        const uint64_t need_stage = h[CNT_BATCH + MB_STAGE_MAX] * swaves, need_spill = 2 * h[CNT_BATCH + MB_SPILL_MAX] * swaves;
        if (need_stage > BATCH_OFFSET_CAP) {
          if (n == 1) return fail(c, 6, "one read has %llu tuples (> 2^31)", (unsigned long long)h[CNT_BATCH + MB_STAGE_MAX]);
          cur.halve(n);
          again = true;
          break;
        }
        if (h[CNT_FLAGS] & FLAG_SPEC_REFUSED)
          return fail(c, 12, "internal: the kernel instance specialised for geometry %d refused this run's parameters", c->spec_geom);
        if (h[CNT_FLAGS] || need_stage > c->stage.cap || need_spill > c->spill.cap) {
          if (need_stage > c->stage.cap && (rc = ensure(c, c->stage, need_stage + need_stage / 4 + swaves))) return rc;
          if (need_spill > c->spill.cap && (rc = ensure(c, c->spill, need_spill + need_spill / 4 + swaves))) return rc;
          again = true;
          break;
        }
        for (int i = 0; i < CNT_BATCH_WORDS; i++) tot[i] += h[CNT_BATCH + i];
        if ((rc = ensure(c, c->hits, h[CNT_HITS] + h[CNT_BATCH + MB_TUPLES], true))) return rc;
      }
      Range rgc("scan + k_compact_w");
      const dim3 cgrid(std::min(nblk(ntiles, 4), 4u * MAX_GRID));
      if ((rc = launch_compact(c, clk.tm, k_compact_w, cgrid, ntiles, c->bs[0].tbase.p, c->stream))) return rc;
      r0 += n;
    }
    if (again) continue;
    if (!replay && (rc = pass_close(c, pl, capture ? nullptr : clk.ev1))) return rc;
    if (capture) {
      hipGraph_t g = nullptr;
      hipError_t ge = cap.end(&g);
      if (ge == hipSuccess) ge = hipGraphInstantiate(&c->graph_exec, g, nullptr, nullptr, 0);
      if (g) (void)hipGraphDestroy(g);
      if (ge != hipSuccess) {
        (void)hipGetLastError();
        c->graph_exec = nullptr;
        *what = PASS_RERUN_NO_GRAPH;
        return 0;
      }
      c->graph_epoch = c->data_epoch;
      c->graph_params = *pl.P;
      c->graph_block_mode = pl.block_mode;
      c->graph_batches = c->stats.n_batches;
    }
    if (capture || replay) {
      c->stats.n_batches = c->stats.match_launches = c->graph_batches;
      HIPCHK(c, hipEventRecord(clk.ev0, c->stream));
      HIPCHK(c, hipGraphLaunch(c->graph_exec, c->stream));
      HIPCHK(c, hipEventRecord(clk.ev1, c->stream));
    }
    return pass_verdict(c, pl, cur, tot, clk, what);
  }
}

static int pass_two_kernel(musc_ctx* c, const PassPlan& pl, BatchCursor cur, PassOutcome* what) {
  int rc = 0;
  PassClock clk(c);
  if (!clk.ev0 || !clk.ev1) return fail(c, 10, "hipEventCreate failed");
  HIPCHK(c, hipEventRecord(clk.ev0, c->stream));

  if (pl.mask && !c->rdm && c->nreads) {
    const uint64_t words = c->nreads * (uint64_t)c->rw;
    HIPCHK(c, hipMalloc((void**)&c->rdm, words * 4 + 256));
    HIPCHK(c, hipMemsetAsync(c->rdm, 0, words * 4 + 256, c->stream));
  }
  if (pl.mask && !c->dbm2) {
    HIPCHK(c, hipMalloc((void**)&c->dbm2, (c->db_words + 64) * 4));
    HIPCHK(c, hipMemsetAsync(c->dbm2, 0, (c->db_words + 64) * 4, c->stream));
    if ((rc = db_xblocks(c))) return rc;
  }

  const bool sized = pl.sized;
  uint64_t tot[CNT_BATCH_WORDS] = {0}, r0 = 0;
  if (sized) HIPCHK(c, hipMemsetAsync(c->counters + CNT_BATCH, 0, CNT_BATCH_WORDS * sizeof(unsigned long long), c->stream));
  const bool piped = sized && c->env.pipeline && c->nreads > cur.bsz && c->bs[1].cdesc.cap >= c->bs[0].cdesc.cap;
  hipStream_t sA = c->stream, sB = piped ? c->stream2 : c->stream;
  c->s_confirm = sB;
  c->cur = 0;
  if (piped) {
    HIPCHK(c, hipEventRecord(c->ev_join, sA));
    HIPCHK(c, hipStreamWaitEvent(sB, c->ev_join, 0));
  }
  uint32_t batch_no = 0;
  while (r0 < c->nreads) {
    const uint32_t n = cur.reads_at(r0, c->nreads);
    if (piped) {
      c->cur = (int)(batch_no & 1u);
      if (batch_no >= 2) HIPCHK(c, hipStreamWaitEvent(sA, c->ev_free[c->cur], 0));
    }
    auto& b = c->bs[c->cur];
    const uint32_t ntiles = nblk(n, TILE);
    uint64_t total = 1;
    if (!sized) {
      if ((rc = ensure_tiles(c, b, ntiles)) || (rc = ensure(c, b.tcount, (uint64_t)ntiles + 1)) ||
          (rc = ensure(c, b.wb, (uint64_t)n * pl.pp.W)) || (rc = ensure(c, b.rvalid, (uint64_t)n + 1)) ||
          (rc = ensure(c, b.cdesc, std::max<uint64_t>(FIRST_PASS_DESC_PER_READ * n, FIRST_PASS_DESC_MIN))))
        return rc;
      HIPCHK(c, hipMemsetAsync(c->counters + CNT_BATCH, 0, CNT_BATCH_WORDS * sizeof(unsigned long long), c->stream));
    }

    if ((rc = upload_prepare(c, r0, n, c->stream))) return rc;
    clk.tm.begin(0);
    {
      Range rg("k_screen");
      launch_screen(c, pl, r0, n);
    }
    HIPCHK(c, hipGetLastError());
    clk.tm.end(0);
    if (piped) {
      HIPCHK(c, hipEventRecord(c->ev_ready[c->cur], sA));
      HIPCHK(c, hipStreamWaitEvent(sB, c->ev_ready[c->cur], 0));
    }
    if (!sized) {
      if ((rc = pass_peek(c))) return rc;
      const uint64_t* h = c->h_pinned;
      total = h[CNT_BATCH + SB_PAIRS];
      const uint64_t sgrid = screen_grid(c, n, pl.mask);
      const uint64_t region = h[CNT_BATCH + SB_DESC_MAX], need = region * sgrid;
      if (need > BATCH_OFFSET_CAP || region > b.cdesc.cap / sgrid) {
        if (need > BATCH_OFFSET_CAP) {
          if (n == 1) return fail(c, 6, "one read has %llu candidate pairs (> 2^31)", (unsigned long long)total);
          cur.halve(n);
        } else if ((rc = ensure(c, b.cdesc, need + need / 8 + sgrid))) {
          return rc;
        }
        HIPCHK(c, hipMemsetAsync(c->counters + CNT_FLAGS, 0, 8, c->stream));
        continue;
      }
      for (int i = 0; i < CNT_BATCH_WORDS; i++) tot[i] += h[CNT_BATCH + i];
      if ((rc = ensure(c, c->p_nx, b.cdesc.cap))) return rc;
      if ((rc = ensure(c, c->stage, b.cdesc.cap))) return rc;
      if ((rc = ensure(c, c->hits, h[CNT_HITS] + total, true))) return rc;
    }
    c->stats.n_batches++;

    if (total) {
      clk.tm.begin(3, sB);
      {
        Range rg("k_confirm");
        launch_confirm(c, pl, r0, n);
      }
      HIPCHK(c, hipGetLastError());
      clk.tm.end(3, sB);
      c->stats.confirm_launches++;

      Range rgc("scan + k_compact");
      const dim3 cgrid(std::min(nblk(n, TILE), MAX_GRID));
      if ((rc = launch_compact(c, clk.tm, k_compact, cgrid, ntiles, b.tbase.p, sB))) return rc;
    }
    if (piped) HIPCHK(c, hipEventRecord(c->ev_free[c->cur], sB));
    r0 += n;
    batch_no++;
  }
  if (piped) {
    HIPCHK(c, hipEventRecord(c->ev_join, sB));
    HIPCHK(c, hipStreamWaitEvent(sA, c->ev_join, 0));
  }
  c->cur = 0;
  c->s_confirm = c->stream;
  if ((rc = pass_close(c, pl, clk.ev1))) return rc;
  return pass_verdict(c, pl, cur, tot, clk, what);
}

static int match_index_pass(musc_ctx* c, const musc_params* P, uint64_t* nhits) {
  bool forced_exact = false;
  int rc = 0;
  for (;;) {
    PassPlan pl;
    BatchCursor cur;
    PassOutcome what = PASS_DONE;
    if ((rc = ensure_index(c, P, c->max_len))) break;
    if (nhits) *nhits = 0;
    if ((rc = pass_setup(c, P, &pl, &cur))) break;
    rc = c->idx_kind == 1 ? pass_fused(c, pl, cur, &what) : pass_two_kernel(c, pl, cur, &what);
    if (rc || what == PASS_DONE) break;
    if (what == PASS_RERUN_CAREFUL) {
      c->sized_epoch = 0;
    } else if (what == PASS_RERUN_NO_GRAPH) {
      c->graph_failed = true;
    } else {
      c->force_exact_blocks = forced_exact = true;
      c->exact_epoch = c->data_epoch;
      c->exact_params = *P;
    }
  }
  if (forced_exact) c->force_exact_blocks = false;
  if (!rc && nhits) *nhits = c->nhits;
  return rc;
}

static int match_device_impl(musc_ctx* c, const musc_params* P, uint64_t* nhits) {
  Range rg_pass("musc_match_device");
  int rc = check_params(c, P);
  if (rc) return rc;
  if (!c->db2) return fail(c, 4, "no database loaded");
  if (!c->rd && c->nreads) return fail(c, 4, "no reads loaded");
  HIPCHK(c, hipSetDevice(c->device));
  if ((rc = plan_partitions(c, P, c->max_len))) return rc;
  c->cur_part = 0;
  if (c->part_first.size() > 2) return match_partitioned(c, P, nhits);
  return match_index_pass(c, P, nhits);
}

extern "C" int musc_match_device(musc_ctx* c, const musc_params* P, uint64_t* nhits) {
  if (!c) return 1;
  c->hits_current = false;
  const int rc = match_device_impl(c, P, nhits);
  if (rc != 0 && c->up.active && c->up.s_up) (void)hipStreamSynchronize(c->up.s_up);
  c->hits_current = rc == 0;
  return rc;
}
```

Measured before the change: 2.098 billion.

## Defer per-batch hit compaction via staged slabs and a tile directory

Instead of compacting each batch's staged tuples into the dense hit list right after every match launch, each batch now writes into its own slab of the stage buffer. A small kernel records per-tile source offsets and prefix sums in a directory. Consumers (copy, pack, compact-pack, partition accumulate, results order) read straight through the directory, and dense compaction happens lazily only when needed. This removes a per-batch device-to-device copy of all hits, at the cost of a larger resident stage buffer and a binary search plus indirection in the pack kernels. The old eager path remains available behind an environment variable.

Result: no change. 2.103 billion, median of 2 (+0.2%).

```diff
diff --git a/include/muscato_hip.h b/include/muscato_hip.h
--- a/include/muscato_hip.h
+++ b/include/muscato_hip.h
@@ -136,6 +136,9 @@
 int musc_stream_plan(uint64_t nreads, uint32_t fixed_len, uint32_t batch_reads, uint64_t* ends, uint8_t* is_batch_end,
                      uint64_t capacity, uint64_t* n, uint64_t* planned_batches);
 
+int musc_stage_plan(uint64_t nreads, uint32_t batch_reads, int streamed, uint32_t resident_wg, uint64_t* r0, uint64_t* tile0,
+                    uint64_t* slab_off, uint64_t* slab_cap, uint64_t capacity, uint64_t* n, uint64_t* ntiles, uint64_t* stage_tuples);
+
 int musc_overflow_probes(musc_ctx* ctx, uint32_t** read_idx, uint32_t** window, uint64_t* n);
 void musc_free_u32(uint32_t* p);
 
diff --git a/muscato_amd/_lib.py b/muscato_amd/_lib.py
--- a/muscato_amd/_lib.py
+++ b/muscato_amd/_lib.py
@@ -67,7 +67,7 @@
     "musc_reads_load_ascii", "musc_reads_load_packed", "musc_reads_load_packed32", "musc_reads_sort_unique",
     "musc_reads_prep_fastq", "musc_fastq_prep_free",
     "musc_match_device", "musc_hits_copy", "musc_hits_copy_packed", "musc_hits_copy_compact", "musc_hits_unpack", "musc_match", "musc_free_hits",
-    "musc_get_stats", "musc_last_instance", "musc_instances", "musc_stream_plan", "musc_gather", "musc_gather_rccl", "musc_rccl_probe", "musc_overflow_probes", "musc_free_u32",
+    "musc_get_stats", "musc_last_instance", "musc_instances", "musc_stream_plan", "musc_stage_plan", "musc_gather", "musc_gather_rccl", "musc_rccl_probe", "musc_overflow_probes", "musc_free_u32",
     "musc_results_set_gene_text", "musc_results_set_read_text", "musc_results_order", "musc_results_hits", "musc_results_text",
     "musc_results_last_ms", "musc_results_number_key",
 ]
@@ -130,6 +130,9 @@
     lib.musc_last_instance.argtypes = [vp, ctypes.POINTER(ctypes.c_uint32)]
     lib.musc_instances.argtypes = [ctypes.POINTER(ctypes.c_uint32), ctypes.c_uint32, ctypes.POINTER(ctypes.c_uint32)]
     lib.musc_stream_plan.argtypes = [u64, ctypes.c_uint32, ctypes.c_uint32, vp, vp, u64, ctypes.POINTER(u64), ctypes.POINTER(u64)]
+    lib.musc_stage_plan.argtypes = [u64, ctypes.c_uint32, ctypes.c_int, ctypes.c_uint32, vp, vp, vp, vp, u64, ctypes.POINTER(u64),
+                                    ctypes.POINTER(u64), ctypes.POINTER(u64)]
+    lib.musc_stage_plan.restype = ctypes.c_int
     lib.musc_overflow_probes.argtypes = [vp, ctypes.POINTER(vp), ctypes.POINTER(vp), ctypes.POINTER(u64)]
     lib.musc_overflow_probes.restype = ctypes.c_int
     lib.musc_free_u32.argtypes = [vp]
diff --git a/muscato_amd/csrc/kernels_stage_dir.hpp b/muscato_amd/csrc/kernels_stage_dir.hpp
--- /dev/null
+++ b/muscato_amd/csrc/kernels_stage_dir.hpp
@@ -0,0 +1,87 @@
+#pragma once
+
+MUSC_KERNEL __launch_bounds__(256) void k_tile_dir(uint32_t nwt, const uint32_t* __restrict__ tbase, const uint32_t* __restrict__ tpre,
+                                                  unsigned long long slab, unsigned long long tile0,
+                                                  unsigned long long* __restrict__ dir_src, unsigned long long* dir_pre,
+                                                  unsigned long long* __restrict__ counters) {
+  const unsigned long long base = dir_pre[tile0];
+  for (uint32_t wt = blockIdx.x * blockDim.x + threadIdx.x; wt < nwt; wt += gridDim.x * blockDim.x) {
+    dir_src[tile0 + wt] = slab + tbase[wt];
+    dir_pre[tile0 + wt + 1] = base + tpre[wt + 1];
+  }
+  if (blockIdx.x == 0 && threadIdx.x == 0) counters[CNT_HITS] = base + tpre[nwt];
+}
+
+DEV unsigned long long dir_find(const unsigned long long* __restrict__ dir_pre, unsigned long long ntiles, unsigned long long i) {
+  unsigned long long lo = 0, hi = ntiles;
+  while (hi - lo > 1) {
+    const unsigned long long mid = lo + (hi - lo) / 2;
+    if (dir_pre[mid] <= i) lo = mid;
+    else hi = mid;
+  }
+  return lo;
+}
+
+MUSC_KERNEL __launch_bounds__(256) void k_compact_dir(unsigned long long ntiles, const unsigned long long* __restrict__ dir_src,
+                                                     const unsigned long long* __restrict__ dir_pre, const uint4* __restrict__ stage,
+                                                     uint4* __restrict__ dst, unsigned long long cap, uint32_t* __restrict__ bad) {
+  if (dir_pre[ntiles] > cap) {
+    if (blockIdx.x == 0 && threadIdx.x == 0) atomicOr(bad, 1u);
+    return;
+  }
+  const uint32_t lane = threadIdx.x & 63;
+  for (unsigned long long t = blockIdx.x * 4ull + (threadIdx.x >> 6); t < ntiles; t += gridDim.x * 4ull) {
+    const unsigned long long p0 = dir_pre[t], m = dir_pre[t + 1] - p0;
+    const uint4* __restrict__ src = stage + dir_src[t];
+    uint4* __restrict__ d = dst + p0;
+    for (unsigned long long j = lane; j < m; j += 64) d[j] = src[j];
+  }
+}
+
+
+MUSC_KERNEL __launch_bounds__(256) void k_pack_hits_dir(unsigned long long ntiles, const unsigned long long* __restrict__ dir_src,
+                                                       const unsigned long long* __restrict__ dir_pre, const uint4* __restrict__ stage,
+                                                       unsigned long long t0, unsigned long long t1, uint64_t read_base, PackBits b,
+                                                       uint64_t* __restrict__ out, uint32_t* __restrict__ bad) {
+  const uint32_t lane = threadIdx.x & 63;
+  const unsigned long long ta = dir_find(dir_pre, ntiles, t0), tb = dir_find(dir_pre, ntiles, t1 - 1) + 1;
+  for (unsigned long long t = ta + blockIdx.x * 4ull + (threadIdx.x >> 6); t < tb; t += gridDim.x * 4ull) {
+    const unsigned long long p0 = dir_pre[t], p1 = dir_pre[t + 1];
+    const uint4* __restrict__ src = stage + dir_src[t];
+    const unsigned long long hi = (p1 < t1 ? p1 : t1) - p0;
+    for (unsigned long long j = (p0 > t0 ? 0 : t0 - p0) + lane; j < hi; j += 64) {
+      const uint4 h = src[j];
+      const uint64_t r = (uint64_t)h.x + read_base;
+      if ((b.read < 64 && (r >> b.read)) || ((uint64_t)h.y >> b.gene) || ((uint64_t)h.z >> b.pos) || ((uint64_t)h.w >> b.nmiss))
+        atomicOr(bad, 1u);
+      out[p0 + j] = (((((r << b.gene) | h.y) << b.pos) | h.z) << b.nmiss) | h.w;
+    }
+  }
+}
+
+MUSC_KERNEL __launch_bounds__(256) void k_pack_compact_dir(unsigned long long ntiles, const unsigned long long* __restrict__ dir_src,
+                                                          const unsigned long long* __restrict__ dir_pre,
+                                                          const uint4* __restrict__ stage, unsigned long long t0, unsigned long long t1,
+                                                          PackBits b, uint32_t* __restrict__ words, uint8_t* __restrict__ counts,
+                                                          uint32_t* __restrict__ bad) {
+  const uint32_t lane = threadIdx.x & 63;
+  const unsigned long long ta = dir_find(dir_pre, ntiles, t0), tb = dir_find(dir_pre, ntiles, t1 - 1) + 1;
+  for (unsigned long long t = ta + blockIdx.x * 4ull + (threadIdx.x >> 6); t < tb; t += gridDim.x * 4ull) {
+    const unsigned long long p0 = dir_pre[t], p1 = dir_pre[t + 1], m = p1 - p0;
+    const uint4* __restrict__ src = stage + dir_src[t];
+    const unsigned long long hi = (p1 < t1 ? p1 : t1) - p0;
+    for (unsigned long long j = (p0 > t0 ? 0 : t0 - p0) + lane; j < hi; j += 64) {
+      const uint4 h = src[j];
+      if (((uint64_t)h.y >> b.gene) || ((uint64_t)h.z >> b.pos) || ((uint64_t)h.w >> b.nmiss)) atomicOr(bad, 1u);
+      words[p0 + j] = (((h.y << b.pos) | h.z) << b.nmiss) | h.w;
+      const uint32_t prev = j ? src[j - 1].x : 0xFFFFFFFFu;
+      if (j && prev > h.x) atomicOr(bad, 4u);
+      if (j == 0 || prev != h.x) {
+        uint32_t cnt = 1;
+        while (j + cnt < m && cnt < 256 && src[j + cnt].x == h.x) cnt++;
+        if (cnt > 255) atomicOr(bad, 2u);
+        counts[h.x] = (uint8_t)cnt;
+      }
+    }
+  }
+}
diff --git a/muscato_amd/csrc/muscato_hip.hip b/muscato_amd/csrc/muscato_hip.hip
--- a/muscato_amd/csrc/muscato_hip.hip
+++ b/muscato_amd/csrc/muscato_hip.hip
@@ -20,6 +20,7 @@
 #include "kernels_index.hpp"
 #include "kernels_screen.hpp"
 #include "kernels_confirm.hpp"
+#include "kernels_stage_dir.hpp"
 #include "kernels_match.hpp"
 #include "kernels_match_lane_inst.hpp"
 #include "kernels_screen_lane.hpp"
@@ -149,6 +150,11 @@
   return it == sp.batch_end.end() ? 0 : *it - r0;
 }
 
+struct StageSlab {
+  uint32_t n;
+  uint64_t cap;
+};
+
 struct EnvKnobs {
   enum { IDX_AUTO = 0, IDX_CLASSIC, IDX_LINES, IDX_CLASSIC64 };
   int index = IDX_AUTO;
@@ -166,6 +172,7 @@
   bool no_spec = false;
   long batch_reads = 0;
   long index_budget_mb = 0;
+  bool eager_compact = false;
   void read() {
     *this = EnvKnobs();
     auto is = [](const char* v, const char* w) { return v && !strcmp(v, w); };
@@ -187,6 +194,7 @@
     no_spec = getenv("MUSC_NO_SPEC") != nullptr;
     if ((e = getenv("MUSC_BATCH_READS"))) batch_reads = atol(e);
     if ((e = getenv("MUSC_DEBUG_INDEX_BUDGET_MB"))) index_budget_mb = atol(e);
+    eager_compact = (e = getenv("MUSC_EAGER_COMPACT")) && atoi(e) > 0;
   }
 };
 
@@ -299,6 +307,10 @@
 
   DevBuf<musc_hit> hits;
   uint64_t nhits = 0;
+  bool staged = false;
+  DevBuf<unsigned long long> dir_src, dir_pre;
+  uint64_t dir_tiles = 0;
+  std::vector<StageSlab> slabs;
   DevBuf<uint64_t> packed;
   std::vector<hipEvent_t> dl_ev;
   DevBuf<musc_hit> gathered;
@@ -330,6 +342,7 @@
   musc_params graph_params;
   int graph_block_mode = -1;
   uint32_t graph_batches = 0;
+  uint64_t graph_tiles = 0;
   std::vector<hipEvent_t> ev_pool;
   size_t ev_used = 0;
   double nm_pmatch = -1.0;
@@ -634,6 +647,7 @@
     c->bs[i].cdesc.release();
   }
   c->scan_tmp.release(); c->tcount2.release(); c->tpre.release(); c->stage.release(); c->rdx.release();
+  c->dir_src.release(); c->dir_pre.release();
   c->p_nx.release();
   c->nmiss_tab.release();
   c->block_table.release();
@@ -1488,6 +1502,29 @@
 #include "muscato_pass.hpp"
 
 extern "C" {
+
+static int staged_compact(musc_ctx* c, musc_hit* dst, uint64_t cap) {
+  if (!c->staged || !c->nhits) return 0;
+  Range rg("k_compact_dir");
+  HIPCHK(c, hipMemsetAsync(c->d_flag, 0, 4, c->stream));
+  hipLaunchKernelGGL(k_compact_dir, dim3(std::min(nblk(c->dir_tiles, 4), 4u * MAX_GRID)), dim3(256), 0, c->stream,
+                     (unsigned long long)c->dir_tiles, c->dir_src.p, c->dir_pre.p, c->stage.p, reinterpret_cast<uint4*>(dst),
+                     (unsigned long long)cap, c->d_flag);
+  HIPCHK(c, hipGetLastError());
+  uint32_t* const h_bad = reinterpret_cast<uint32_t*>(c->h_pinned);
+  HIPCHK(c, hipMemcpyAsync(h_bad, c->d_flag, 4, hipMemcpyDeviceToHost, c->stream));
+  HIPCHK(c, hipStreamSynchronize(c->stream));
+  if (*h_bad) return fail(c, 12, "internal: the staged tuples do not fit the %llu their list has room for", (unsigned long long)cap);
+  return 0;
+}
+
+static int hits_dense(musc_ctx* c) {
+  if (!c->staged) return 0;
+  int rc;
+  if ((rc = ensure(c, c->hits, c->nhits ? c->nhits : 1)) || (rc = staged_compact(c, c->hits.p, c->hits.cap))) return rc;
+  c->staged = false;
+  return 0;
+}
 
 static int match_partitions_run(musc_ctx* c, const musc_params* P, uint64_t* nhits) {
   const uint32_t np = (uint32_t)c->part_first.size() - 1;
@@ -1534,7 +1571,11 @@
     sum.index_bytes = s.index_bytes;
     if (nh) {
       if ((rc = ensure(c, c->pacc, seg[p] + nh, true))) break;
-      HIPCHK(c, hipMemcpyAsync(c->pacc.p + seg[p], c->hits.p, nh * sizeof(musc_hit), hipMemcpyDeviceToDevice, c->stream));
+      if (c->staged) {
+        if ((rc = staged_compact(c, c->pacc.p + seg[p], nh))) break;
+      } else {
+        HIPCHK(c, hipMemcpyAsync(c->pacc.p + seg[p], c->hits.p, nh * sizeof(musc_hit), hipMemcpyDeviceToDevice, c->stream));
+      }
       hipLaunchKernelGGL(k_part_best, dim3(std::min(nblk(nh, 256), 4u * MAX_GRID)), dim3(256), 0, c->stream,
                          reinterpret_cast<const uint4*>(c->pacc.p + seg[p]), nh, c->pbest.p);
       HIPCHK(c, hipGetLastError());
@@ -1606,6 +1647,7 @@
   sum.ms_total += merge_ms;
   sum.n_reads = nr;
   sum.n_hits = c->nhits = total;
+  c->staged = false;
   sum.n_overflow_blocks = check_blocks ? c->h_pinned[0] : ~0ull;
   c->stats = sum;
   c->last_exact_blocks = check_blocks;
@@ -1636,6 +1678,9 @@
   if (c->nhits == 0) return 0;
   if (!dst) return fail(c, 2, "musc_hits_copy: dst is NULL");
   HIPCHK(c, hipSetDevice(c->device));
+  if (c->staged && dst_on_device) return staged_compact(c, dst, capacity);
+  int rc = hits_dense(c);
+  if (rc) return rc;
   HIPCHK(c, hipMemcpyAsync(dst, c->hits.p, c->nhits * sizeof(musc_hit),
                            dst_on_device ? hipMemcpyDeviceToDevice : hipMemcpyDeviceToHost, c->stream));
   HIPCHK(c, hipStreamSynchronize(c->stream));
@@ -1737,6 +1782,8 @@
   if (!hits) {
     if (!c->hits_current)
       return fail(c, 2, "musc_results_order: the resident tuple list is not that of a pass over the reads and the database in hand");
+    const int rcd = hits_dense(c);
+    if (rcd) return rcd;
     d_in = reinterpret_cast<const uint4*>(c->hits.p);
     n = c->nhits;
   } else if (on_device && ((uintptr_t)hits & 15u)) {
@@ -2004,6 +2051,13 @@
   return 0;
 }
 
+static unsigned staged_grid_n(const musc_ctx* c, uint64_t t0, uint64_t t1) {
+  const double share = c->nhits ? (double)(t1 - t0) / (double)c->nhits : 1.0;
+  const uint64_t tiles = (uint64_t)((double)c->dir_tiles * share) + 64;
+  return std::max(1u, std::min(nblk(tiles, 4), 4u * MAX_GRID));
+}
+#define staged_grid(c, t0, t1) dim3(staged_grid_n((c), (t0), (t1)))
+
 extern "C++" {
 template <class Pack>
 static int download_chunks(musc_ctx* c, uint64_t n, size_t elem, const void* src, void* dst, Pack pack) {
@@ -2077,8 +2131,13 @@
   HIPCHK(c, hipMemsetAsync(c->d_flag, 0, 4, c->stream));
   const uint4* const hits = reinterpret_cast<const uint4*>(c->hits.p);
   auto pack = [&](uint64_t t0, uint64_t t1) {
-    hipLaunchKernelGGL(k_pack_hits, dim3(std::min(nblk(t1 - t0, 256), MAX_GRID)), dim3(256), 0, c->stream, hits + t0, t1 - t0,
-                       read_base, b, out + t0, c->d_flag);
+    if (c->staged)
+      hipLaunchKernelGGL(k_pack_hits_dir, staged_grid(c, t0, t1), dim3(256), 0, c->stream, (unsigned long long)c->dir_tiles,
+                         c->dir_src.p, c->dir_pre.p, c->stage.p, (unsigned long long)t0, (unsigned long long)t1, read_base, b, out,
+                         c->d_flag);
+    else
+      hipLaunchKernelGGL(k_pack_hits, dim3(std::min(nblk(t1 - t0, 256), MAX_GRID)), dim3(256), 0, c->stream, hits + t0, t1 - t0,
+                         read_base, b, out + t0, c->d_flag);
   };
   uint32_t* const h_bad = reinterpret_cast<uint32_t*>(c->h_pinned);
   if (dst_on_device) {
@@ -2128,16 +2187,24 @@
   uint32_t* const h_bad = reinterpret_cast<uint32_t*>(c->h_pinned);
   if (dst_on_device) {
     if (c->nhits) {
-      hipLaunchKernelGGL(k_pack_compact, dim3(std::min(nblk(c->nhits, 256), MAX_GRID)), dim3(256), 0, c->stream, hits, c->nhits,
-                         b, dw, dc, c->d_flag);
+      if (c->staged)
+        hipLaunchKernelGGL(k_pack_compact_dir, staged_grid(c, 0, c->nhits), dim3(256), 0, c->stream, (unsigned long long)c->dir_tiles,
+                           c->dir_src.p, c->dir_pre.p, c->stage.p, 0ull, (unsigned long long)c->nhits, b, dw, dc, c->d_flag);
+      else
+        hipLaunchKernelGGL(k_pack_compact, dim3(std::min(nblk(c->nhits, 256), MAX_GRID)), dim3(256), 0, c->stream, hits, c->nhits,
+                           b, dw, dc, c->d_flag);
       HIPCHK(c, hipGetLastError());
     }
     HIPCHK(c, hipMemcpyAsync(h_bad, c->d_flag, 4, hipMemcpyDeviceToHost, c->stream));
     HIPCHK(c, hipStreamSynchronize(c->stream));
   } else {
     int rc = download_chunks(c, c->nhits, 4, dw, words, [&](uint64_t t0, uint64_t t1) {
-      hipLaunchKernelGGL(k_pack_compact_range, dim3(std::min(nblk(t1 - t0, 256), MAX_GRID)), dim3(256), 0, c->stream, hits,
-                         c->nhits, t0, t1, b, dw, dc, c->d_flag);
+      if (c->staged)
+        hipLaunchKernelGGL(k_pack_compact_dir, staged_grid(c, t0, t1), dim3(256), 0, c->stream, (unsigned long long)c->dir_tiles,
+                           c->dir_src.p, c->dir_pre.p, c->stage.p, (unsigned long long)t0, (unsigned long long)t1, b, dw, dc, c->d_flag);
+      else
+        hipLaunchKernelGGL(k_pack_compact_range, dim3(std::min(nblk(t1 - t0, 256), MAX_GRID)), dim3(256), 0, c->stream, hits,
+                           c->nhits, t0, t1, b, dw, dc, c->d_flag);
     });
     const int rc_end = download_end(c, h_bad, counts, dc, c->nreads);
     if (rc || rc_end) return rc ? rc : rc_end;
@@ -2308,6 +2375,39 @@
   return 0;
 }
 
+int musc_stage_plan(uint64_t nreads, uint32_t batch_reads, int streamed, uint32_t resident_wg, uint64_t* r0, uint64_t* tile0,
+                    uint64_t* slab_off, uint64_t* slab_cap, uint64_t capacity, uint64_t* n, uint64_t* ntiles, uint64_t* stage_tuples) {
+  if (!n || resident_wg < 1 || nreads >= 0xFFFFFFF0ull) return 1;
+  if (batch_reads < 1 || batch_reads > (16u << 20)) batch_reads = 16u << 20;
+  StreamPlan sp;
+  BatchCursor cur;
+  cur.bsz = batch_reads;
+  if (streamed) {
+    stream_plan(nreads, batch_reads, &sp);
+    cur.plan = &sp;
+  }
+  StageCursor sc;
+  StageSlab prev{0, 0};
+  for (uint64_t at = 0; at < nreads;) {
+    const uint32_t nb = cur.reads_at(at, nreads);
+    if (!nb) return 1;
+    const uint64_t cap = stage_slab_first(nb, stage_waves(nb, resident_wg), sc.b ? &prev : nullptr);
+    if (sc.b < capacity) {
+      if (r0) r0[sc.b] = at;
+      if (tile0) tile0[sc.b] = sc.tile0;
+      if (slab_off) slab_off[sc.b] = sc.slab_off;
+      if (slab_cap) slab_cap[sc.b] = cap;
+    }
+    prev = StageSlab{nb, cap};
+    sc.next(nblk(nb, WT), cap);
+    at += nb;
+  }
+  *n = sc.b;
+  if (ntiles) *ntiles = sc.tile0;
+  if (stage_tuples) *stage_tuples = sc.slab_off;
+  return 0;
+}
+
 int musc_gather(musc_ctx* const* ctxs, int n, const uint64_t* read_base, musc_hit** hits, uint64_t* nhits) {
   if (!ctxs || n < 1 || !hits || !nhits) return 1;
   uint64_t total = 0;
@@ -2432,8 +2532,17 @@
   HIPCHK(c0, hipSetDevice(c0->device));
   int rc = ensure(c0, c0->gathered, total ? total : 1);
   if (rc) return rc;
-  if (c0->nhits)
+  if (c0->nhits && c0->staged) {
+    if ((rc = staged_compact(c0, c0->gathered.p, c0->gathered.cap))) return rc;
+  } else if (c0->nhits) {
     HIPCHK(c0, hipMemcpyAsync(c0->gathered.p, c0->hits.p, c0->nhits * sizeof(musc_hit), hipMemcpyDeviceToDevice, c0->stream));
+  }
+  for (int i = 1; i < n; i++) {
+    if (!ctxs[i]->nhits || !ctxs[i]->staged) continue;
+    HIPCHK(ctxs[i], hipSetDevice(ctxs[i]->device));
+    if ((rc = hits_dense(ctxs[i]))) return fail(c0, rc, "musc_gather_rccl: %s", ctxs[i]->err.c_str());
+  }
+  HIPCHK(c0, hipSetDevice(c0->device));
   if (n > 1) {
     ncclResult_t r = api->GroupStart();
     for (int i = 1; i < n && r == ncclSuccess; i++) {
diff --git a/muscato_amd/csrc/muscato_pass.hpp b/muscato_amd/csrc/muscato_pass.hpp
--- a/muscato_amd/csrc/muscato_pass.hpp
+++ b/muscato_amd/csrc/muscato_pass.hpp
@@ -108,6 +108,22 @@
 constexpr uint64_t BATCH_OFFSET_CAP = 1ull << 31;
 
 constexpr uint64_t FIRST_PASS_TUPLES_PER_READ = 2, FIRST_PASS_DESC_PER_READ = 4, FIRST_PASS_DESC_MIN = 1024;
+
+static uint64_t stage_waves(uint64_t n, uint64_t resident) { return std::min<uint64_t>(nblk(n, TILE), resident) * (TILE / 64); }
+static uint64_t stage_slab_first(uint64_t n, uint64_t swaves, const StageSlab* prev) {
+  uint64_t cap = std::max<uint64_t>(FIRST_PASS_TUPLES_PER_READ * n, swaves * 64);
+  if (prev && prev->n) cap = std::max<uint64_t>(cap, (prev->cap * n + prev->n - 1) / prev->n);
+  return std::min<uint64_t>(cap, BATCH_OFFSET_CAP);
+}
+static uint64_t stage_slab_grown(uint64_t need, uint64_t swaves) { return need + need / 4 + swaves; }
+struct StageCursor {
+  uint64_t b = 0, tile0 = 0, slab_off = 0;
+  void next(uint32_t ntiles, uint64_t cap) {
+    b++;
+    tile0 += ntiles;
+    slab_off += cap;
+  }
+};
 
 struct PassClock {
   Timer tm;
@@ -199,11 +215,11 @@
   return resident;
 }
 
-static void launch_match(musc_ctx* c, const PassPlan& pl, uint64_t r0, uint32_t n, unsigned ngrid) {
+static void launch_match(musc_ctx* c, const PassPlan& pl, uint64_t r0, uint32_t n, unsigned ngrid, uint4* stage, uint64_t stage_cap) {
   const size_t lds = match_dyn_lds(match_kind(c, pl.pp.W), pl.pp.W, pl.block_mode);
   const uint32_t* const rdx = c->reads_have_x ? (const uint32_t*)c->rdx.p : (const uint32_t*)nullptr;
   hipLaunchKernelGGL(pl.kern, dim3(ngrid), dim3(TILE), lds, c->stream, c->rd, r0, n, c->d_mp, c->nmiss_tab.p, c->ctx_T,
-                     c->ctx_E, c->stage.p, c->stage.cap, c->spill.p, c->spill.cap, c->bs[0].tbase.p, c->tcount2.p,
+                     c->ctx_E, stage, stage_cap, c->spill.p, c->spill.cap, c->bs[0].tbase.p, c->tcount2.p,
                      pl.block_mode, pl.block_thr, c->block_table.p, c->counters, rdx);
 }
 
@@ -258,6 +274,7 @@
   c->stats.ms_index_build = keep_index_ms;
   c->stats.n_reads = c->nreads;
   c->nhits = 0;
+  c->staged = false;
 
   pl->P = P;
   PathParams& pp = pl->pp;
@@ -364,6 +381,20 @@
                      reinterpret_cast<uint4*>(c->hits.p), c->hits.cap, c->counters);
   HIPCHK(c, hipGetLastError());
   hipLaunchKernelGGL(k_advance, dim3(1), dim3(64), 0, st, c->tpre.p, ntiles, c->counters);
+  HIPCHK(c, hipGetLastError());
+  tm.end(4, st);
+  return 0;
+}
+
+static int launch_directory(musc_ctx* c, Timer& tm, uint32_t ntiles, const StageCursor& sc) {
+  hipStream_t st = c->stream;
+  tm.begin(4, st);
+  tm.begin(1, st);
+  const int rc = scan_u32(c, c->tcount2.p, c->tpre.p, (uint64_t)ntiles + 1, false, c->scan_tmp.p, st);
+  if (rc) return rc;
+  tm.end(1, st);
+  hipLaunchKernelGGL(k_tile_dir, dim3(std::min(nblk(ntiles, 256), MAX_GRID)), dim3(256), 0, st, ntiles, c->bs[0].tbase.p, c->tpre.p,
+                     (unsigned long long)sc.slab_off, (unsigned long long)sc.tile0, c->dir_src.p, c->dir_pre.p, c->counters);
   HIPCHK(c, hipGetLastError());
   tm.end(4, st);
   return 0;
@@ -445,6 +476,7 @@
     (void)hipGraphExecDestroy(c->graph_exec);
     c->graph_exec = nullptr;
   }
+  const bool eager = c->env.eager_compact;
   for (int attempt = 0;; attempt++) {
     if (attempt > 40) return fail(c, 12, "internal: the context pass did not converge on buffer sizes");
     PassClock clk(c);
@@ -470,27 +502,52 @@
     uint64_t tot[CNT_BATCH_WORDS] = {0}, r0 = 0;
     c->stats.n_batches = c->stats.match_launches = 0;
     bool again = false;
+    StageCursor sc;
+    if (!eager && !sized && ((rc = ensure(c, c->dir_pre, 2)) || (rc = ensure(c, c->dir_src, 1)))) return rc;
+    if (!eager && (!c->dir_pre.p || !c->dir_src.p)) {
+      *what = PASS_RERUN_CAREFUL;
+      return 0;
+    }
     if (!replay) {
       HIPCHK(c, hipMemsetAsync(c->counters, 0, CNT_WORDS * sizeof(unsigned long long), c->stream));
       if (pl.block_mode == 2) HIPCHK(c, hipMemsetAsync(c->block_table.p, 0, (1ull << BLOCK_TABLE_BITS) * 4, c->stream));
+      if (!eager) HIPCHK(c, hipMemsetAsync(c->dir_pre.p, 0, sizeof(unsigned long long), c->stream));
     }
     while (!replay && r0 < c->nreads) {
       const uint32_t n = cur.reads_at(r0, c->nreads);
       const uint32_t ntiles = nblk(n, WT);
       const uint64_t sgrid = std::min<uint64_t>(nblk(n, TILE), pl.resident);
-      const uint64_t swaves = sgrid * (TILE / 64);
+      const uint64_t swaves = stage_waves(n, pl.resident);
+      uint64_t slab_cap = 0;
       if (!sized) {
-        if ((rc = ensure_tiles(c, c->bs[0], ntiles)) ||
-            (rc = ensure(c, c->stage, std::max<uint64_t>(FIRST_PASS_TUPLES_PER_READ * n, swaves * 64))) ||
-            (rc = ensure(c, c->spill, swaves * 32)))
-          return rc;
+        if ((rc = ensure_tiles(c, c->bs[0], ntiles)) || (rc = ensure(c, c->spill, swaves * 32))) return rc;
+        if (eager) {
+          if ((rc = ensure(c, c->stage, std::max<uint64_t>(FIRST_PASS_TUPLES_PER_READ * n, swaves * 64)))) return rc;
+        } else {
+          if (sc.b >= c->slabs.size() || c->slabs[sc.b].n != n) {
+            c->slabs.resize(sc.b);
+            c->slabs.push_back(StageSlab{n, stage_slab_first(n, swaves, sc.b ? &c->slabs[sc.b - 1] : nullptr)});
+          }
+          if ((rc = ensure(c, c->stage, sc.slab_off + c->slabs[sc.b].cap, true)) ||
+              (rc = ensure(c, c->dir_src, sc.tile0 + ntiles + 1, true)) || (rc = ensure(c, c->dir_pre, sc.tile0 + ntiles + 2, true)))
+            return rc;
+        }
         HIPCHK(c, hipMemsetAsync(c->counters + CNT_BATCH, 0, CNT_BATCH_WORDS * sizeof(unsigned long long), c->stream));
+      }
+      if (eager) {
+        slab_cap = c->stage.cap;
+      } else if (sc.b < c->slabs.size() && c->slabs[sc.b].n == n && sc.slab_off + c->slabs[sc.b].cap <= c->stage.cap &&
+                 sc.tile0 + ntiles + 1 <= c->dir_pre.cap && sc.tile0 + ntiles <= c->dir_src.cap) {
+        slab_cap = c->slabs[sc.b].cap;
+      } else {
+        *what = PASS_RERUN_CAREFUL;
+        return 0;
       }
       if ((rc = upload_prepare(c, r0, n, c->stream))) return rc;
       clk.tm.begin(0);
       {
         Range rg("k_match");
-        launch_match(c, pl, r0, n, (unsigned)sgrid);
+        launch_match(c, pl, r0, n, (unsigned)sgrid, c->stage.p + sc.slab_off, slab_cap);
       }
       HIPCHK(c, hipGetLastError());
       clk.tm.end(0);
@@ -508,18 +565,27 @@
         }
         if (h[CNT_FLAGS] & FLAG_SPEC_REFUSED)
           return fail(c, 12, "internal: the kernel instance specialised for geometry %d refused this run's parameters", c->spec_geom);
-        if (h[CNT_FLAGS] || need_stage > c->stage.cap || need_spill > c->spill.cap) {
-          if (need_stage > c->stage.cap && (rc = ensure(c, c->stage, need_stage + need_stage / 4 + swaves))) return rc;
+        if (h[CNT_FLAGS] || need_stage > slab_cap || need_spill > c->spill.cap) {
+          if (need_stage > slab_cap) {
+            if (!eager) c->slabs[sc.b].cap = stage_slab_grown(need_stage, swaves);
+            else if ((rc = ensure(c, c->stage, stage_slab_grown(need_stage, swaves)))) return rc;
+          }
           if (need_spill > c->spill.cap && (rc = ensure(c, c->spill, need_spill + need_spill / 4 + swaves))) return rc;
           again = true;
           break;
         }
         for (int i = 0; i < CNT_BATCH_WORDS; i++) tot[i] += h[CNT_BATCH + i];
-        if ((rc = ensure(c, c->hits, h[CNT_HITS] + h[CNT_BATCH + MB_TUPLES], true))) return rc;
-      }
-      Range rgc("scan + k_compact_w");
-      const dim3 cgrid(std::min(nblk(ntiles, 4), 4u * MAX_GRID));
-      if ((rc = launch_compact(c, clk.tm, k_compact_w, cgrid, ntiles, c->bs[0].tbase.p, c->stream))) return rc;
+        if (eager && (rc = ensure(c, c->hits, h[CNT_HITS] + h[CNT_BATCH + MB_TUPLES], true))) return rc;
+      }
+      if (eager) {
+        Range rgc("scan + k_compact_w");
+        const dim3 cgrid(std::min(nblk(ntiles, 4), 4u * MAX_GRID));
+        if ((rc = launch_compact(c, clk.tm, k_compact_w, cgrid, ntiles, c->bs[0].tbase.p, c->stream))) return rc;
+      } else {
+        Range rgc("scan + k_tile_dir");
+        if ((rc = launch_directory(c, clk.tm, ntiles, sc))) return rc;
+      }
+      if (!eager) sc.next(ntiles, slab_cap);
       r0 += n;
     }
     if (again) continue;
@@ -539,6 +605,7 @@
       c->graph_params = *pl.P;
       c->graph_block_mode = pl.block_mode;
       c->graph_batches = c->stats.n_batches;
+      c->graph_tiles = sc.tile0;
     }
     if (capture || replay) {
       c->stats.n_batches = c->stats.match_launches = c->graph_batches;
@@ -546,7 +613,13 @@
       HIPCHK(c, hipGraphLaunch(c->graph_exec, c->stream));
       HIPCHK(c, hipEventRecord(clk.ev1, c->stream));
     }
-    return pass_verdict(c, pl, cur, tot, clk, what);
+    *what = PASS_DONE;
+    if ((rc = pass_verdict(c, pl, cur, tot, clk, what))) return rc;
+    if (*what == PASS_DONE && !eager) {
+      c->staged = true;
+      c->dir_tiles = replay ? c->graph_tiles : sc.tile0;
+    }
+    return 0;
   }
 }
 
```
